# maxpit/human-pose-estimation

Hardware: AMD Instinct MI355X
Metric: images/sec (224x224, batch 256/GPU) (higher is better)
Workload: dtype f32; 1 GPU; batch=256/GPU 224x224x3 synthetic images, fp32 ResNet-50 v1 + 3-iter regressor + SMPL LBS at all 3 stages (configs[1] at batch 256; the BASELINE metric batch); global_batch=256, parallelism=dp1 (batch shard, replicated weights), regressor=synthetic 'survey' variant, input=float32 images resident in HBM

## Files before the change

### human-pose-estimation_amd/_lib.py

```python
from __future__ import annotations

import ctypes as C
import os

import numpy as np

_HERE = os.path.dirname(os.path.abspath(__file__))
LIB_PATH = os.path.join(_HERE, "lib", "libhpe_hip.so")

NUM_CONV = 53
NUM_DENSE = 3
NUM_CRITIC_DENSE = 9
NUM_VERTS = 6890
THETA_DIM = 85
FEATURE_DIM = 2048


class HpeError(RuntimeError):
    pass


class HpeConfig(C.Structure):
    _fields_ = [
        ("struct_size", C.c_int),
        ("device", C.c_int),
        ("max_batch", C.c_int),
        ("num_stage", C.c_int),
        ("bn_eps", C.c_float),
        ("encoder_dtype", C.c_int),
        ("n_streams", C.c_int),
        ("dual_gemm", C.c_int),
        ("stem_fused", C.c_int),
        ("wino_min_c", C.c_int),
        ("wino_min_items", C.c_int),
        ("wino_fused", C.c_int),
        ("wino_fused_min_hw", C.c_int),
        ("mesh_a2b", C.c_int),
        ("wino_f4", C.c_int),
        ("wino4_fused", C.c_int),
        ("bf16_p8", C.c_int),
        ("wino4_ksplit", C.c_int),
        ("chain_fuse", C.c_int),
        ("halo3", C.c_int),
        ("f32_split", C.c_int),
    ]


PLAN_OPTIONS = ("n_streams", "dual_gemm", "stem_fused", "wino_min_c", "wino_min_items", "wino_fused", "wino_fused_min_hw", "mesh_a2b", "wino_f4", "wino4_fused", "bf16_p8", "wino4_ksplit", "chain_fuse", "halo3", "f32_split")


class HpeSmplModel(C.Structure):
    _fields_ = [
        ("v_template", C.c_void_p),
        ("shapedirs", C.c_void_p),
        ("posedirs", C.c_void_p),
        ("J_regressor", C.c_void_p),
        ("weights", C.c_void_p),
        ("kp_regressor", C.c_void_p),
        ("parents", C.c_void_p),
        ("num_kp", C.c_int),
    ]


class HpeCriticModel(C.Structure):
    _fields_ = [("kernel", C.c_void_p * NUM_CRITIC_DENSE), ("bias", C.c_void_p * NUM_CRITIC_DENSE)]


class HpeRenderParams(C.Structure):
    _fields_ = [
        ("struct_size", C.c_int),
        ("color_id", C.c_int),
        ("do_alpha", C.c_int),
        ("rot_axis", C.c_int),
        ("rot_deg", C.c_float),
        ("near", C.c_float),
        ("far", C.c_float),
    ]


class HpeAugmentFrame(C.Structure):
    _fields_ = [("frame_offset", C.c_longlong), ("seg_offset", C.c_longlong), ("H", C.c_int), ("W", C.c_int), ("newH", C.c_int),
                ("newW", C.c_int), ("cx", C.c_int), ("cy", C.c_int), ("fx", C.c_float), ("fy", C.c_float), ("flip", C.c_int),
                ("inside", C.c_int), ("rx", C.c_float), ("ry", C.c_float)]


class HpeJpegInfo(C.Structure):
    _fields_ = [("status", C.c_int), ("H", C.c_int), ("W", C.c_int), ("ncomp", C.c_int), ("hs", C.c_int * 3), ("vs", C.c_int * 3),
                ("blocks_w", C.c_int * 3), ("blocks_h", C.c_int * 3), ("coefs", C.c_longlong)]


class HpeJpegImage(C.Structure):
    _fields_ = [("coef_offset", C.c_longlong * 3), ("plane_offset", C.c_longlong * 3), ("out_offset", C.c_longlong), ("H", C.c_int),
                ("W", C.c_int), ("ncomp", C.c_int), ("channels", C.c_int), ("hmax", C.c_int), ("vmax", C.c_int), ("blocks_w", C.c_int * 3),
                ("blocks_h", C.c_int * 3), ("idct_group0", C.c_int), ("store_group0", C.c_int), ("quant", (C.c_ubyte * 64) * 3)]


class HpeJpegEncImage(C.Structure):
    _fields_ = [("frame_offset", C.c_longlong), ("coef_offset", C.c_longlong * 3), ("H", C.c_int), ("W", C.c_int), ("C", C.c_int),
                ("hmax", C.c_int), ("vmax", C.c_int), ("blocks_w", C.c_int * 3), ("blocks_h", C.c_int * 3), ("real_w", C.c_int * 3),
                ("real_h", C.c_int * 3), ("group0", C.c_int), ("quant", (C.c_ubyte * 64) * 2)]


class HpePngImage(C.Structure):
    _fields_ = [("raw_offset", C.c_longlong), ("pal_offset", C.c_longlong), ("work_offset", C.c_longlong), ("out_offset", C.c_longlong),
                ("H", C.c_int), ("W", C.c_int), ("color_type", C.c_int), ("depth", C.c_int), ("channels", C.c_int), ("rowbytes", C.c_int),
                ("bpp", C.c_int), ("store_group0", C.c_int)]


class HpePngFilterImage(C.Structure):
    _fields_ = [("frame_offset", C.c_longlong), ("scan_offset", C.c_longlong), ("H", C.c_int), ("W", C.c_int), ("C", C.c_int), ("row0", C.c_int)]


def record_dtype(struct):
    d = np.dtype(struct)
    formats = []
    for name in d.names:
        t, shape = d.fields[name][0], ()
        while t.subdtype:
            t, shape = t.subdtype[0], shape + t.subdtype[1]
        formats.append((t, shape))
    return np.dtype({"names": list(d.names), "formats": formats, "offsets": [d.fields[n][1] for n in d.names], "itemsize": d.itemsize})


GEMM_DENSE, GEMM_STRIDED, GEMM_CONV3, GEMM_DUAL = 0, 1, 2, 4
GEMM_TILES = ((128, 128), (128, 64), (64, 64), (64, 128), (128, 128), (128, 64), (256, 128))


class HpeDebugGemm(C.Structure):
    _fields_ = [("struct_size", C.c_int), ("mode", C.c_int), ("tile", C.c_int), ("M", C.c_int), ("N", C.c_int), ("K", C.c_int),
                ("lda", C.c_int), ("ldw", C.c_int), ("ldy", C.c_int), ("ldres", C.c_int), ("w_rows", C.c_int), ("relu", C.c_int),
                ("Hi", C.c_int), ("Wi", C.c_int), ("Cin", C.c_int), ("Ho", C.c_int), ("Wo", C.c_int), ("stride", C.c_int),
                ("k1_slabs", C.c_int), ("y_slab8", C.c_int), ("use_splitk", C.c_int), ("reserved", C.c_int),
                ("x", C.c_void_p), ("x2", C.c_void_p), ("wt", C.c_void_p), ("residual", C.c_void_p), ("scale", C.c_void_p),
                ("shift", C.c_void_p), ("y", C.c_void_p), ("split_k", C.POINTER(C.c_int))]


CONV_KERNELS = ("f32", "f32s", "bf16", "bf16_p8", "halo3", "wino", "wino_fused", "wino4", "wino4_fused")
BLOCK_JOINS = ("separate", "dual", "chain")


class HpeConvRoute(C.Structure):
    _fields_ = [("struct_size", C.c_int), ("kernel", C.c_int), ("mode", C.c_int), ("tile", C.c_int), ("in_slab8", C.c_int), ("out_slab8", C.c_int),
                ("join", C.c_int), ("join_kernel", C.c_int), ("join_tile", C.c_int), ("next_slab8", C.c_int), ("packs", C.c_uint), ("reserved", C.c_int)]


def conv_route(lib, cfg, idx, B, concurrent=False, residual=False, workspace=True):
    r = HpeConvRoute(struct_size=C.sizeof(HpeConvRoute))
    check(lib.hpe_debug_conv_route(C.byref(cfg), int(idx), int(B), int(concurrent), int(residual), int(workspace), C.byref(r)))
    return r


ENCODER_PACKINGS = ("w", "w_split", "wino_u", "wino4_u", "stem_w", "scale", "shift", "w_dual", "w_dual_split", "shift_dual", "dxw", "flat")

OUTPUT_FIELDS = ("verts", "joints", "cams", "theta", "J_transformed", "kp2d", "verts2d", "Rs")


class HpeOutputs(C.Structure):
    _fields_ = [(n, C.c_void_p) for n in OUTPUT_FIELDS]


_PROTOS = {
    "hpe_last_error": (C.c_char_p, []),
    "hpe_version": (C.c_char_p, []),
    "hpe_conv_layer_name": (C.c_char_p, [C.c_int]),
    "hpe_bn_layer_name": (C.c_char_p, [C.c_int]),
    "hpe_conv_layer_geometry": (C.c_int, [C.c_int, C.POINTER(C.c_int)]),
    "hpe_config_init": (None, [C.POINTER(HpeConfig)]),
    "hpe_create": (C.c_int, [C.POINTER(HpeConfig), C.POINTER(C.c_void_p)]),
    "hpe_destroy": (C.c_int, [C.c_void_p]),
    "hpe_load_smpl": (C.c_int, [C.c_void_p, C.POINTER(HpeSmplModel)]),
    "hpe_load_conv": (C.c_int, [C.c_void_p, C.c_int] + [C.c_void_p] * 6),
    "hpe_load_dense": (C.c_int, [C.c_void_p, C.c_int, C.c_void_p, C.c_void_p]),
    "hpe_load_mean_theta": (C.c_int, [C.c_void_p, C.c_void_p]),
    "hpe_finalize": (C.c_int, [C.c_void_p]),
    "hpe_forward": (C.c_int, [C.c_void_p, C.c_void_p, C.c_int, C.POINTER(HpeOutputs), C.c_int, C.c_void_p]),
    "hpe_forward_pipelined": (C.c_int, [C.c_void_p, C.c_void_p, C.c_int, C.POINTER(HpeOutputs), C.c_int, C.c_void_p]),
    "hpe_join": (C.c_int, [C.c_void_p, C.c_void_p]),
    "hpe_tail": (C.c_int, [C.c_void_p, C.c_void_p, C.c_int, C.POINTER(HpeOutputs), C.c_int, C.c_void_p]),
    "hpe_tail_stream": (C.c_void_p, [C.c_void_p]),
    "hpe_encoder": (C.c_int, [C.c_void_p, C.c_void_p, C.c_int, C.c_void_p, C.c_void_p]),
    "hpe_regress_stage": (C.c_int, [C.c_void_p, C.c_void_p, C.c_void_p, C.c_int, C.c_void_p, C.c_void_p]),
    "hpe_smpl": (C.c_int, [C.c_void_p, C.c_void_p, C.c_int, C.POINTER(HpeOutputs), C.c_void_p]),
    "hpe_smpl_backward": (C.c_int, [C.c_void_p, C.c_void_p, C.c_int, C.POINTER(HpeOutputs), C.c_void_p, C.c_void_p]),
    "hpe_orth_proj": (C.c_int, [C.c_void_p, C.c_void_p, C.c_int, C.c_int, C.c_void_p, C.c_void_p]),
    "hpe_reproject_vertices": (C.c_int, [C.c_void_p, C.c_void_p, C.c_int, C.c_int, C.c_float, C.c_float, C.c_void_p, C.c_void_p]),
    "hpe_preprocess_u8": (C.c_int, [C.c_void_p, C.c_int, C.c_int, C.c_int, C.c_void_p, C.POINTER(C.c_int), C.c_void_p]),
    "hpe_preprocess_u8_batch": (C.c_int, [C.c_void_p, C.POINTER(C.c_longlong), C.POINTER(C.c_int), C.c_int, C.c_int, C.c_void_p, C.POINTER(C.c_int),
                                          C.c_void_p, C.c_void_p]),
    "hpe_augment_plan": (C.c_int, [C.c_int, C.c_void_p, C.c_void_p, C.c_void_p, C.c_void_p, C.c_void_p, C.c_int, C.c_void_p, C.c_void_p, C.c_void_p]),
    "hpe_augment_batch": (C.c_int, [C.c_void_p, C.c_void_p, C.c_void_p, C.c_void_p, C.c_void_p, C.c_int, C.c_void_p, C.c_void_p, C.c_void_p, C.c_void_p]),
    "hpe_adam_advance": (C.c_int, [C.c_void_p, C.c_double, C.c_double, C.c_double, C.c_void_p]),
    "hpe_adam_apply": (C.c_int, [C.c_void_p, C.c_void_p, C.c_void_p, C.c_void_p, C.c_longlong, C.c_void_p, C.c_float, C.c_float, C.c_float, C.c_void_p]),
    "hpe_adam_set_step": (C.c_int, [C.c_void_p, C.c_longlong, C.c_double, C.c_double, C.c_void_p]),
    "hpe_debug_adam_power": (C.c_int, [C.c_double, C.c_longlong, C.POINTER(C.c_double)]),
    "hpe_jpeg_info": (C.c_int, [C.c_int, C.c_void_p, C.c_void_p, C.c_void_p]),
    "hpe_jpeg_decode": (C.c_int, [C.c_int, C.c_void_p, C.c_void_p, C.c_void_p, C.c_int, C.c_void_p, C.c_longlong, C.c_void_p, C.c_void_p, C.c_void_p]),
    "hpe_jpeg_backend": (C.c_int, [C.c_void_p, C.c_void_p, C.c_int, C.c_void_p, C.c_longlong, C.c_void_p, C.c_longlong, C.c_void_p, C.c_longlong,
                                   C.c_void_p]),
    "hpe_jpeg_encode_layout": (C.c_int, [C.c_int, C.c_void_p, C.c_void_p, C.c_int, C.c_int, C.c_int, C.c_void_p, C.c_void_p]),
    "hpe_jpeg_forward": (C.c_int, [C.c_void_p, C.c_void_p, C.c_int, C.c_void_p, C.c_longlong, C.c_void_p, C.c_longlong, C.c_void_p]),
    "hpe_jpeg_entropy_encode": (C.c_int, [C.c_void_p, C.c_int, C.c_void_p, C.c_longlong, C.c_int, C.c_int, C.c_int, C.c_int, C.c_void_p, C.c_longlong,
                                          C.c_void_p, C.c_void_p]),
    "hpe_png_backend": (C.c_int, [C.c_void_p, C.c_void_p, C.c_int, C.c_void_p, C.c_longlong, C.c_void_p, C.c_longlong, C.c_void_p, C.c_longlong,
                                  C.c_void_p]),
    "hpe_png_filter": (C.c_int, [C.c_void_p, C.c_void_p, C.c_int, C.c_void_p, C.c_longlong, C.c_void_p, C.c_longlong, C.c_void_p]),
    "hpe_draw_panels": (C.c_int, [C.c_void_p] * 6 + [C.c_int, C.c_int, C.c_int, C.c_void_p, C.c_void_p]),
    "hpe_draw_skeleton": (C.c_int, [C.c_void_p] * 4 + [C.c_int, C.c_int, C.c_int, C.c_int, C.c_int, C.c_void_p]),
    "hpe_get_original": (C.c_int, [C.c_void_p, C.c_void_p, C.c_int, C.c_int, C.c_int, C.POINTER(C.c_int), C.c_float, C.c_int, C.c_void_p, C.POINTER(C.c_float), C.c_void_p, C.c_void_p, C.c_void_p]),
    "hpe_kp_loss": (C.c_int, [C.c_void_p, C.c_void_p, C.c_int, C.c_int, C.c_void_p, C.c_void_p]),
    "hpe_kp_loss_backward": (C.c_int, [C.c_void_p, C.c_void_p, C.c_int, C.c_int, C.c_void_p, C.c_void_p, C.c_void_p]),
    "hpe_mesh_loss": (C.c_int, [C.c_void_p, C.c_void_p, C.c_void_p, C.c_int, C.c_int, C.c_int, C.c_int, C.c_void_p, C.c_void_p]),
    "hpe_mesh_loss_grad": (C.c_int, [C.c_void_p, C.c_void_p, C.c_void_p, C.c_int, C.c_int, C.c_int, C.c_int, C.c_void_p, C.c_void_p, C.c_void_p,
                                     C.c_void_p, C.c_void_p]),
    "hpe_val_losses": (C.c_int, [C.c_void_p, C.c_void_p, C.c_void_p, C.POINTER(C.c_void_p), C.POINTER(C.c_void_p), C.c_int, C.c_int, C.c_int,
                                 C.c_int, C.c_int, C.c_int, C.c_void_p, C.c_void_p]),
    "hpe_critic_layer_name": (C.c_char_p, [C.c_int]),
    "hpe_critic_layer_shape": (C.c_int, [C.c_int, C.POINTER(C.c_int)]),
    "hpe_load_critic": (C.c_int, [C.c_void_p, C.POINTER(HpeCriticModel)]),
    "hpe_critic": (C.c_int, [C.c_void_p, C.c_void_p, C.c_int, C.c_void_p, C.c_int, C.c_void_p, C.c_int, C.c_void_p, C.c_void_p, C.c_void_p]),
    "hpe_critic_backward": (C.c_int, [C.c_void_p, C.c_void_p, C.c_int, C.c_void_p, C.c_int, C.c_void_p, C.c_int, C.c_void_p, C.c_void_p,
                                      C.c_void_p, C.c_void_p, C.c_void_p, C.c_void_p]),
    "hpe_critic_param_floats": (C.c_int, []),
    "hpe_critic_param_offset": (C.c_int, [C.c_int, C.c_int]),
    "hpe_critic_weight_grad_ws_floats": (C.c_longlong, [C.c_int]),
    "hpe_critic_reserve": (C.c_int, [C.c_void_p, C.c_int]),
    "hpe_critic_weight_grad": (C.c_int, [C.c_void_p, C.c_void_p, C.c_int, C.c_void_p, C.c_int, C.c_void_p, C.c_int, C.c_void_p, C.c_void_p,
                                         C.c_void_p, C.c_void_p, C.c_void_p, C.c_int, C.c_void_p, C.c_void_p]),
    "hpe_critic_get_params": (C.c_int, [C.c_void_p, C.c_void_p, C.c_void_p]),
    "hpe_critic_set_params_dev": (C.c_int, [C.c_void_p, C.c_void_p, C.c_void_p]),
    "hpe_regressor_param_floats": (C.c_int, []),
    "hpe_regressor_param_offset": (C.c_int, [C.c_int, C.c_int]),
    "hpe_regressor_get_params": (C.c_int, [C.c_void_p, C.c_void_p, C.c_void_p]),
    "hpe_regressor_set_params_dev": (C.c_int, [C.c_void_p, C.c_void_p, C.c_void_p]),
    "hpe_regressor_forward_train": (C.c_int, [C.c_void_p, C.c_void_p, C.c_int, C.c_void_p, C.c_void_p, C.c_void_p]),
    "hpe_regressor_backward": (C.c_int, [C.c_void_p, C.c_void_p, C.c_int, C.c_void_p, C.c_void_p, C.c_void_p, C.c_void_p, C.c_void_p]),
    "hpe_encoder_param_floats": (C.c_int, []),
    "hpe_encoder_param_offset": (C.c_int, [C.c_int, C.c_int]),
    "hpe_encoder_train_reserve": (C.c_int, [C.c_void_p, C.c_int]),
    "hpe_encoder_train_ws_floats": (C.c_longlong, [C.c_int]),
    "hpe_encoder_wg_slices": (C.c_int, [C.c_int, C.c_int]),
    "hpe_encoder_forward_train": (C.c_int, [C.c_void_p, C.c_void_p, C.c_int, C.c_void_p, C.c_void_p]),
    "hpe_encoder_backward": (C.c_int, [C.c_void_p, C.c_void_p, C.c_int, C.c_void_p, C.c_void_p, C.c_void_p]),
    "hpe_encoder_get_params": (C.c_int, [C.c_void_p, C.c_void_p, C.c_void_p]),
    "hpe_encoder_set_params": (C.c_int, [C.c_void_p, C.c_void_p]),
    "hpe_encoder_set_params_dev": (C.c_int, [C.c_void_p, C.c_void_p, C.c_void_p]),
    "hpe_debug_encoder_packing_bytes": (C.c_longlong, [C.c_void_p, C.c_int, C.c_int]),
    "hpe_debug_encoder_packing": (C.c_int, [C.c_void_p, C.c_int, C.c_int, C.c_void_p, C.c_void_p]),
    "hpe_debug_conv_backward": (C.c_int, [C.c_void_p, C.c_int, C.c_void_p, C.c_void_p, C.c_void_p, C.c_int, C.c_void_p, C.c_void_p, C.c_void_p]),
    "hpe_debug_maxpool_backward": (C.c_int, [C.c_void_p, C.c_void_p, C.c_int, C.c_int, C.c_int, C.c_void_p, C.c_void_p]),
    "hpe_debug_avgpool_backward": (C.c_int, [C.c_void_p, C.c_int, C.c_int, C.c_int, C.c_void_p, C.c_void_p]),
    "hpe_debug_encoder_stash": (C.c_int, [C.c_void_p, C.c_int, C.c_void_p, C.c_void_p]),
    "hpe_debug_encoder_stash_batch": (C.c_int, [C.c_void_p]),
    "hpe_encoder_stat_floats": (C.c_int, []),
    "hpe_encoder_stat_offset": (C.c_int, [C.c_int, C.c_int]),
    "hpe_encoder_train_reserve_batchnorm": (C.c_int, [C.c_void_p, C.c_int]),
    "hpe_encoder_train_ws_floats_batchnorm": (C.c_longlong, [C.c_int]),
    "hpe_debug_encoder_bn_slices": (C.c_int, [C.c_int, C.c_int]),
    "hpe_encoder_forward_batchnorm": (C.c_int, [C.c_void_p, C.c_void_p, C.c_int, C.c_void_p, C.c_void_p]),
    "hpe_encoder_backward_batchnorm": (C.c_int, [C.c_void_p, C.c_void_p, C.c_int, C.c_void_p, C.c_void_p, C.c_void_p]),
    "hpe_encoder_get_stats": (C.c_int, [C.c_void_p, C.c_void_p, C.c_void_p]),
    "hpe_encoder_update_stats": (C.c_int, [C.c_void_p, C.c_void_p, C.c_double, C.c_int, C.c_void_p]),
    "hpe_encoder_set_stats_dev": (C.c_int, [C.c_void_p, C.c_void_p, C.c_void_p]),
    "hpe_debug_conv_batchnorm": (C.c_int, [C.c_void_p, C.c_int, C.c_void_p, C.c_int, C.c_void_p, C.c_int, C.c_void_p, C.c_void_p, C.c_void_p, C.c_void_p]),
    "hpe_debug_conv_backward_batchnorm": (C.c_int, [C.c_void_p, C.c_int, C.c_void_p, C.c_void_p, C.c_void_p, C.c_void_p, C.c_int, C.c_void_p, C.c_void_p,
                                                    C.c_void_p]),
    "hpe_debug_encoder_stash_raw": (C.c_int, [C.c_void_p, C.c_int, C.c_void_p, C.c_void_p]),
    "hpe_debug_encoder_batch_stats": (C.c_int, [C.c_void_p, C.c_void_p, C.c_void_p]),
    "hpe_device_status": (C.c_int, [C.c_void_p, C.c_void_p]),
    "hpe_debug_conv": (C.c_int, [C.c_void_p, C.c_int, C.c_void_p, C.c_int, C.c_void_p, C.c_int, C.c_void_p, C.c_void_p]),
    "hpe_debug_chain": (C.c_int, [C.c_void_p, C.c_int, C.c_void_p, C.c_void_p, C.c_int, C.c_void_p, C.c_void_p, C.POINTER(C.c_int), C.c_void_p]),
    "hpe_debug_stem": (C.c_int, [C.c_void_p, C.c_void_p, C.c_int, C.c_int, C.c_void_p, C.c_void_p]),
    "hpe_debug_gemm": (C.c_int, [C.c_void_p, C.c_void_p, C.c_void_p, C.c_int, C.c_int, C.c_int, C.c_int, C.c_int, C.c_void_p, C.c_int, C.c_void_p, C.c_void_p]),
    "hpe_debug_gemm_ex": (C.c_int, [C.c_void_p, C.POINTER(HpeDebugGemm), C.c_void_p]),
    "hpe_debug_gemm_check": (C.c_int, [C.POINTER(HpeDebugGemm), C.c_int, C.c_int]),
    "hpe_debug_conv_route": (C.c_int, [C.POINTER(HpeConfig), C.c_int, C.c_int, C.c_int, C.c_int, C.c_int, C.POINTER(HpeConvRoute)]),
    "hpe_debug_maxpool": (C.c_int, [C.c_void_p, C.c_int, C.c_int, C.c_int, C.c_void_p, C.c_void_p]),
    "hpe_debug_avgpool": (C.c_int, [C.c_void_p, C.c_int, C.c_int, C.c_int, C.c_void_p, C.c_void_p]),
    "hpe_debug_joint_regress": (C.c_int, [C.c_void_p, C.c_void_p, C.c_int, C.c_int, C.c_void_p, C.c_void_p]),
    "hpe_enable_timing": (C.c_int, [C.c_void_p, C.c_int]),
    "hpe_get_timings": (C.c_int, [C.c_void_p, C.POINTER(C.c_float)]),
    "hpe_get_span_stats": (C.c_int, [C.c_void_p, C.POINTER(C.c_float), C.POINTER(C.c_int)]),
    "hpe_get_loss_timings": (C.c_int, [C.c_void_p, C.POINTER(C.c_float)]),
    "hpe_debug_set_loss_counter": (C.c_int, [C.c_void_p, C.c_void_p]),
    "hpe_get_conv_timings": (C.c_int, [C.c_void_p, C.POINTER(C.c_float)]),
    "hpe_render_params_init": (None, [C.POINTER(HpeRenderParams)]),
    "hpe_renderer_create": (C.c_int, [C.c_int, C.c_void_p, C.c_int, C.c_int, C.c_int, C.POINTER(C.c_void_p)]),
    "hpe_renderer_destroy": (C.c_int, [C.c_void_p]),
    "hpe_render": (C.c_int, [C.c_void_p, C.c_void_p, C.c_void_p, C.c_int, C.c_int, C.c_int, C.c_void_p, C.POINTER(HpeRenderParams), C.c_void_p,
                             C.c_void_p]),
    "hpe_debug_render_ids": (C.c_int, [C.c_void_p, C.c_void_p, C.c_void_p, C.c_int, C.c_int, C.c_int, C.POINTER(HpeRenderParams), C.c_void_p,
                                       C.c_void_p, C.c_void_p]),
    "hpe_debug_render_vertices": (C.c_int, [C.c_void_p, C.c_void_p, C.c_void_p, C.c_int, C.c_int, C.c_int, C.POINTER(HpeRenderParams),
                                            C.c_void_p, C.c_void_p]),
}

_lib = None


def load():
    global _lib
    if _lib is not None:
        return _lib
    if not os.path.exists(LIB_PATH):
        raise HpeError(
            "%s not found: build it with `python -c 'import __graft_entry__ as g; g.build()'` "
# ... 29 lines not shown
```

### human-pose-estimation_amd/build.py

```python
from __future__ import annotations

import os
import shutil
import subprocess
import sys

HERE = os.path.dirname(os.path.abspath(__file__))
CSRC = os.path.join(HERE, "csrc")
LIBDIR = os.path.join(HERE, "lib")
LIB = os.path.join(LIBDIR, "libhpe_hip.so")
SOURCES = ["conv_gemm.hip", "conv_gemm_f32s.hip", "conv_gemm_bf16.hip", "conv_gemm_bf16_p8.hip", "conv_chain_bf16.hip", "conv_chain_f32.hip", "conv3_halo_bf16.hip", "conv_wino.hip", "conv_wino4.hip", "stem_fused.hip", "encoder_ops.hip", "smpl.hip", "losses.hip", "prepost.hip", "render.hip", "hpe_plan.hip", "hpe_finalize.hip", "hpe_encoder.hip", "hpe_api.hip", "hpe_render_api.hip", "smpl_bwd.hip", "critic.hip", "critic_train.hip", "regressor_train.hip", "augment.hip", "encoder_train.hip", "encoder_grad.hip", "encoder_repack.hip", "encoder_bn.hip", "jpeg_entropy.hip", "jpeg_decode.hip", "jpeg_huffman_enc.hip", "jpeg_encode.hip", "png_decode.hip", "png_encode.hip", "draw.hip", "adam.hip"]
CFLAGS = ["--offload-arch=gfx950", "-O3", "-std=c++17", "-fPIC", "-fvisibility=hidden", "-fno-fast-math"]


def _hipcc():
    for cand in (os.environ.get("HIPCC"), shutil.which("hipcc"), "/opt/rocm/bin/hipcc"):
        if cand and os.path.exists(cand):
            return cand
    raise RuntimeError("hipcc not found (set HIPCC or install ROCm under /opt/rocm)")


def _deps():
    return [os.path.join(CSRC, f) for f in os.listdir(CSRC) if f.endswith(".h")] + [os.path.join(HERE, "..", "include", "hpe.h")]


def _obj_stale(src, obj):
    if not os.path.exists(obj):
        return True
    t = os.path.getmtime(obj)
    return any(os.path.getmtime(d) > t for d in [src] + _deps() if os.path.exists(d))


def _flags_now():
    return " ".join(CFLAGS + os.environ.get("HPE_EXTRA_FLAGS", "").split())


def built_flags():
    tag = os.path.join(LIBDIR, "obj", "flags.txt")
    return open(tag).read() if os.path.exists(tag) else ""


def _stale():
    if not os.path.exists(LIB):
        return True
    if built_flags() != _flags_now():
        return True
    t = os.path.getmtime(LIB)
    deps = [os.path.join(CSRC, f) for f in os.listdir(CSRC)] + [os.path.join(HERE, "..", "include", "hpe.h")]
    return any(os.path.getmtime(d) > t for d in deps if os.path.exists(d))


def build(force=False, verbose=False):
    if not force and not _stale():
        return LIB
    os.makedirs(LIBDIR, exist_ok=True)
    objdir = os.path.join(LIBDIR, "obj")
    os.makedirs(objdir, exist_ok=True)
    extra = os.environ.get("HPE_EXTRA_FLAGS", "").split()
    tag = os.path.join(objdir, "flags.txt")
    flags_now = _flags_now()
    if force or not os.path.exists(tag) or open(tag).read() != flags_now:
        for f in os.listdir(objdir):
            os.remove(os.path.join(objdir, f))
    hipcc = _hipcc()
    jobs = []
    for s in SOURCES:
        src = os.path.join(CSRC, s)
        if not os.path.exists(src):
            continue
        obj = os.path.join(objdir, s.replace(".hip", ".o"))
        jobs.append((src, obj))

    def compile_one(job):
        src, obj = job
        if not _obj_stale(src, obj):
            return None
        cmd = [hipcc] + CFLAGS + extra + ["-c", "-o", obj + ".tmp%d" % os.getpid(), src]
        if verbose:
            print(" ".join(cmd), file=sys.stderr)
        r = subprocess.run(cmd, capture_output=True, text=True)
        if r.returncode != 0:
            return "hipcc failed on %s:\n%s%s" % (os.path.basename(src), r.stdout, r.stderr)
        os.replace(obj + ".tmp%d" % os.getpid(), obj)
        return None

    from concurrent.futures import ThreadPoolExecutor

    with ThreadPoolExecutor(max_workers=min(len(jobs), max(1, (os.cpu_count() or 2) - 1))) as ex:
        errs = [e for e in ex.map(compile_one, jobs) if e]
    if errs:
        raise RuntimeError("\n".join(errs))
    open(tag, "w").write(flags_now)
    tmp = LIB + ".tmp%d" % os.getpid()
    cmd = [hipcc, "--offload-arch=gfx950", "-shared", "-fPIC", "-o", tmp] + [o for _, o in jobs]
    r = subprocess.run(cmd, capture_output=True, text=True)
    if r.returncode != 0:
        raise RuntimeError("link failed:\n" + r.stdout + r.stderr)
    os.replace(tmp, LIB)
    return LIB


if __name__ == "__main__":
    print(build(force="--force" in sys.argv, verbose=True))
```

### human-pose-estimation_amd/csrc/encoder_repack.hip

```cpp
#include <hip/hip_runtime.h>

#include <string>

#include "hpe_ctx.h"

namespace {

struct RepackLayer {
    float *w, *scale, *shift, *wino_u, *wino4_u, *dxw;
    unsigned short* w_split;
    int kh, cin, cout, n_pad, k_pad;
    int off[4];
    int stat;
};

struct RepackDual {
    float *w, *shift;
    unsigned short* split;
    int i2c, i1, K1, K2, N, n_pad;
};

enum { F_WT, F_BN, F_WINO, F_WINO4, F_DXW, F_DUAL, F_COUNT };

struct RepackForm {
    int n;
    int item[HPE_NUM_CONV];
    unsigned block0[HPE_NUM_CONV + 1];
};

struct RepackTable {
    RepackLayer L[HPE_NUM_CONV];
    RepackDual D[4];
    RepackForm F[F_COUNT];
};

constexpr int TILE_N = 32, TILE_K = 64;

__device__ inline int find_item(const RepackForm& f, unsigned b, unsigned* local) {
    int s = 0;
    while (s + 1 < f.n && f.block0[s + 1] <= b) ++s;
    *local = b - f.block0[s];
    return f.item[s];
}

__device__ inline void store_split(unsigned short* d, size_t piece, float x) {
    unsigned short h[3];
    bf16_split3(x, h);
    d[0] = h[0];
    d[piece] = h[1];
    d[2 * piece] = h[2];
}

__global__ __launch_bounds__(256) void repack_wt_kernel(const RepackTable* __restrict__ T, const float* __restrict__ flat) {
    unsigned lb;
    const int idx = find_item(T->F[F_WT], blockIdx.x, &lb);
    const RepackLayer& L = T->L[idx];
    const int kt_n = (L.k_pad + TILE_K - 1) / TILE_K;
    const int nt = lb / kt_n, kt = lb - nt * kt_n;
    const int k = kt * TILE_K + (threadIdx.x & 63);
    if (k >= L.k_pad) return;
    long row = -1;
    if (idx == 0) {
        const int kh = k >> 5, kw = (k & 31) >> 2, ci = k & 3;
        if (kh < 7 && kw < 7 && ci < 3) row = (kh * 7 + kw) * 3 + ci;
    } else if (k < L.kh * L.kh * L.cin) {
        row = k;
    }
    const float* src = flat + L.off[0];
    const int n0 = nt * TILE_N + (threadIdx.x >> 6) * 8;
#pragma unroll
    for (int j = 0; j < 8; ++j) {
        const int n = n0 + j;
        if (n >= L.n_pad) break;
        const float v = (row >= 0 && n < L.cout) ? src[row * L.cout + n] : 0.f;
        L.w[(size_t)n * L.k_pad + k] = v;
        if (L.w_split) store_split(L.w_split + (size_t)n * 3 * L.k_pad + k, L.k_pad, v);
    }
}

__global__ __launch_bounds__(256) void repack_bn_kernel(const RepackTable* __restrict__ T, const float* __restrict__ flat,
                                                        const float* __restrict__ mean, const double* __restrict__ sd) {
    unsigned lb;
    const RepackLayer& L = T->L[find_item(T->F[F_BN], blockIdx.x, &lb)];
    const int n = lb * 256 + threadIdx.x;
    if (n >= L.cout) return;
    double scale, shift;
    bn_fold_sd(flat[L.off[2] + n], flat[L.off[1] + n], mean[L.stat + n], flat[L.off[3] + n], sd[L.stat + n], &scale, &shift);
    L.scale[n] = (float)scale;
    L.shift[n] = (float)shift;
}

__global__ __launch_bounds__(256) void repack_stem_kernel(unsigned short* __restrict__ stem_w, const float* __restrict__ kernel) {
    const int o = blockIdx.x * 256 + threadIdx.x;
    if (o >= 64 * 224) return;
    const int n = o / 224, k = o - n * 224;
    const int kh = k >> 5, kw = (k & 31) >> 2, ci = k & 3;
    float v = 0.f;
    if (kw < 7 && ci < 3) v = kernel[((kh * 7 + kw) * 3 + ci) * 64 + n];
    store_split(stem_w + o, 64 * 224, v);
}

template <int TT>
__global__ __launch_bounds__(256) void repack_wino_kernel(const RepackTable* __restrict__ T, const float* __restrict__ flat) {
    unsigned lb;
    const RepackLayer& L = T->L[find_item(T->F[TT == 4 ? F_WINO : F_WINO4], blockIdx.x, &lb)];
    const int c4 = L.cin / 4;
    const int nb = lb / c4, cb = lb - nb * c4;
    const int n = nb * 64 + (threadIdx.x >> 2), ci = cb * 4 + (threadIdx.x & 3);
    const float* src = flat + L.off[0];
    double g[3][3];
#pragma unroll
    for (int a = 0; a < 3; ++a)
#pragma unroll
        for (int b = 0; b < 3; ++b) g[a][b] = src[(((size_t)a * 3 + b) * L.cin + ci) * L.cout + n];
    float* out = TT == 4 ? L.wino_u + wino_u_base(n, ci, L.cin) : L.wino4_u + wino4_u_base(n, ci, L.cin);
    constexpr size_t step = TT == 4 ? 512 : 256;
#pragma unroll
    for (int xi = 0; xi < TT; ++xi)
#pragma unroll
        for (int nu = 0; nu < TT; ++nu) {
            double gx[3], gn[3];
#pragma unroll
            for (int a = 0; a < 3; ++a) {
                gx[a] = TT == 4 ? wino_g(xi, a) : wino4_g(xi, a);
                gn[a] = TT == 4 ? wino_g(nu, a) : wino4_g(nu, a);
            }
            out[(size_t)(xi * TT + nu) * step] = wino_elem(gx, gn, g);
        }
}

__global__ __launch_bounds__(256) void repack_dxw_kernel(const RepackTable* __restrict__ T, const float* __restrict__ flat) {
    unsigned lb;
    const RepackLayer& L = T->L[find_item(T->F[F_DXW], blockIdx.x, &lb)];
    const int taps = L.kh * L.kh, K = taps * L.cout;
    const unsigned o = lb * 256 + threadIdx.x;
    const int ci = (int)(o / (unsigned)K), r = (int)(o - (unsigned)ci * K);
    if (ci >= ((L.cin + 127) / 128) * 128) return;
    const int t = r / L.cout, n = r - t * L.cout;
    L.dxw[o] = ci < L.cin ? flat[L.off[0] + ((size_t)(taps - 1 - t) * L.cin + ci) * L.cout + n] : 0.f;
}

__global__ __launch_bounds__(256) void repack_dual_kernel(const RepackTable* __restrict__ T, const float* __restrict__ flat,
                                                          const float* __restrict__ mean, const double* __restrict__ sd) {
#pragma clang fp contract(off)
    unsigned lb;
    const RepackDual& D = T->D[find_item(T->F[F_DUAL], blockIdx.x, &lb)];
    const int K = D.K1 + D.K2;
    const int kt_n = (K + TILE_K - 1) / TILE_K;
    const int nt = lb / kt_n, kt = lb - nt * kt_n;
    const int k = kt * TILE_K + (threadIdx.x & 63);
    if (k >= K) return;
    const RepackLayer &L2 = T->L[D.i2c], &L1 = T->L[D.i1];
    const RepackLayer& L = k < D.K1 ? L2 : L1;
    const float* src = flat + L.off[0] + (size_t)(k < D.K1 ? k : k - D.K1) * D.N;
    const int n0 = nt * TILE_N + (threadIdx.x >> 6) * 8;
#pragma unroll
    for (int j = 0; j < 8; ++j) {
        const int n = n0 + j;
        if (n >= D.n_pad) break;
        float v = 0.f;
        if (n < D.N) {
            double inv, shift;
            bn_fold_sd(flat[L.off[2] + n], flat[L.off[1] + n], mean[L.stat + n], flat[L.off[3] + n], sd[L.stat + n], &inv, &shift);
            v = (float)(inv * (double)src[n]);
            if (k == 0) {
                double inv1, shift1;
                bn_fold_sd(flat[L1.off[2] + n], flat[L1.off[1] + n], mean[L1.stat + n], flat[L1.off[3] + n], sd[L1.stat + n], &inv1, &shift1);
                D.shift[n] = (float)(shift + shift1);
            }
        }
        D.w[(size_t)n * K + k] = v;
        if (D.split) store_split(D.split + (size_t)n * 3 * K + k, K, v);
    }
}

unsigned blocks_of(int form, const ConvSpec& s, const ConvLayer& L, int idx) {
    switch (form) {
        case F_WT: return (unsigned)(L.n_pad / TILE_N) * ((L.k_pad + TILE_K - 1) / TILE_K);
        case F_BN: return (unsigned)(s.cout + 255) / 256;
        case F_WINO: return L.wino_u ? (unsigned)(s.cin / 4) * (s.cout / 64) : 0;
        case F_WINO4: return L.wino4_u ? (unsigned)(s.cin / 4) * (s.cout / 64) : 0;
        case F_DXW: return (unsigned)((conv_dxw_floats(idx) + 255) / 256);
    }
    return 0;
}

int check_debug(hpe_ctx* c, int idx, int which) {
    if (!c) return fail(HPE_ERR_INVALID, "null ctx");
    if (idx < 0 || idx >= HPE_NUM_CONV || which < 0 || which >= HPE_PACK_COUNT) return fail(HPE_ERR_INVALID, "hpe_debug_encoder_packing: idx or which out of range");
    if (c->dead) return fail(HPE_ERR_STATE, "hpe_finalize failed on this ctx: destroy it and create a new one");
    if (!c->finalized) return fail(HPE_ERR_STATE, "hpe_finalize() has not been called");
    if (!c->have_encoder) return fail(HPE_ERR_STATE, "encoder weights were not loaded before hpe_finalize");
    if (c->bf16) return fail(HPE_ERR_STATE, "hpe_debug_encoder_packing needs an fp32 context");
    return HPE_OK;
}

const void* packing_of(hpe_ctx* c, int idx, int which, size_t* bytes) {
    const ConvSpec& s = specs()[idx];
    const ConvLayer& L = c->conv[idx];
    const size_t wt = (size_t)L.n_pad * L.k_pad, dual = (size_t)round_up(s.cout, 128) * L.k_dual, u = (size_t)s.cin * s.cout;
    const void* p = nullptr;
    size_t n = 0;
    switch (which) {
        case HPE_PACK_W: p = L.w, n = wt * 4; break;
        case HPE_PACK_W_SPLIT: p = L.w_split, n = wt * 3 * 2; break;
        case HPE_PACK_WINO_U: p = L.wino_u, n = u * 16 * 4; break;
        case HPE_PACK_WINO4_U: p = L.wino4_u, n = u * 36 * 4; break;
        case HPE_PACK_STEM_W: p = L.stem_w, n = (size_t)3 * 64 * 224 * 2; break;
        case HPE_PACK_SCALE: p = L.scale, n = (size_t)s.cout * 4; break;
        case HPE_PACK_SHIFT: p = L.shift, n = (size_t)s.cout * 4; break;
        case HPE_PACK_W_DUAL: p = L.w_dual, n = dual * 4; break;
        case HPE_PACK_W_DUAL_SPLIT: p = L.w_dual_split, n = dual * 3 * 2; break;
        case HPE_PACK_SHIFT_DUAL: p = L.shift_dual, n = (size_t)s.cout * 4; break;
        case HPE_PACK_DXW: p = c->et.dxw[idx], n = conv_dxw_floats(idx) * 4; break;
        case HPE_PACK_FLAT:
            if (c->et.flat) p = c->et.flat + layout().off[idx][0];
            n = ((size_t)s.kh * s.kw * s.cin * s.cout + 3 * (size_t)s.cout) * 4;
            break;
    }
    *bytes = p ? n : 0;
    return *bytes ? p : nullptr;
}

}

size_t encoder_repack_reserve_floats() { return (sizeof(RepackTable) + 3) / 4; }

int encoder_repack_reserve(hpe_ctx* c) {
    RepackTable t{};
    for (int i = 0; i < HPE_NUM_CONV; ++i) {
        const ConvSpec& s = specs()[i];
        const ConvLayer& L = c->conv[i];
        RepackLayer& r = t.L[i];
        r.w = L.w;
        r.scale = L.scale;
        r.shift = L.shift;
        r.wino_u = L.wino_u;
        r.wino4_u = L.wino4_u;
        r.dxw = c->et.dxw[i];
        r.w_split = static_cast<unsigned short*>(L.w_split);
        r.kh = s.kh;
        r.cin = s.cin;
        r.cout = s.cout;
        r.n_pad = L.n_pad;
        r.k_pad = L.k_pad;
        for (int w = 0; w < 4; ++w) r.off[w] = layout().off[i][w];
        r.stat = layout().stat[i];
        if (s.kh != s.kw || L.n_pad % TILE_N != 0 || ((L.wino_u || L.wino4_u) && (s.cin % 8 != 0 || s.cout % 64 != 0)))
            return fail(HPE_ERR_STATE, std::string("encoder repack: unexpected geometry of ") + s.name);
    }
    for (int f = 0; f < F_DUAL; ++f) {
        RepackForm& F = t.F[f];
        unsigned b = 0;
        for (int i = 0; i < HPE_NUM_CONV; ++i) {
            const unsigned nb = blocks_of(f, specs()[i], c->conv[i], i);
            if (!nb) continue;
            F.item[F.n] = i;
            F.block0[F.n++] = b;
            b += nb;
        }
        F.block0[F.n] = b;
    }
    {
        RepackForm& F = t.F[F_DUAL];
        unsigned b = 0;
        for (const ResBlock& blk : blocks()) {
            if (!blk.first || !c->conv[blk.i2c].w_dual) continue;
            const ConvLayer& L2 = c->conv[blk.i2c];
            RepackDual& d = t.D[F.n];
            d.w = L2.w_dual;
            d.shift = L2.shift_dual;
            d.split = static_cast<unsigned short*>(L2.w_dual_split);
            d.i2c = blk.i2c;
            d.i1 = blk.i1;
            d.K1 = L2.k1_dual;
            d.K2 = L2.k_dual - L2.k1_dual;
            d.N = specs()[blk.i2c].cout;
            d.n_pad = round_up(d.N, 128);
            F.item[F.n] = F.n;
            F.block0[F.n++] = b;
            b += (unsigned)(d.n_pad / TILE_N) * ((L2.k_dual + TILE_K - 1) / TILE_K);
        }
        F.block0[F.n] = b;
    }
    float* p = nullptr;
    int rc = dev_alloc(c, &p, encoder_repack_reserve_floats(), false);
    if (rc) return rc;
    HIP_TRY(hipMemcpy(p, &t, sizeof(t), hipMemcpyHostToDevice));
    c->et.repack = p;
    static_assert(F_COUNT <= 8, "grid array");
    for (int f = 0; f < F_COUNT; ++f) c->et.repack_grid[f] = t.F[f].block0[t.F[f].n];
    return HPE_OK;
}

hipError_t encoder_repack_launch(hpe_ctx* c, const float* flat, hipStream_t st) {
    const EncTrainWork& w = c->et;
    const RepackTable* T = static_cast<const RepackTable*>(w.repack);
    const unsigned* grid = w.repack_grid;
    if (grid[F_WT]) hipLaunchKernelGGL(repack_wt_kernel, dim3(grid[F_WT]), dim3(256), 0, st, T, flat);
    if (grid[F_BN]) hipLaunchKernelGGL(repack_bn_kernel, dim3(grid[F_BN]), dim3(256), 0, st, T, flat, w.mean, w.sd);
    if (c->conv[0].stem_w)
        hipLaunchKernelGGL(repack_stem_kernel, grid1(64 * 224), dim3(256), 0, st, static_cast<unsigned short*>(c->conv[0].stem_w),
                           flat + layout().off[0][0]);
    if (grid[F_WINO]) hipLaunchKernelGGL(repack_wino_kernel<4>, dim3(grid[F_WINO]), dim3(256), 0, st, T, flat);
    if (grid[F_WINO4]) hipLaunchKernelGGL(repack_wino_kernel<6>, dim3(grid[F_WINO4]), dim3(256), 0, st, T, flat);
    if (grid[F_DXW]) hipLaunchKernelGGL(repack_dxw_kernel, dim3(grid[F_DXW]), dim3(256), 0, st, T, flat);
    if (grid[F_DUAL]) hipLaunchKernelGGL(repack_dual_kernel, dim3(grid[F_DUAL]), dim3(256), 0, st, T, flat, w.mean, w.sd);
    HIPE(hipGetLastError());
    return hipMemcpyAsync(w.flat, flat, (size_t)layout().total * sizeof(float), hipMemcpyDeviceToDevice, st);
}

hipError_t encoder_repack_stats_launch(hpe_ctx* c, hipStream_t st) {
    const EncTrainWork& w = c->et;
    const RepackTable* T = static_cast<const RepackTable*>(w.repack);
    const unsigned* grid = w.repack_grid;
    if (grid[F_BN]) hipLaunchKernelGGL(repack_bn_kernel, dim3(grid[F_BN]), dim3(256), 0, st, T, w.flat, w.mean, w.sd);
    if (grid[F_DUAL]) hipLaunchKernelGGL(repack_dual_kernel, dim3(grid[F_DUAL]), dim3(256), 0, st, T, w.flat, w.mean, w.sd);
    return hipGetLastError();
}

#pragma GCC visibility push(default)
extern "C" {

long long hpe_debug_encoder_packing_bytes(hpe_ctx* c, int idx, int which) {
    if (!c || idx < 0 || idx >= HPE_NUM_CONV || which < 0 || which >= HPE_PACK_COUNT) return 0;
    if (c->dead || !c->finalized || !c->have_encoder || c->bf16) return 0;
    size_t n;
    packing_of(c, idx, which, &n);
    return (long long)n;
}

int hpe_debug_encoder_packing(hpe_ctx* c, int idx, int which, void* dst, void* stream) {
    int rc = check_debug(c, idx, which);
    if (rc) return rc;
    if (!dst) return fail(HPE_ERR_INVALID, "null dst_dev");
    size_t n;
    const void* p = packing_of(c, idx, which, &n);
    if (!p) return fail(HPE_ERR_STATE, "hpe_debug_encoder_packing: this context does not hold that form of that layer");
    DeviceGuard g(c->cfg.device);
    HIP_TRY(hipMemcpyAsync(dst, p, n, hipMemcpyDeviceToDevice, static_cast<hipStream_t>(stream)));
    return HPE_OK;
}

}
#pragma GCC visibility pop
```

### human-pose-estimation_amd/csrc/hpe_api.hip

```cpp
#include <hip/hip_runtime.h>

#include <algorithm>
#include <cmath>
#include <cstdint>
#include <cstdio>
#include <cstdlib>
#include <cstring>
#include <string>
#include <vector>

#include "gemm_contract.h"
#include "hpe_ctx.h"

namespace {
thread_local std::string g_err;
}

int fail(int code, const std::string& msg) {
    g_err = msg;
    return code;
}

int check_ready(hpe_ctx* c, int B, int need) {
    if (!c) return fail(HPE_ERR_INVALID, "null ctx");
    if (c->dead) return fail(HPE_ERR_STATE, "hpe_finalize failed on this ctx: destroy it and create a new one");
    if (!c->finalized) return fail(HPE_ERR_STATE, "hpe_finalize() has not been called");
    if (B < 1 || B > c->cfg.max_batch) return fail(HPE_ERR_INVALID, "batch " + std::to_string(B) + " outside [1, max_batch]");
    if ((need & NEED_ENC) && !c->have_encoder) return fail(HPE_ERR_STATE, "encoder weights were not loaded before hpe_finalize");
    if ((need & NEED_REG) && !c->have_regressor) return fail(HPE_ERR_STATE, "regressor weights / mean theta were not loaded");
    if ((need & NEED_SMPL) && !c->have_smpl) return fail(HPE_ERR_STATE, "SMPL model was not loaded before hpe_finalize");
    return HPE_OK;
}

#pragma GCC visibility push(default)
extern "C" {


const char* hpe_last_error(void) { return g_err.c_str(); }
const char* hpe_version(void) { return "hpe_hip 0.1 (gfx950)"; }

const char* hpe_conv_layer_name(int idx) { return (idx >= 0 && idx < HPE_NUM_CONV) ? specs()[idx].name : nullptr; }
const char* hpe_bn_layer_name(int idx) { return (idx >= 0 && idx < HPE_NUM_CONV) ? specs()[idx].bn : nullptr; }

int hpe_conv_layer_geometry(int idx, int out[7]) {
    if (idx < 0 || idx >= HPE_NUM_CONV || !out) return fail(HPE_ERR_INVALID, "bad conv index");
    const ConvSpec& s = specs()[idx];
    out[0] = s.kh;
    out[1] = s.kw;
    out[2] = s.cin;
    out[3] = s.cout;
    out[4] = s.stride;
    out[5] = s.hin;
    out[6] = s.hout;
    return HPE_OK;
}

void hpe_config_init(HpeConfig* cfg) {
    if (!cfg) return;
    cfg->struct_size = (int)sizeof(HpeConfig);
    cfg->device = 0;
    cfg->max_batch = 8;
    cfg->num_stage = 3;
    cfg->bn_eps = 1e-3f;
    cfg->encoder_dtype = 0;
    cfg->n_streams = cfg->dual_gemm = cfg->stem_fused = cfg->wino_min_c = cfg->wino_min_items = cfg->wino_fused = -1;
    cfg->wino_fused_min_hw = cfg->mesh_a2b = cfg->wino_f4 = cfg->wino4_fused = cfg->bf16_p8 = cfg->wino4_ksplit = cfg->chain_fuse = cfg->halo3 = cfg->f32_split = -1;
}

int hpe_create(const HpeConfig* cfg, hpe_ctx** out) {
    if (!cfg || !out) return fail(HPE_ERR_INVALID, "null argument");
    if (cfg->struct_size != (int)sizeof(HpeConfig))
        return fail(HPE_ERR_INVALID, "HpeConfig.struct_size is " + std::to_string(cfg->struct_size) + ", this library expects " +
                                         std::to_string(sizeof(HpeConfig)) + ": fill the struct with hpe_config_init() of the same header");
    if (cfg->n_streams > 4 || cfg->n_streams == 0) return fail(HPE_ERR_INVALID, "n_streams must be -1 (default) or 1..4");
    if (cfg->mesh_a2b > 2) return fail(HPE_ERR_INVALID, "mesh_a2b must be -1 (default), 0 (grid), 1 (valu) or 2 (mfma)");
    if (cfg->max_batch < 1 || cfg->max_batch > 1024) return fail(HPE_ERR_INVALID, "max_batch must be in [1,1024]");
    if (cfg->num_stage < 1 || cfg->num_stage > 16) return fail(HPE_ERR_INVALID, "num_stage must be in [1,16]");
    if (cfg->encoder_dtype != 0 && cfg->encoder_dtype != 1) return fail(HPE_ERR_INVALID, "encoder_dtype must be 0 (fp32) or 1 (bf16)");
    int ndev = 0;
    if (hipGetDeviceCount(&ndev) != hipSuccess || ndev < 1) return fail(HPE_ERR_NO_DEVICE, "no HIP device visible");
    if (cfg->device < 0 || cfg->device >= ndev) return fail(HPE_ERR_INVALID, "device ordinal out of range");
    hipDeviceProp_t prop;
    HIP_TRY(hipGetDeviceProperties(&prop, cfg->device));
    if (strncmp(prop.gcnArchName, "gfx950", 6) != 0)
        return fail(HPE_ERR_NO_DEVICE, std::string("device is ") + prop.gcnArchName + ", kernels are built for gfx950 only");
    hpe_ctx* c = new hpe_ctx();
    c->cfg = *cfg;
    c->bf16 = cfg->encoder_dtype == 1;
    if (c->cfg.bn_eps <= 0.f) c->cfg.bn_eps = 1e-3f;
    *out = c;
    return HPE_OK;
}

int hpe_destroy(hpe_ctx* c) {
    if (!c) return HPE_OK;
    DeviceGuard g(c->cfg.device);
    (void)hipDeviceSynchronize();
    release_device_state(c);
    delete c;
    return HPE_OK;
}

int hpe_finalize(hpe_ctx* c) {
    if (!c) return fail(HPE_ERR_INVALID, "null ctx");
    if (c->dead) return fail(HPE_ERR_STATE, "an earlier hpe_finalize failed: destroy this ctx and create a new one");
    if (c->finalized) return fail(HPE_ERR_STATE, "already finalized");
    const int rc = finalize_impl(c);
    if (rc != HPE_OK && rc != HPE_ERR_STATE) {
        const std::string keep = g_err;
        DeviceGuard g(c->cfg.device);
        (void)hipDeviceSynchronize();
        release_device_state(c);
        c->dead = true;
        g_err = keep;
    }
    return rc;
}

int hpe_encoder(hpe_ctx* c, const float* images, int B, float* features, void* stream) {
    int rc = check_ready(c, B, NEED_ENC);
    if (rc) return rc;
    if (!images || !features) return fail(HPE_ERR_INVALID, "null pointer");
    DeviceGuard g(c->cfg.device);
    hipStream_t st = static_cast<hipStream_t>(stream);
    if (c->timing) {
        HIP_TRY(hipEventRecord(c->ev[0], st));
        HIP_TRY(hipEventRecord(c->span0[c->span_n % hpe_ctx::SPAN_RING], st));
    }
    HIP_TRY(encoder_impl(c, images, B, features, HPE_FEATURE_DIM, st));
    if (c->timing) {
        HIP_TRY(hipEventRecord(c->span1[c->span_n % hpe_ctx::SPAN_RING], st));
        ++c->span_n;
        HIP_TRY(hipEventRecord(c->ev[1], st));
        HIP_TRY(hipEventRecord(c->ev[4], st));
        c->timed_valid = true;
        c->conv_timed_valid = c->timing >= 2;
    }
    return HPE_OK;
}

int hpe_regress_stage(hpe_ctx* c, const float* features, const float* theta_prev, int B, float* theta_out, void* stream) {
    int rc = check_ready(c, B, NEED_REG);
    if (rc) return rc;
    if (!features || !theta_out) return fail(HPE_ERR_INVALID, "null pointer");
    DeviceGuard g(c->cfg.device);
    hipStream_t st = static_cast<hipStream_t>(stream);
    HIP_TRY(join_tail(c, st));
    HIP_TRY(features_proj(c, features, B, st));
    if (theta_prev)
        HIP_TRY(hpe_launch_copy_theta(theta_prev, HPE_THETA_DIM, c->thA, THETA_LD, B, HPE_THETA_DIM, st));
    else
        HIP_TRY(hpe_launch_tile_theta(c->mean_dev, c->thA, B, THETA_LD, st));
    HIP_TRY(regress_impl(c, c->thA, c->thB, B, st));
    HIP_TRY(hpe_launch_copy_theta(c->thB, THETA_LD, theta_out, HPE_THETA_DIM, B, HPE_THETA_DIM, st));
    return HPE_OK;
}

int hpe_smpl(hpe_ctx* c, const float* theta, int B, const HpeOutputs* outs, void* stream) {
    int rc = check_ready(c, B, NEED_SMPL);
    if (rc) return rc;
    if (!theta || !outs) return fail(HPE_ERR_INVALID, "null pointer");
    DeviceGuard g(c->cfg.device);
    HIP_TRY(join_tail(c, static_cast<hipStream_t>(stream)));
    HIP_TRY(hpe_launch_smpl(c->smpl, c->work, theta, HPE_THETA_DIM, B, outs, static_cast<hipStream_t>(stream)));
    return HPE_OK;
}

int hpe_smpl_backward(hpe_ctx* c, const float* theta, int B, const HpeOutputs* grad_outs, float* grad_theta, void* stream) {
    int rc = check_ready(c, B, NEED_SMPL);
    if (rc) return rc;
    if (!theta || !grad_outs || !grad_theta) return fail(HPE_ERR_INVALID, "null pointer");
    DeviceGuard g(c->cfg.device);
    HIP_TRY(hpe_launch_smpl_backward(c->smpl, c->bwd, theta, B, grad_outs, grad_theta, static_cast<hipStream_t>(stream)));
    return HPE_OK;
}

int hpe_forward(hpe_ctx* c, const float* images, int B, const HpeOutputs* stage_outs, int n_outs, void* stream) {
    return forward_impl(c, images, B, stage_outs, n_outs, static_cast<hipStream_t>(stream), false);
}

int hpe_forward_pipelined(hpe_ctx* c, const float* images, int B, const HpeOutputs* stage_outs, int n_outs, void* stream) {
    return forward_impl(c, images, B, stage_outs, n_outs, static_cast<hipStream_t>(stream), true);
}

int hpe_tail(hpe_ctx* c, const float* features, int B, const HpeOutputs* stage_outs, int n_outs, void* stream) {
    int rc = check_ready(c, B, NEED_REG | NEED_SMPL);
    if (rc) return rc;
    if (!features || !stage_outs) return fail(HPE_ERR_INVALID, "null pointer");
    if (n_outs < 1 || n_outs > c->cfg.num_stage) return fail(HPE_ERR_INVALID, "n_outs must be in [1, num_stage]");
    DeviceGuard g(c->cfg.device);
    hipStream_t st = static_cast<hipStream_t>(stream);
    HIP_TRY(join_tail(c, st));
    c->dense_on_tail = true;
    const hipError_t e = tail_impl(c, features, B, stage_outs, n_outs, st, nullptr);
    c->dense_on_tail = false;
    if (e != hipSuccess) return fail(HPE_ERR_HIP, std::string("hpe_tail: ") + hipGetErrorString(e));
    return HPE_OK;
}

int hpe_join(hpe_ctx* c, void* stream) {
    if (!c || !c->finalized) return fail(HPE_ERR_STATE, "needs a finalized ctx");
    DeviceGuard g(c->cfg.device);
    if (c->tail_pending) HIP_TRY(hipStreamWaitEvent(static_cast<hipStream_t>(stream), c->ev_tail, 0));
    return HPE_OK;
}

void* hpe_tail_stream(hpe_ctx* c) { return (c && c->finalized) ? static_cast<void*>(c->tail_st) : nullptr; }

int hpe_orth_proj(const float* X, const float* cam, int B, int P, float* out, void* stream) {
    if (!X || !cam || !out || B < 1 || P < 1) return fail(HPE_ERR_INVALID, "bad argument");
    HIP_TRY(hpe_launch_orth_proj(X, cam, B, P, 0.f, 0.f, 0, out, static_cast<hipStream_t>(stream)));
    return HPE_OK;
}

int hpe_reproject_vertices(const float* verts, const float* cam, int B, int P, float im_w, float im_h, float* out, void* stream) {
    if (!verts || !cam || !out || B < 1 || P < 1) return fail(HPE_ERR_INVALID, "bad argument");
    HIP_TRY(hpe_launch_orth_proj(verts, cam, B, P, im_w, im_h, 1, out, static_cast<hipStream_t>(stream)));
    return HPE_OK;
}
// ... 692 lines not shown
```

### human-pose-estimation_amd/csrc/hpe_ctx.h

```cpp
#pragma once
#include <hip/hip_runtime.h>

#include <cmath>
#include <cstdint>
#include <cstring>
#include <string>
#include <vector>

#include "../../include/hpe.h"
#include "hpe_internal.h"
#include "hpe_plan.h"

int fail(int code, const std::string& msg);

#define HIP_TRY(expr)                                                                                             \
    do {                                                                                                          \
        hipError_t _e = (expr);                                                                                   \
        if (_e != hipSuccess)                                                                                     \
            return fail(HPE_ERR_HIP, std::string(#expr) + ": " + hipGetErrorString(_e) + " (" __FILE__ ":" +      \
                                         std::to_string(__LINE__) + ")");                                         \
    } while (0)

struct ConvSpec {
    char name[24];
    char bn[24];
    int kh, kw, cin, cout, stride, hin, hout;
};

const std::vector<ConvSpec>& specs();

struct ResBlock {
    int stage;
    bool first, last;
    int i2a, i2b, i2c, i1;
    int in;
};
const std::vector<ResBlock>& blocks();

inline int round_up(int x, int m) { return ((x + m - 1) / m) * m; }

struct ConvLayer {
    std::vector<float> kernel, bias, gamma, beta, mean, var;
    bool loaded = false;
    float* w = nullptr;
    float* scale = nullptr;
    float* shift = nullptr;
    float* w_dual = nullptr;
    float* shift_dual = nullptr;
    int k_dual = 0, k1_dual = 0;
    void* w_split = nullptr;
    void* w_dual_split = nullptr;
    void* stem_w = nullptr;
    float* wino_u = nullptr;
    float* wino4_u = nullptr;
    int n_pad = 0, k_pad = 0;
};

inline int conv_wt_k(int idx, int kh, int kw, int ci) {
    const ConvSpec& s = specs()[idx];
    return idx == 0 ? kh * 32 + kw * 4 + ci : (kh * s.kw + kw) * s.cin + ci;
}

inline int conv_k_pad(int idx, bool bf16) { return round_up(idx == 0 ? 7 * 32 : specs()[idx].kh * specs()[idx].kw * specs()[idx].cin, bf16 ? 64 : 32); }


__host__ __device__ inline size_t wino_u_base(int n, int ci, int cin) {
    return ((((size_t)(n >> 6) * (cin / 8) + (ci >> 3)) * 16) * 2 + ((ci >> 2) & 1)) * 256 + (size_t)(n & 63) * 4 + (ci & 3);
}
__host__ __device__ inline size_t wino4_u_base(int n, int ci, int cin) {
    return (((size_t)(n >> 6) * (cin / 4) + (ci >> 2)) * 36) * 256 + (size_t)(n & 63) * 4 + (ci & 3);
}
__host__ __device__ inline double wino_g(int xi, int a) {
    constexpr double G[4][3] = {{1, 0, 0}, {0.5, 0.5, 0.5}, {0.5, -0.5, 0.5}, {0, 0, 1}};
    return G[xi][a];
}
__host__ __device__ inline double wino4_g(int xi, int a) {
    constexpr double G4[6][3] = {{0.25, 0, 0}, {-1.0 / 6, -1.0 / 6, -1.0 / 6}, {-1.0 / 6, 1.0 / 6, -1.0 / 6},
                                 {1.0 / 24, 1.0 / 12, 1.0 / 6}, {1.0 / 24, -1.0 / 12, 1.0 / 6}, {0, 0, 1}};
    return G4[xi][a];
}
__host__ __device__ inline float wino_elem(const double gx[3], const double gn[3], const double g[3][3]) {
#pragma clang fp contract(off)
    double u = 0.0;
    for (int a = 0; a < 3; ++a)
        for (int b = 0; b < 3; ++b) u += gx[a] * gn[b] * g[a][b];
    return (float)u;
}

__host__ __device__ inline void bn_fold_sd(float gamma, float bias, float mean, float beta, double sd, double* scale, double* shift) {
#pragma clang fp contract(off)
    *scale = (double)gamma / sd;
    *shift = ((double)bias - (double)mean) * *scale + (double)beta;
}
inline double bn_sd(const ConvLayer& L, int n, float eps) { return std::sqrt((double)L.var[n] + (double)eps); }
inline void bn_fold(const ConvLayer& L, int n, float eps, double* scale, double* shift) {
    bn_fold_sd(L.gamma[n], L.bias[n], L.mean[n], L.beta[n], bn_sd(L, n, eps), scale, shift);
}
inline float bn_istd(const ConvLayer& L, int n, float eps) { return (float)(1.0 / std::sqrt((double)L.var[n] + (double)eps)); }

__host__ __device__ inline unsigned short f2bf(float f) {
    unsigned u;
    memcpy(&u, &f, 4);
    return (unsigned short)((u + 0x7FFFu + ((u >> 16) & 1u)) >> 16);
}
__host__ __device__ inline float bf2f(unsigned short h) {
    const unsigned u = (unsigned)h << 16;
    float f;
    memcpy(&f, &u, 4);
    return f;
}
__host__ __device__ inline void bf16_split3(float x, unsigned short h[3]) {
    h[0] = f2bf(x);
    const float r1 = x - bf2f(h[0]);
    h[1] = f2bf(r1);
    const float r2 = r1 - bf2f(h[1]);
    h[2] = f2bf(r2);
}

struct DenseLayer {
    std::vector<float> kernel, bias;
    bool loaded = false;
};

constexpr int STEM_HP = 230;
constexpr int STEM_WP = 232;
constexpr int THETA_LD = 96;
constexpr size_t WINO_V_PITCH = 802816 + 16384;
constexpr size_t WINO_V_SLACK = 524288;


struct RegTrainWork {
    float *w1k = nullptr;
    float *w2k = nullptr;
    float *w3k = nullptr;
    float *p1 = nullptr;
    float *a1 = nullptr, *a2 = nullptr;
    float *th = nullptr;
    float *g = nullptr;
    float *r = nullptr;
    float *da = nullptr;
    float *dz1 = nullptr, *dz2 = nullptr;
    float *sum1 = nullptr;
    float *zeros = nullptr;
    float *partial = nullptr;
    size_t partial_floats = 0;
};

struct EncTrainWork {
    int B = 0;
    int stash_B = 0;
    float *flat = nullptr;
    float *mean = nullptr, *istd = nullptr;
    double *sd = nullptr;
    void *repack = nullptr;
    unsigned repack_grid[8] = {};
    float *stash = nullptr;
    float *g0 = nullptr, *g1 = nullptr;
    float *sbig = nullptr;
    float *t0 = nullptr, *t1 = nullptr, *ssmall = nullptr;
    float *partial = nullptr;
    size_t partial_floats = 0;
    float *dsh = nullptr;
    float *wgp = nullptr;
    float *zeros = nullptr;
    float *feat = nullptr;
    float *dxw[HPE_NUM_CONV] = {};
    int bn_B = 0;
    int bn_stat_B = 0;
    float *zstash = nullptr;
    float *bn_batch = nullptr;
    float *bn_stats = nullptr;
    double *bn_part = nullptr;
    int *bn_hw = nullptr;
};
constexpr int BN_MAX_SLICES = 512;
constexpr int BN_PART_COLS = 262144;
constexpr int WG_MAX_SLICES = 128;
constexpr int WG_WGP_FLOATS = 1152 * 512;
inline size_t conv_dxw_floats(int idx) {
    const ConvSpec& s = specs()[idx];
    return idx == 0 ? 0 : (size_t)round_up(s.cin, 128) * s.kh * s.kw * s.cout;
}
struct EncLayout {
    int off[HPE_NUM_CONV][4];
    int stat[HPE_NUM_CONV];
    size_t stash[HPE_NUM_CONV];
    size_t stash_pool, stash_per_image;
    int total, channels;
};
const EncLayout& layout();

struct hpe_ctx {
    HpeConfig cfg{};
    bool finalized = false;
    bool dead = false;
    HpePlan plan;
    bool bf16 = false;
    bool have_encoder = false, have_regressor = false, have_smpl = false;
    ConvLayer conv[HPE_NUM_CONV];
    DenseLayer dense[HPE_NUM_DENSE];
    bool smpl_loaded = false, mean_loaded = false;
    std::vector<float> h_vt, h_sd, h_pd, h_jreg, h_w, h_kreg;
    std::vector<int> h_par;
    int num_kp = 19;
    float h_mean[HPE_THETA_DIM];
    float *w1f = nullptr, *w1t = nullptr, *w2 = nullptr, *w3 = nullptr, *b1 = nullptr, *b2 = nullptr, *b3 = nullptr;
    float *ones = nullptr, *zeros = nullptr, *mean_dev = nullptr;
    EncTrainWork et{};
    RegTrainWork rt{};
    SmplDev smpl{};
    SmplWork work{};
    SmplBwdWork bwd{};
    float* smpl_basis_src = nullptr;
    float *padded = nullptr, *X0 = nullptr, *X1 = nullptr, *T1 = nullptr, *T2 = nullptr, *SC = nullptr;
    float *feat = nullptr, *P1 = nullptr, *H1 = nullptr, *H2 = nullptr, *thA = nullptr, *thB = nullptr;
    float* critic_buf = nullptr;
    CriticW critic{};
    bool have_critic = false;
    float* critic_ws = nullptr;
    size_t critic_ws_floats = 0;
    float* loss_ws = nullptr;
    size_t loss_ws_floats = 0;
    std::vector<void*> allocs;
    float* partial = nullptr;
    size_t partial_floats = 0;
    float* wino_v = nullptr;
    float* wino_ws = nullptr;
    unsigned* wino_flags = nullptr;
    unsigned* dev_err = nullptr;
    unsigned wino_epoch = 0;
    int n_cu = 0;
    bool loss_attr_done = false;
    unsigned long long* loss_counter = nullptr;
    hipStream_t aux[3]{};
    hipEvent_t ev_fork{}, ev_join[3]{};
    hipStream_t tail_st{};
    hipEvent_t ev_enc{}, ev_tail{}, ev_feat_free[2]{};
    bool feat_free_valid[2] = {false, false};
    bool tail_pending = false;
    unsigned pipe_idx = 0;
    float* feat_alt = nullptr;
    int co_running = 1;
    float* w4_split = nullptr;
    float* partial_tail = nullptr;
    size_t partial_tail_floats = 0;
    bool dense_on_tail = false;
    int timing = 0;
    hipEvent_t ev[8]{};
    static constexpr int SPAN_RING = 64;
    hipEvent_t span0[SPAN_RING]{}, span1[SPAN_RING]{};
    unsigned span_n = 0;
    hipEvent_t cev0[HPE_NUM_CONV]{}, cev1[HPE_NUM_CONV]{};
    hipEvent_t lev0[16]{}, lev1[16]{}, lev_all[2]{};
    int loss_timed_stages = 0;
    bool ev_ok = false, timed_valid = false, conv_timed_valid = false;
};

struct DeviceGuard {
    int prev = -1;
    bool changed = false;
    explicit DeviceGuard(int dev) {
        if (hipGetDevice(&prev) == hipSuccess && prev != dev) changed = hipSetDevice(dev) == hipSuccess;
    }
    ~DeviceGuard() {
        if (changed) (void)hipSetDevice(prev);
    }
};

int dev_alloc(hpe_ctx* c, float** p, size_t n_floats, bool zero);
// ... 63 lines not shown
```

### human-pose-estimation_amd/csrc/hpe_encoder.hip

```cpp
#include <hip/hip_runtime.h>

#include <cmath>
#include <cstdint>
#include <cstdio>
#include <cstdlib>
#include <cstring>
#include <string>
#include <vector>

#include "hpe_ctx.h"

static hipError_t launch_gemm(hpe_ctx* c, GemmArgs& p, const ConvRoute& r, const void* w_split, hipStream_t st) {
    if (!r.concurrent) p.partial = c->partial, p.partial_floats = c->partial_floats;
    if (r.kernel == CONV_K_BF16 || r.kernel == CONV_K_BF16_P8) return hpe_launch_gemm_bf16(p, r.mode, r.tile, st);
    if (r.kernel != CONV_K_F32S) return hpe_launch_gemm(p, r.mode, r.tile, c->plan.splitk_min_slabs, st);
    if (!w_split) return hipErrorInvalidValue;
    p.w = static_cast<const float*>(w_split);
    p.w_piece = p.ldw;
    p.ldw *= 3;
    return hpe_launch_gemm_f32s(p, r.mode, r.tile, st);
}

hipError_t run_conv(hpe_ctx* c, int idx, const ConvRoute& r, const float* x, int B, const float* res, int relu, float* y, hipStream_t st,
                    float* wino_v, int slot, const float* scale, const float* shift) {
    const ConvSpec& s = specs()[idx];
    const ConvLayer& L = c->conv[idx];
    if (!scale) scale = L.scale;
    if (!shift) shift = L.shift;
    const int H = s.hin;
    const bool f2 = r.kernel == CONV_K_WINO || r.kernel == CONV_K_WINO_FUSED, f4 = r.kernel == CONV_K_WINO4 || r.kernel == CONV_K_WINO4_FUSED;
    if ((r.kernel >= CONV_K_HALO3 && res) || (f2 && !L.wino_u) || (f4 && !L.wino4_u) || ((f2 || f4) && !r.in_slab8 && !wino_v)) return hipErrorInvalidValue;
    switch (r.kernel) {
        case CONV_K_WINO4_FUSED: return hpe_launch_wino4_fused_conv3(x, L.wino4_u, scale, shift, c->zeros, y, s.cout, B, H, H, s.cin, s.cout, relu, st);
        case CONV_K_WINO_FUSED: return hpe_launch_wino_fused_conv3(x, L.wino_u, scale, shift, c->zeros, y, s.cout, B, H, H, s.cin, s.cout, relu, st);
        case CONV_K_WINO4:
            return hpe_launch_wino4_conv3(x, s.cin, L.wino4_u, scale, shift, y, s.cout, B, H, H, s.cin, s.cout, relu, wino_v, st, r.concurrent ? c->co_running : 1,
                                          c->w4_split && slot >= 0 && slot < 4 ? c->w4_split + (size_t)slot * hpe_wino4_split_ws_floats() : nullptr, c->plan.wino4_n32,
                                          c->plan.w4_abl);
        case CONV_K_WINO: {
            WinoStreamK sk{};
            if (c->wino_ws && slot >= 0 && slot < 4) {
                sk.ws = c->wino_ws + (size_t)slot * c->n_cu * HPE_WINO_WS_FLOATS;
                sk.flags = c->wino_flags + (size_t)slot * c->n_cu;
                sk.epoch = ++c->wino_epoch;
                if (sk.epoch == 0) sk.epoch = ++c->wino_epoch;
                sk.n_wg = c->n_cu;
                sk.err = c->dev_err;
            }
            return hpe_launch_wino_conv3(x, s.cin, L.wino_u, scale, shift, y, s.cout, B, H, H, s.cin, s.cout, relu, wino_v, c->wino_ws ? &sk : nullptr, st);
        }
        case CONV_K_HALO3: {
            Halo3Args h{};
            h.x = reinterpret_cast<const __bf16*>(x), h.w = reinterpret_cast<const __bf16*>(L.w), h.y = reinterpret_cast<__bf16*>(y);
            h.scale = scale, h.shift = shift;
            h.M = B * s.hout * s.hout, h.N = s.cout, h.ldw = L.k_pad;
            h.relu = relu, h.two = c->plan.halo3_two;
            return hpe_launch_halo3_bf16(h, H, s.cin, st);
        }
    }
    GemmArgs p{};
    p.x = x, p.w = L.w, p.scale = scale, p.shift = shift, p.res = res, p.y = y, p.zero = c->zeros;
    p.M = B * s.hout * s.hout, p.N = s.cout, p.K = L.k_pad;
    p.lda = s.cin, p.ldw = L.k_pad, p.w_rows = L.n_pad, p.ldy = p.ldres = s.cout;
    p.Hi = p.Wi = H, p.Cin = s.cin, p.Ho = p.Wo = s.hout, p.stride = s.stride;
    p.cin_slabs = s.cin / (c->bf16 ? 64 : 32);
    p.relu = relu, p.y_slab8 = r.out_slab8 ? 1 : 0;
    if (r.mode == GEMM_STEM) p.Hi = STEM_HP, p.Wi = STEM_WP, p.Cin = 4;
    return launch_gemm(c, p, r, L.w_split, st);
}

hipError_t run_conv_nhwc(hpe_ctx* c, int idx, const float* x, int B, const float* res, int relu, float* y, hipStream_t st, const float* scale,
                         const float* shift) {
    const ConvRoute r = route_conv(c->plan, c->bf16, idx, ConvQuery{B, false, res != nullptr, c->wino_v != nullptr});
    if (r.in_slab8) {
        const ConvSpec& s = specs()[idx];
        HIPE(hpe_launch_nhwc_to_slab8(x, c->T1, (long)B * s.hin * s.hin, s.cin, st));
        x = c->T1;
    }
    return run_conv(c, idx, r, x, B, res, relu, y, st, c->wino_v, 0, scale, shift);
}

static hipError_t run_dual(hpe_ctx* c, int i2c, int i1, const ConvRoute& r, const float* t2, const float* x, int B, float* y, hipStream_t st) {
    const ConvSpec& s2 = specs()[i2c];
    const ConvSpec& s1 = specs()[i1];
    const ConvLayer& L = c->conv[i2c];
    GemmArgs p{};
    p.x = t2, p.x2 = x, p.w = L.w_dual, p.scale = c->ones, p.shift = L.shift_dual, p.y = y, p.zero = c->zeros;
    p.M = B * s2.hout * s2.hout, p.N = s2.cout, p.K = L.k_dual;
    p.k1_slabs = L.k1_dual / (c->bf16 ? 64 : 32), p.relu = 1;
    p.lda = s2.cin, p.ldw = L.k_dual, p.w_rows = round_up(s2.cout, 128), p.ldy = s2.cout;
    p.Hi = p.Wi = s1.hin, p.Cin = s1.cin, p.Ho = p.Wo = s1.hout, p.stride = s1.stride;
    return launch_gemm(c, p, r, L.w_dual_split, st);
}

hipError_t run_chain(hpe_ctx* c, int i2c, bool first, const float* t2, const float* res, int B, float* t3, float* u1, hipStream_t st,
                     bool u1_slab8) {
    const ConvSpec& s2 = specs()[i2c];
    const int inext = i2c + (first ? 2 : 1);
    const ConvSpec& sn = specs()[inext];
    const ConvLayer& L2 = c->conv[i2c];
    const ConvLayer& Ln = c->conv[inext];
    if (!c->bf16) {
        ChainArgsF32 q{};
        q.t2 = t2;
        q.res = res;
        q.w2c = L2.w;
        q.w2a = Ln.w;
        q.scaleA = L2.scale;
        q.shiftA = L2.shift;
        q.scaleB = Ln.scale;
        q.shiftB = Ln.shift;
        q.t3 = t3;
        q.u1 = u1;
        q.M = B * s2.hout * s2.hout;
        q.ldw2c = L2.k_pad;
        q.ldw2a = Ln.k_pad;
        q.u1_slab8 = u1_slab8 ? 1 : 0;
        return hpe_launch_chain_f32(q, s2.cin, s2.cout, sn.cout, st);
    }
    ChainArgs p{};
    p.t2 = reinterpret_cast<const __bf16*>(t2);
    if (first) {
        p.x2 = reinterpret_cast<const __bf16*>(res);
        p.w2c = reinterpret_cast<const __bf16*>(L2.w_dual);
        p.scaleA = c->ones;
        p.shiftA = L2.shift_dual;
        p.ldw2c = L2.k_dual;
    } else {
        p.res = reinterpret_cast<const __bf16*>(res);
        p.w2c = reinterpret_cast<const __bf16*>(L2.w);
        p.scaleA = L2.scale;
        p.shiftA = L2.shift;
        p.ldw2c = L2.k_pad;
    }
    p.w2a = reinterpret_cast<const __bf16*>(Ln.w);
    p.scaleB = Ln.scale;
    p.shiftB = Ln.shift;
    p.t3 = reinterpret_cast<__bf16*>(t3);
    p.u1 = reinterpret_cast<__bf16*>(u1);
    p.M = B * s2.hout * s2.hout;
    p.ldw2a = Ln.k_pad;
    return hpe_launch_chain_bf16(p, s2.cin, s2.cout, sn.cout, first ? specs()[i2c + 1].cin : 0, st);
}

hipError_t run_dense(hpe_ctx* c, const float* x, int lda, int M, int K, const float* w, int w_rows, int N, const float* scale,
                     const float* shift, const float* res, int ldres, int relu, float* y, int ldy, hipStream_t st, float* partial,
                     size_t partial_floats) {
    if (M <= 4) return hpe_launch_dense_gemv(x, lda, M, K, w, N, scale, shift, res, ldres, relu, y, ldy, st);
    GemmArgs p{};
    p.zero = shift;
    p.partial = partial ? partial : c->dense_on_tail ? c->partial_tail : c->partial;
    p.partial_floats = partial ? partial_floats : c->dense_on_tail ? c->partial_tail_floats : c->partial_floats;
    p.x = x;
    p.w = w;
    p.scale = scale;
    p.shift = shift;
    p.res = res;
    p.y = y;
    p.M = M;
    p.N = N;
    p.K = K;
    p.lda = lda;
    p.ldw = K;
    p.w_rows = w_rows;
    p.ldy = ldy;
    p.ldres = ldres;
    p.relu = relu;
    return hpe_launch_gemm(p, GEMM_DENSE, TILE_64x64, c->plan.splitk_min_slabs, st);
}

static hipError_t timed_conv(hpe_ctx* c, int idx, const ConvRoute& r, const float* x, int B, const float* res, int relu, float* y, hipStream_t st,
                             float* wino_v = nullptr, int slot = 0) {
    const bool t2 = c->timing >= 2;
    if (t2) HIPE(hipEventRecord(c->cev0[idx], st));
    HIPE(run_conv(c, idx, r, x, B, res, relu, y, st, wino_v, slot));
    if (t2) HIPE(hipEventRecord(c->cev1[idx], st));
    return hipSuccess;
}

static hipError_t encoder_chunk(hpe_ctx* c, const float* images, int i0, int B, float* features, int ldfeat, hipStream_t st, int slot = 0,
                         bool concurrent = false) {
    const int esz = c->bf16 ? 2 : 4;
    auto at = [&](float* base, size_t elems) { return reinterpret_cast<float*>(reinterpret_cast<char*>(base) + elems * esz); };
    const size_t o_img = (size_t)i0 * HPE_IMG_SIZE * HPE_IMG_SIZE * 3;
    const size_t o_pad = (size_t)i0 * STEM_HP * STEM_WP * 4;
    const size_t o_big = (size_t)i0 * 802816;
    const size_t o_mid = (size_t)i0 * 200704;
    float* padded = at(c->padded, o_pad);
    float* SC = at(c->SC, o_big);
    float* T1 = at(c->T1, o_mid);
    float* T2 = at(c->T2, o_mid);
    float* cur = at(c->X0, o_big);
    float* nxt = at(c->X1, o_big);
    float* wv = (c->wino_v && (i0 == 0 || B >= 32)) ? c->wino_v + (size_t)i0 * WINO_V_PITCH : nullptr;
    const ConvQuery q{B, concurrent, false, wv != nullptr};
    if (c->plan.stem_fused && (reinterpret_cast<uintptr_t>(images + o_img) & 15) == 0) {
        const bool t2 = c->timing >= 2;
        if (t2) HIPE(hipEventRecord(c->cev0[0], st));
        HIPE(hpe_launch_stem_fused(images + o_img, c->conv[0].stem_w, c->conv[0].scale, c->conv[0].shift, cur, B, hpe_stem_fused_pick_rows(B),
                                   c->bf16 ? 1 : 0, st));
        if (t2) HIPE(hipEventRecord(c->cev1[0], st));
    } else if (c->bf16) {
        HIPE(hpe_launch_pad_input_bf16(images + o_img, padded, B, HPE_IMG_SIZE, HPE_IMG_SIZE, STEM_HP, STEM_WP, st));
        HIPE(timed_conv(c, 0, route_conv(c->plan, true, 0, q), padded, B, nullptr, 1, SC, st));
// ... 184 lines not shown
```

### human-pose-estimation_amd/csrc/hpe_finalize.hip

```cpp
#include <hip/hip_runtime.h>

#include <algorithm>
#include <cmath>
#include <cstdint>
#include <cstdio>
#include <cstdlib>
#include <cstring>
#include <string>
#include <vector>

#include "hpe_ctx.h"

int dev_alloc(hpe_ctx* c, float** p, size_t n_floats, bool zero) {
    void* q = nullptr;
    HIP_TRY(hipMalloc(&q, n_floats * sizeof(float)));
    c->allocs.push_back(q);
    if (zero) HIP_TRY(hipMemset(q, 0, n_floats * sizeof(float)));
    *p = static_cast<float*>(q);
    return HPE_OK;
}

int upload(hpe_ctx* c, float** p, const std::vector<float>& h) {
    int rc = dev_alloc(c, p, h.size(), false);
    if (rc) return rc;
// ... 90 lines not shown
    if (c->finalized) return fail(HPE_ERR_STATE, "already finalized");
    if (!kernel || !bias) return fail(HPE_ERR_INVALID, "null dense array");
    const int din[3] = {2133, 1024, 1024}, dout[3] = {1024, 1024, 85};
    c->dense[idx].kernel.assign(kernel, kernel + (size_t)din[idx] * dout[idx]);
    c->dense[idx].bias.assign(bias, bias + dout[idx]);
    c->dense[idx].loaded = true;
    return HPE_OK;
}

int hpe_load_mean_theta(hpe_ctx* c, const float* mean85) {
    if (!c || !mean85) return fail(HPE_ERR_INVALID, "null argument");
    if (c->finalized) return fail(HPE_ERR_STATE, "already finalized");
    memcpy(c->h_mean, mean85, sizeof(float) * HPE_THETA_DIM);
    c->mean_loaded = true;
    return HPE_OK;
}

}
#pragma GCC visibility pop

void release_device_state(hpe_ctx* c) {
    for (void* p : c->allocs) (void)hipFree(p);
    c->allocs.clear();
    c->rt = RegTrainWork{};
    c->et = EncTrainWork{};
    if (c->critic_buf) {
        (void)hipFree(c->critic_buf);
        c->critic_buf = nullptr;
        c->critic = CriticW{};
        c->have_critic = false;
    }
    if (c->critic_ws) {
        (void)hipFree(c->critic_ws);
        c->critic_ws = nullptr;
        c->critic_ws_floats = 0;
    }
    for (auto& a : c->aux)
        if (a) {
            (void)hipStreamDestroy(a);
            a = nullptr;
        }
    auto kill = [](hipEvent_t& e) {
        if (e) {
            (void)hipEventDestroy(e);
            e = nullptr;
        }
    };
    kill(c->ev_fork);
    kill(c->ev_enc);
    kill(c->ev_tail);
    for (auto& e : c->ev_feat_free) kill(e);
    if (c->tail_st) {
        (void)hipStreamDestroy(c->tail_st);
        c->tail_st = nullptr;
    }
    for (auto& e : c->ev_join) kill(e);
    for (auto& e : c->ev) kill(e);
    for (auto& e : c->span0) kill(e);
    for (auto& e : c->span1) kill(e);
    for (auto& e : c->cev0) kill(e);
    for (auto& e : c->cev1) kill(e);
    for (auto& e : c->lev0) kill(e);
    for (auto& e : c->lev1) kill(e);
    for (auto& e : c->lev_all) kill(e);
    c->ev_ok = false;
}

static int check_loaded(hpe_ctx* c) {
    int nconv = 0, ndense = 0;
    for (int i = 0; i < HPE_NUM_CONV; ++i) nconv += c->conv[i].loaded ? 1 : 0;
    for (int i = 0; i < HPE_NUM_DENSE; ++i) ndense += c->dense[i].loaded ? 1 : 0;
    if (nconv != 0 && nconv != HPE_NUM_CONV) {
        for (int i = 0; i < HPE_NUM_CONV; ++i)
            if (!c->conv[i].loaded) return fail(HPE_ERR_STATE, std::string("conv layer not loaded: ") + specs()[i].name);
    }
    if (ndense != 0 && (ndense != HPE_NUM_DENSE || !c->mean_loaded))
        return fail(HPE_ERR_STATE, "regressor needs all 3 dense layers and the mean theta");
    c->have_encoder = nconv == HPE_NUM_CONV;
    c->have_regressor = ndense == HPE_NUM_DENSE && c->mean_loaded;
    c->have_smpl = c->smpl_loaded;
    if (!c->have_encoder && !c->have_regressor && !c->have_smpl) return fail(HPE_ERR_STATE, "nothing was loaded");
    return HPE_OK;
}

static int pack_dual_weights(hpe_ctx* c) {
    int rc;
    for (const ResBlock& blk : blocks()) {
        const unsigned packs = layer_packs(c->plan, c->bf16, blk.i2c);
        if (!(packs & PACK_W_DUAL)) continue;
        const ConvSpec& s2 = specs()[blk.i2c];
        const ConvSpec& s1 = specs()[blk.i1];
        ConvLayer& L2 = c->conv[blk.i2c];
        const ConvLayer& L1 = c->conv[blk.i1];
        const int K1 = s2.cin, K2 = s1.cin, N = s2.cout;
        const int n_pad = round_up(N, 128), K = K1 + K2;
        std::vector<float> wt((size_t)n_pad * K, 0.f), sh(N);
        for (int n = 0; n < N; ++n) {
            double inv2, inv1, shift2, shift1;
            bn_fold(L2, n, c->cfg.bn_eps, &inv2, &shift2);
            bn_fold(L1, n, c->cfg.bn_eps, &inv1, &shift1);
            for (int k = 0; k < K1; ++k) wt[(size_t)n * K + k] = (float)(inv2 * (double)L2.kernel[(size_t)k * N + n]);
            for (int k = 0; k < K2; ++k) wt[(size_t)n * K + K1 + k] = (float)(inv1 * (double)L1.kernel[(size_t)k * N + n]);
            sh[n] = (float)(shift2 + shift1);
        }
        if (c->bf16) {
            if ((rc = upload_bf16(c, &L2.w_dual, to_bf16(wt)))) return rc;
        } else {
            if ((rc = upload_to(c, &L2.w_dual, wt))) return rc;
            if ((packs & PACK_W_DUAL_SPLIT) && (rc = upload_split(c, &L2.w_dual_split, wt, n_pad, K))) return rc;
        }
        if ((rc = upload_to(c, &L2.shift_dual, sh))) return rc;
        L2.k_dual = K;
        L2.k1_dual = K1;
    }
    return HPE_OK;
}

static int pack_wino_weights(hpe_ctx* c, const ConvSpec& s, ConvLayer& L) {
    int rc;
    std::vector<float> U((size_t)16 * s.cin * s.cout);
    for (int ci = 0; ci < s.cin; ++ci)
        for (int n = 0; n < s.cout; ++n) {
            double g[3][3];
            for (int a = 0; a < 3; ++a)
                for (int b = 0; b < 3; ++b) g[a][b] = L.kernel[(((size_t)a * 3 + b) * s.cin + ci) * s.cout + n];
            const size_t base = wino_u_base(n, ci, s.cin);
            for (int xi = 0; xi < 4; ++xi)
                for (int nu = 0; nu < 4; ++nu) {
                    const double gx[3] = {wino_g(xi, 0), wino_g(xi, 1), wino_g(xi, 2)}, gn[3] = {wino_g(nu, 0), wino_g(nu, 1), wino_g(nu, 2)};
                    U[base + (size_t)(xi * 4 + nu) * 512] = wino_elem(gx, gn, g);
                }
        }
    if ((rc = upload_to(c, &L.wino_u, U))) return rc;
    return HPE_OK;
}

static int pack_wino4_weights(hpe_ctx* c, const ConvSpec& s, ConvLayer& L) {
    int rc;
    std::vector<float> U((size_t)36 * s.cin * s.cout);
    for (int ci = 0; ci < s.cin; ++ci)
        for (int n = 0; n < s.cout; ++n) {
            double g[3][3];
            for (int a = 0; a < 3; ++a)
                for (int b = 0; b < 3; ++b) g[a][b] = L.kernel[(((size_t)a * 3 + b) * s.cin + ci) * s.cout + n];
            const size_t base = wino4_u_base(n, ci, s.cin);
            for (int xi = 0; xi < 6; ++xi)
                for (int nu = 0; nu < 6; ++nu) {
                    const double gx[3] = {wino4_g(xi, 0), wino4_g(xi, 1), wino4_g(xi, 2)}, gn[3] = {wino4_g(nu, 0), wino4_g(nu, 1), wino4_g(nu, 2)};
                    U[base + (size_t)(xi * 6 + nu) * 256] = wino_elem(gx, gn, g);
                }
        }
    if ((rc = upload_to(c, &L.wino4_u, U))) return rc;
    return HPE_OK;
}

static int pack_stem_weights(hpe_ctx* c, ConvLayer& L) {
    const size_t ld = 7 * 32;
    std::vector<float> wp(64 * ld, 0.f);
    for (int kh = 0; kh < 7; ++kh)
        for (int kw = 0; kw < 7; ++kw)
            for (int ci = 0; ci < 3; ++ci) {
                const int k = conv_wt_k(0, kh, kw, ci);
                for (int n = 0; n < 64; ++n) wp[n * ld + k] = L.kernel[(((size_t)kh * 7 + kw) * 3 + ci) * 64 + n];
            }
    if (c->bf16) return upload_bf16(c, &L.stem_w, to_bf16(wp));
    std::vector<unsigned short> ws(3 * wp.size());
    for (size_t o = 0; o < wp.size(); ++o) {
        unsigned short h[3];
        bf16_split3(wp[o], h);
        for (int j = 0; j < 3; ++j) ws[j * wp.size() + o] = h[j];
    }
    return upload_bf16(c, &L.stem_w, ws);
}

static int pack_conv_weights(hpe_ctx* c) {
    int rc;
    for (int i = 0; i < HPE_NUM_CONV; ++i) {
        const ConvSpec& s = specs()[i];
        ConvLayer& L = c->conv[i];
        const unsigned packs = layer_packs(c->plan, c->bf16, i);
        L.n_pad = round_up(s.cout, 128);
        L.k_pad = conv_k_pad(i, c->bf16);
        std::vector<float> wt((size_t)L.n_pad * L.k_pad, 0.f);
        for (int kh = 0; kh < s.kh; ++kh)
            for (int kw = 0; kw < s.kw; ++kw)
                for (int ci = 0; ci < s.cin; ++ci) {
                    const int k = conv_wt_k(i, kh, kw, ci);
                    const float* src = &L.kernel[(((size_t)kh * s.kw + kw) * s.cin + ci) * s.cout];
                    for (int n = 0; n < s.cout; ++n) wt[(size_t)n * L.k_pad + k] = src[n];
                }
        if (c->bf16) {
            if ((rc = upload_bf16(c, &L.w, to_bf16(wt)))) return rc;
        } else {
            if ((rc = upload_to(c, &L.w, wt))) return rc;
            if ((packs & PACK_W_SPLIT) && (rc = upload_split(c, &L.w_split, wt, L.n_pad, L.k_pad))) return rc;
            if ((packs & PACK_WINO_U) && (rc = pack_wino_weights(c, s, L))) return rc;
            if ((packs & PACK_WINO4_U) && (rc = pack_wino4_weights(c, s, L))) return rc;
        }
        if ((packs & PACK_STEM_W) && (rc = pack_stem_weights(c, L))) return rc;
        std::vector<float> sc(s.cout), sh(s.cout);
        for (int n = 0; n < s.cout; ++n) {
            double scale, shift;
            bn_fold(L, n, c->cfg.bn_eps, &scale, &shift);
            sc[n] = (float)scale;
            sh[n] = (float)shift;
        }
        if ((rc = upload_to(c, &L.scale, sc))) return rc;
        if ((rc = upload_to(c, &L.shift, sh))) return rc;
        std::vector<float>().swap(L.kernel);
    }
    return HPE_OK;
}

static int pack_regressor(hpe_ctx* c) {
    int rc;
    const struct {
        float** p;
        size_t n;
    } live[] = {
        {&c->w1f, (size_t)1024 * 2048},
        {&c->w1t, (size_t)1024 * THETA_LD},
        {&c->w2, (size_t)1024 * 1024},
        {&c->w3, (size_t)128 * 1024},
        {&c->b1, 1024},
        {&c->b2, 1024},
        {&c->b3, 128},
        {&c->mean_dev, HPE_THETA_DIM},
        {&c->rt.w1k, (size_t)(2048 + 128) * 1024},
        {&c->rt.w2k, (size_t)1024 * 1024},
        {&c->rt.w3k, (size_t)1024 * THETA_LD},
    };
    for (const auto& b : live)
        if ((rc = dev_alloc(c, b.p, b.n, true))) return rc;
    std::vector<float> flat((size_t)regressor_param_offset(4, false));
    for (int i = 0; i < HPE_NUM_DENSE; ++i) {
        std::copy(c->dense[i].kernel.begin(), c->dense[i].kernel.end(), flat.begin() + regressor_param_offset(i, false));
        std::copy(c->dense[i].bias.begin(), c->dense[i].bias.end(), flat.begin() + regressor_param_offset(i, true));
    }
    std::copy(c->h_mean, c->h_mean + HPE_THETA_DIM, flat.begin() + regressor_param_offset(3, false));
    float* tmp = nullptr;
    if ((rc = upload(c, &tmp, flat))) return rc;
    HIP_TRY(regressor_params_copy(c, tmp, true, nullptr));
    HIP_TRY(hipDeviceSynchronize());
    c->allocs.pop_back();
    HIP_TRY(hipFree(tmp));
    return HPE_OK;
}

static int pack_smpl(hpe_ctx* c) {
    int rc;
    const int V = HPE_NUM_VERTS, V3 = V * 3;
    std::vector<float> src((size_t)11 * V3);
    memcpy(src.data(), c->h_vt.data(), sizeof(float) * V3);
    for (int i = 0; i < V3; ++i)
        for (int k = 0; k < 10; ++k) src[(size_t)(1 + k) * V3 + i] = c->h_sd[(size_t)i * 10 + k];
    if ((rc = upload(c, &c->smpl_basis_src, src))) return rc;
    c->smpl.v_template = c->smpl_basis_src;
    c->smpl.shapedirs = c->smpl_basis_src + V3;
    std::vector<float> pd((size_t)207 * V3);
    for (int i = 0; i < V3; ++i)
        for (int k = 0; k < 207; ++k) pd[(size_t)k * V3 + i] = c->h_pd[(size_t)i * 207 + k];
    float* p = nullptr;
    if ((rc = upload(c, &p, pd))) return rc;
    c->smpl.posedirs = p;
    if ((rc = upload(c, &p, c->h_w))) return rc;
    c->smpl.weights = p;
    std::vector<float> jr((size_t)V * SMPL_KP_PITCH, 0.f), kr((size_t)V * SMPL_KP_PITCH, 0.f);
    for (int j = 0; j < 24; ++j)
        for (int v = 0; v < V; ++v) jr[(size_t)v * SMPL_KP_PITCH + j] = c->h_jreg[(size_t)j * V + v];
    for (int j = 0; j < c->num_kp; ++j)
        for (int v = 0; v < V; ++v) kr[(size_t)v * SMPL_KP_PITCH + j] = c->h_kreg[(size_t)j * V + v];
    if ((rc = upload(c, &p, jr))) return rc;
    c->smpl.j_reg = p;
    if ((rc = upload(c, &p, kr))) return rc;
    c->smpl.kp_reg = p;
    int depth[24], maxd = 0;
    for (int j = 0; j < 24; ++j) {
        depth[j] = c->h_par[j] < 0 ? 0 : depth[c->h_par[j]] + 1;
        if (depth[j] > maxd) maxd = depth[j];
    }
    void* ip = nullptr;
    HIP_TRY(hipMalloc(&ip, sizeof(int) * 48));
    c->allocs.push_back(ip);
    HIP_TRY(hipMemcpy(ip, c->h_par.data(), sizeof(int) * 24, hipMemcpyHostToDevice));
    HIP_TRY(hipMemcpy(static_cast<int*>(ip) + 24, depth, sizeof(int) * 24, hipMemcpyHostToDevice));
    c->smpl.parents = static_cast<int*>(ip);
    c->smpl.depth = static_cast<int*>(ip) + 24;
    c->smpl.max_depth = maxd;
    c->smpl.num_kp = c->num_kp;
    float* jb = nullptr;
    if ((rc = dev_alloc(c, &jb, 11 * 24 * 3, true))) return rc;
    HIP_TRY(hpe_launch_joint_regress(c->smpl_basis_src, c->smpl.j_reg, 11, 24, jb, nullptr, nullptr, nullptr));
    HIP_TRY(hipDeviceSynchronize());
    c->smpl.j_basis = jb;
    return HPE_OK;
}

static int size_workspaces(hpe_ctx* c) {
    int rc;
    const size_t B = (size_t)c->cfg.max_batch;
    const size_t Bpad = (size_t)round_up(c->cfg.max_batch, SMPL_IMG_TILE);
    if (c->have_encoder) {
        if ((rc = dev_alloc(c, &c->padded, B * STEM_HP * STEM_WP * 4 + 64, true))) return rc;
        if ((rc = dev_alloc(c, &c->X0, B * 802816, false))) return rc;
        if ((rc = dev_alloc(c, &c->X1, B * 802816, false))) return rc;
        if ((rc = dev_alloc(c, &c->SC, B * 802816, false))) return rc;
        if ((rc = dev_alloc(c, &c->T1, B * 200704, false))) return rc;
        if ((rc = dev_alloc(c, &c->T2, B * 200704, false))) return rc;
        if ((rc = dev_alloc(c, &c->feat, B * HPE_FEATURE_DIM, true))) return rc;
        if ((rc = dev_alloc(c, &c->feat_alt, B * HPE_FEATURE_DIM, true))) return rc;
    }
    if (c->have_encoder && !c->bf16 && c->plan.wino_min_c > 0) {
        if ((rc = dev_alloc(c, &c->wino_v, B * WINO_V_PITCH + WINO_V_SLACK, false))) return rc;
        if (c->plan.wino_f4 && c->plan.wino4_ksplit) {
            const size_t nws = hpe_wino4_split_ws_floats();
            if ((rc = dev_alloc(c, &c->w4_split, 4 * nws, false))) return rc;
            for (int k = 0; k < 4; ++k) HIP_TRY(hipMemset(c->w4_split + (k + 1) * nws - 256, 0, 256 * sizeof(unsigned)));
        }
        if (c->plan.wino_streamk) {
            hipDeviceProp_t prop;
            HIP_TRY(hipGetDeviceProperties(&prop, c->cfg.device));
            c->n_cu = prop.multiProcessorCount;
            if ((rc = dev_alloc(c, &c->wino_ws, (size_t)4 * c->n_cu * HPE_WINO_WS_FLOATS, false))) return rc;
            float* fl = nullptr;
            if ((rc = dev_alloc(c, &fl, (size_t)4 * c->n_cu + 4, true))) return rc;
            c->wino_flags = reinterpret_cast<unsigned*>(fl);
            c->dev_err = c->wino_flags + (size_t)4 * c->n_cu;
        }
    }
    {
        c->partial_floats = (size_t)512 * 128 * 128;
        if ((rc = dev_alloc(c, &c->partial, c->partial_floats, false))) return rc;
        c->partial_tail_floats = (size_t)64 * 128 * 128;
        if ((rc = dev_alloc(c, &c->partial_tail, c->partial_tail_floats, false))) return rc;
    }
    if (c->have_regressor) {
        if ((rc = dev_alloc(c, &c->P1, B * 1024, true))) return rc;
        if ((rc = dev_alloc(c, &c->H1, B * 1024, true))) return rc;
        if ((rc = dev_alloc(c, &c->H2, B * 1024, true))) return rc;
        if ((rc = dev_alloc(c, &c->thA, B * THETA_LD, true))) return rc;
        if ((rc = dev_alloc(c, &c->thB, B * THETA_LD, true))) return rc;
        const size_t S = (size_t)c->cfg.num_stage;
        RegTrainWork& t = c->rt;
        if ((rc = dev_alloc(c, &t.p1, B * 1024, true))) return rc;
        if ((rc = dev_alloc(c, &t.a1, S * B * 1024, true))) return rc;
        if ((rc = dev_alloc(c, &t.a2, S * B * 1024, true))) return rc;
        if ((rc = dev_alloc(c, &t.th, (S + 1) * B * THETA_LD, true))) return rc;
        if ((rc = dev_alloc(c, &t.g, (S + 1) * B * THETA_LD, true))) return rc;
        if ((rc = dev_alloc(c, &t.r, B * THETA_LD, true))) return rc;
        if ((rc = dev_alloc(c, &t.da, B * 1024, true))) return rc;
// ... 78 lines not shown
```

### human-pose-estimation_amd/csrc/hpe_internal.h

```cpp
#pragma once
#include <hip/hip_runtime.h>
#include <stddef.h>

#include "../../include/hpe.h"

typedef float f32x4 __attribute__((ext_vector_type(4)));
typedef float f32x16 __attribute__((ext_vector_type(16)));

template <typename Id>
__device__ __forceinline__ int xcd_remap(Id bid, int total) {
    const int xcd = bid & 7;
    const int q = total >> 3, rr = total & 7;
    return (xcd < rr ? xcd * (q + 1) : rr * (q + 1) + (xcd - rr) * q) + (bid >> 3);
}

inline dim3 grid1(long n) { return dim3((unsigned)((n + 255) / 256)); }

enum GemmMode { GEMM_DENSE = 0, GEMM_STRIDED = 1, GEMM_CONV3 = 2, GEMM_STEM = 3, GEMM_DUAL = 4 };
enum GemmTile { TILE_128x128 = 0, TILE_128x64 = 1, TILE_64x64 = 2, TILE_64x128 = 3, TILE_128x128_W8 = 4, TILE_128x64_W8 = 5, TILE_256x128_W8 = 6,
                TILE_P8_256x256 = 7  };

struct GemmArgs {
    const float* x;
    const float* w;
    const float* scale;
    const float* shift;
    const float* res;
    float* y;
    int M, N, K;
    int lda, ldw, ldy, ldres, w_rows;
    int relu;
    int Hi, Wi, Cin, Ho, Wo, stride, cin_slabs;
    int n_mtiles, n_ntiles;
    int split_k;
    float* partial;
    size_t partial_floats;
    const float* zero;
    void* reserved;
    const float* x2;
    int k1_slabs;
    int res_prefetch;
    int y_slab8;
    int w_piece;
};

hipError_t hpe_launch_gemm(GemmArgs p, int mode, int tile, int splitk_min_slabs, hipStream_t st, int* split_k_out = nullptr);
hipError_t hpe_launch_gemm_f32s(GemmArgs p, int mode, int tile, hipStream_t st);

size_t hpe_wino_v_floats(int B, int H, int W, int C);
hipError_t hpe_wino_init_device();
#define HPE_WINO_WS_FLOATS 65536
struct WinoStreamK {
    float* ws;
    unsigned* flags;
    unsigned epoch;
    int n_wg;
    unsigned* err;
};
hipError_t hpe_launch_wino_conv3(const float* x, int lda, const float* U, const float* scale, const float* shift, float* y, int ldy,
                                 int B, int H, int W, int C, int N, int relu, float* V, const WinoStreamK* sk, hipStream_t st);

hipError_t hpe_launch_wino_fused_conv3(const float* xs, const float* U, const float* scale, const float* shift, const float* zero16, float* y,
                                       int ldy, int B, int H, int W, int C, int N, int relu, hipStream_t st);
int hpe_wino_fused_items(int B, int H, int W, int N);
hipError_t hpe_launch_nhwc_to_slab8(const float* x, float* xs, long M, int C, hipStream_t st);

size_t hpe_wino4_v_floats(int B, int H, int W, int C);
int hpe_wino4_items(int B, int H, int W, int N);
hipError_t hpe_wino4_init_device();
hipError_t hpe_launch_wino4_conv3(const float* x, int lda, const float* U, const float* scale, const float* shift, float* y, int ldy, int B,
                                  int H, int W, int C, int N, int relu, float* V, hipStream_t st, int co_running, float* split_ws, int n32_below, int abl);
size_t hpe_wino4_split_ws_floats();

hipError_t hpe_launch_wino4_fused_conv3(const float* xs, const float* U, const float* scale, const float* shift, const float* zero16, float* y,
                                        int ldy, int B, int H, int W, int C, int N, int relu, hipStream_t st);
int hpe_wino4_fused_items(int B, int H, int W, int N);

hipError_t hpe_launch_gemm_bf16(GemmArgs p, int mode, int tile, hipStream_t st);
hipError_t hpe_launch_gemm_bf16_p8(GemmArgs p, int mode, hipStream_t st);
struct ChainArgs {
    const __bf16* t2;
    const __bf16* res;
    const __bf16* x2;
    const __bf16* w2c;
    const __bf16* w2a;
    const float *scaleA, *shiftA;
    const float *scaleB, *shiftB;
    __bf16* t3;
    __bf16* u1;
    int M, ldw2c, ldw2a;
};
struct Halo3Args {
    const __bf16* x;
    const __bf16* w;
    const float* scale;
    const float* shift;
    __bf16* y;
    int M, N, ldw, relu;
    int n_ntiles;
    int two;
};
bool hpe_halo3_bf16_supported(int HW, int Cin, int N);
hipError_t hpe_launch_halo3_bf16(const Halo3Args& p, int HW, int Cin, hipStream_t st);

bool hpe_chain_bf16_supported(int C, int C4, int CP, int C2);
hipError_t hpe_launch_chain_bf16(const ChainArgs& p, int C, int C4, int CP, int C2, hipStream_t st);
hipError_t hpe_chain_bf16_occupancy(int out[3]);
struct ChainArgsF32 {
    const float *t2, *res, *w2c, *w2a, *scaleA, *shiftA, *scaleB, *shiftB;
    float *t3, *u1;
    int M, ldw2c, ldw2a, u1_slab8;
};
bool hpe_chain_f32_supported(int C, int C4, int CP);
hipError_t hpe_launch_chain_f32(const ChainArgsF32& p, int C, int C4, int CP, hipStream_t st);
hipError_t hpe_chain_f32_occupancy(int* out);
hipError_t hpe_launch_f32_to_bf16(const float* x, void* y, long n, hipStream_t st);
hipError_t hpe_launch_bf16_to_f32(const void* x, float* y, long n, hipStream_t st);
hipError_t hpe_launch_pad_input_bf16(const float* img, void* out, int B, int H, int W, int Hp, int Wp, hipStream_t st);
hipError_t hpe_launch_maxpool_bf16(const void* x, void* y, int B, int H, int C, hipStream_t st);
hipError_t hpe_launch_avgpool_bf16(const void* x, float* y, int B, int HW, int C, int ldy, hipStream_t st);

hipError_t hpe_launch_stem_fused(const float* img, const void* w, const float* scale, const float* shift, void* y, int B, int R, int bf16,
                                 hipStream_t st);
hipError_t hpe_stem_fused_init_device();
int hpe_stem_fused_pick_rows(int B);

hipError_t hpe_launch_pad_input(const float* img, float* out, int B, int H, int W, int Hp, int Wp, hipStream_t st);
hipError_t hpe_launch_maxpool(const float* x, float* y, int B, int H, int C, hipStream_t st);
hipError_t hpe_launch_avgpool(const float* x, float* y, int B, int HW, int C, int ldy, hipStream_t st);
hipError_t hpe_launch_dense_gemv(const float* x, int lda, int M, int K, const float* wt, int N, const float* scale, const float* shift, const float* res,
                                 int ldres, int relu, float* y, int ldy, hipStream_t st);
hipError_t hpe_launch_tile_theta(const float* mean85, float* theta, int B, int ld, hipStream_t st);
hipError_t hpe_launch_copy_theta(const float* src, int lds, float* dst, int ldd, int B, int n, hipStream_t st);

struct SmplDev {
    const float* v_template;
    const float* shapedirs;
    const float* posedirs;
    const float* weights;
    const float* kp_reg;
    const float* j_reg;
    const float* j_basis;
    const int* parents;
    const int* depth;
    int num_kp;
    int max_depth;
};
#define SMPL_V 6890
#define SMPL_KP_PITCH 24
#define SMPL_IMG_TILE 8
#define SMPL_SMALL_B 8

struct SmplWork {
    float* pfT;
    float* betaT;
    float* A;
    float* cams;
    float* verts_tmp;
    float* kp_part;
    int Bpad;
};

struct HpeOutputs;
hipError_t hpe_launch_smpl(const SmplDev& d, const SmplWork& w, const float* theta, int ldtheta, int B, const HpeOutputs* o,
                           hipStream_t st);
hipError_t hpe_launch_joint_regress(const float* X, const float* reg, int n, int K, float* out, const float* cams,
                                    float* kp2d, hipStream_t st);
hipError_t hpe_launch_orth_proj(const float* X, const float* cam, int B, int P, float sx, float sy, int pixels, float* out,
                                hipStream_t st);

#define SMPL_BWD_PART 512
struct SmplBwdWork {
    float* pfT;
    float* betaT;
    float* A;
    float* cams;
    float* rjg;
    float* gj;
    float* part;
    int Bpad;
};
size_t hpe_smpl_bwd_part_floats(int Bpad);
hipError_t hpe_launch_smpl_backward(const SmplDev& d, const SmplBwdWork& w, const float* theta, int B, const HpeOutputs* g,
                                    float* grad_theta, hipStream_t st);

#define CRITIC_ROWS 4
struct CriticLayerSpec {
    const char* name;
    int in, out;
};
const CriticLayerSpec* hpe_critic_layers();
struct CriticW {
    const float* w[HPE_NUM_CRITIC_DENSE];
    const float* wt[HPE_NUM_CRITIC_DENSE];
    const float* b[HPE_NUM_CRITIC_DENSE];
};
size_t hpe_critic_live_floats();
CriticW hpe_critic_live_view(const float* buf);
hipError_t hpe_launch_critic(const CriticW& w, const float* joints, int K, const float* betas, int betas_stride, const float* Rs, long N,
                             float* scores, float* kcs, hipStream_t st);
hipError_t hpe_launch_critic_backward(const CriticW& w, const float* joints, int K, const float* betas, int betas_stride, const float* Rs,
                                      long N, const float* grad_scores, float* grad_joints, float* grad_betas, float* grad_Rs,
                                      float* grad_kcs, hipStream_t st);

#define CRITIC_PARAM_FLOATS 114273
#define CRITIC_WG_ROW_FLOATS 1664
#define CRITIC_WG_CHUNK 64
int hpe_critic_wg_chunks(long N);
size_t hpe_critic_wg_ws_floats(long N);
int hpe_critic_flat_offset(int idx, bool bias);
hipError_t hpe_launch_critic_weight_grad(const CriticW& w, const float* joints, int K, const float* betas, int betas_stride, const float* Rs,
                                         long N, const float* grad_scores, const float* t_kcs, const float* t_joints, const float* t_betas,
                                         const float* t_Rs, int tangent_per_row, float* ws, float* grad_params, hipStream_t st);
hipError_t hpe_launch_critic_params(const CriticW& w, float* flat, bool set, hipStream_t st);

hipError_t hpe_launch_kp_loss(const float* gt, const float* pred, int n, float* out, hipStream_t st);
hipError_t hpe_launch_kp_loss_backward(const float* gt, const float* pred, int n, const float* grad_loss, float* grad_pred, hipStream_t st);
hipError_t hpe_losses_init_device();
size_t hpe_mesh_loss_ws_floats(int B, int H, int W, int P);
hipError_t hpe_launch_mesh_loss(const float* seg, const float* v2d, int B, int H, int W, int P, float* ws, float* out,
                                hipStream_t st, int a2b_mode, unsigned long long* counter);
hipError_t hpe_launch_mesh_loss_prepare(const float* seg, int B, int H, int W, int P, float* ws, hipStream_t st);
hipError_t hpe_launch_mesh_loss_search(const float* v2d, int B, int H, int W, int P, float* ws, float* out, hipStream_t st,
                                       hipEvent_t ev_a2b0, hipEvent_t ev_a2b1, int a2b_mode, unsigned long long* counter);

hipError_t hpe_launch_mesh_loss_grad(const float* seg, const float* v2d, int B, int H, int W, int P, float* ws, float* out, float* grad,
                                     int* nn_pix, int* nn_vert, hipStream_t st, int a2b_mode, unsigned long long* counter);

hipError_t hpe_launch_preprocess_u8(const unsigned char* img, int H, int W, int C, int newH, int newW, int start_x, int start_y,
                                    int margin, float* out, int S, hipStream_t st);
struct PreprocFrame {
    long long offset;
    int H, W, newH, newW, start_x, start_y;
};
hipError_t hpe_launch_preprocess_u8_batch(const unsigned char* img, const PreprocFrame* table_dev, PreprocFrame uni, int B, int C, int margin,
                                          float* out, int S, hipStream_t st);
hipError_t hpe_launch_shift_verts(const float* verts, const float* cam, int B, int P, float flength, float img_size, float* out,
                                  hipStream_t st);

struct RenderVert {
    int U, V;
    int valid;
    int pad;
    float iz;
    float r, g, b;
};
struct RenderArgs {
    const float* verts;
    const float* cam;
    const int* faces;
    const int* adj_off;
    const int* adj_face;
    RenderVert* rec;
    uint2* box;
    float* center;
    const unsigned char* bg;
// ... 13 lines not shown
```

### human-pose-estimation_amd/csrc/hpe_plan.h

```cpp
#pragma once
#include "../../include/hpe.h"
#include "hpe_internal.h"

struct HpePlan {
    int n_streams = 2;
    int dual_gemm = 1;
    int stem_fused = 1;
    int wino_min_c = 128;
    int wino_min_items = 128;
    int wino_fused = 1;
    int wino_fused_min_hw = 28;
    int mesh_a2b = 0;
    int wino_f4 = 7;
    int wino4_fused = 0;
    int bf16_p8 = 0;
    int wino4_ksplit = 1;
    int chain_fuse = 0;
    int halo3 = 0;
    int f32_split = 0;
    int chunk_images = 0;
    int min_chunk = 32;
    int halo3_two = 4;
    int f32s_min_tiles = 128;
    int wino_streamk = 0;
    int concurrent_tiles = 0;
    int bf16_w8_min_tiles = 128;
    int wide128_min_tiles = 384;
    int force_wide = -1;
    int splitk_min_slabs = 4;
    int wino4_min_items = 64;
    int wino4_n32 = 256;
    int w4_abl = 0;
};

constexpr int PLAN_BF16_128_MIN_TILES = 192;
constexpr int PLAN_BF16_P8_MIN_N = 256;
constexpr int PLAN_BF16_P8_MIN_K = 512;
constexpr int PLAN_EXPAND_SMALL_GRID = 128;
constexpr int PLAN_SHORTK_TILE = TILE_128x64_W8;
constexpr int PLAN_F32S_TILE = TILE_128x128;
constexpr int PLAN_F32S_EXPAND_TILE = TILE_128x128_W8;
constexpr int PLAN_F32S_EXPAND_MIN_K = 256;

HpePlan hpe_resolve_plan(const HpeConfig& cfg);

inline int stage_bit(int hout) { return hout >= 56 ? 1 : (hout >= 28 ? 2 : (hout >= 14 ? 4 : 8)); }
inline int f4_bit(int hin) { return hin <= 7 ? 1 : (hin <= 14 ? 2 : (hin <= 28 ? 4 : 8)); }

constexpr unsigned PACK_W_SPLIT = 1u << HPE_PACK_W_SPLIT, PACK_WINO_U = 1u << HPE_PACK_WINO_U, PACK_WINO4_U = 1u << HPE_PACK_WINO4_U,
                   PACK_STEM_W = 1u << HPE_PACK_STEM_W, PACK_W_DUAL = 1u << HPE_PACK_W_DUAL, PACK_W_DUAL_SPLIT = 1u << HPE_PACK_W_DUAL_SPLIT;
unsigned layer_packs(const HpePlan& pl, bool bf16, int idx);

enum ConvKernel { CONV_K_F32 = 0, CONV_K_F32S, CONV_K_BF16, CONV_K_BF16_P8, CONV_K_HALO3, CONV_K_WINO, CONV_K_WINO_FUSED, CONV_K_WINO4, CONV_K_WINO4_FUSED };
struct ConvQuery { int B; bool concurrent, residual, workspace; };
struct ConvRoute {
    int kernel, mode, tile;
    bool in_slab8;
    bool out_slab8;
    bool concurrent;
};
enum BlockJoin { JOIN_SEPARATE = 0, JOIN_DUAL, JOIN_CHAIN };
struct BlockRoute {
    ConvRoute r2a, r2b, r2c, r1;
    int join;
    bool u1_slab8;
};
struct ResBlock;
ConvRoute route_conv(const HpePlan& pl, bool bf16, int idx, const ConvQuery& q);
BlockRoute route_block(const HpePlan& pl, bool bf16, const ResBlock& blk, ConvQuery q);
int pick_tile(const HpePlan& pl, int M, int N, int K, bool residual_expand = false, bool concurrent = false);
```

### human-pose-estimation_amd/csrc/hpe_plan.hip

```cpp
#include <hip/hip_runtime.h>

#include <climits>
#include <cmath>
#include <cstdint>
#include <cstdio>
#include <cstdlib>
#include <cstring>
#include <string>
#include <vector>

#include "gemm_contract.h"
#include "hpe_ctx.h"

namespace {

struct Network {
    std::vector<ConvSpec> specs;
    std::vector<ResBlock> blocks;
};

Network build_network() {
    Network net;
    std::vector<ConvSpec>& v = net.specs;
    auto add = [&](const std::string& n, const std::string& b, int kh, int cin, int cout, int s, int hin, int hout) {
        ConvSpec c;
        snprintf(c.name, sizeof c.name, "%s", n.c_str());
        snprintf(c.bn, sizeof c.bn, "%s", b.c_str());
        c.kh = c.kw = kh;
        c.cin = cin;
        c.cout = cout;
        c.stride = s;
        c.hin = hin;
        c.hout = hout;
        v.push_back(c);
    };
    add("conv1", "bn_conv1", 7, 3, 64, 2, 224, 112);
    const int nblk[4] = {3, 4, 6, 3};
    const int filt[4][3] = {{64, 64, 256}, {128, 128, 512}, {256, 256, 1024}, {512, 512, 2048}};
    int cin = 64, h = 56;
    int in = -1;
    for (int st = 0; st < 4; ++st) {
        for (int b = 0; b < nblk[st]; ++b) {
            const bool first = b == 0;
            const int s = (first && st > 0) ? 2 : 1;
            const int hout = h / s;
            const int i2a = (int)v.size();
            net.blocks.push_back(ResBlock{st, first, b == nblk[st] - 1, i2a, i2a + 1, i2a + 2, first ? i2a + 3 : -1, in});
            in = i2a + 2;
            char base[24], bn[24];
            snprintf(base, sizeof base, "res%d%c_branch", st + 2, 'a' + b);
            snprintf(bn, sizeof bn, "bn%d%c_branch", st + 2, 'a' + b);
            add(std::string(base) + "2a", std::string(bn) + "2a", 1, cin, filt[st][0], s, h, hout);
            add(std::string(base) + "2b", std::string(bn) + "2b", 3, filt[st][0], filt[st][1], 1, hout, hout);
            add(std::string(base) + "2c", std::string(bn) + "2c", 1, filt[st][1], filt[st][2], 1, hout, hout);
            if (first) add(std::string(base) + "1", std::string(bn) + "1", 1, cin, filt[st][2], s, h, hout);
            cin = filt[st][2];
            h = hout;
        }
    }
    return net;
}

const Network& network() {
    static const Network n = build_network();
    return n;
}

}

const std::vector<ConvSpec>& specs() { return network().specs; }
const std::vector<ResBlock>& blocks() { return network().blocks; }

struct PlanOption {
    int HpePlan::*member;
    int HpeConfig::*cfg;
    const char* env;
    int dflt[2];
    int mask[2];
    int lo, hi;
};

constexpr int ANY = -1, NO_LO = INT_MIN, NO_HI = INT_MAX;

const PlanOption kPlanOptions[] = {
    {&HpePlan::n_streams, &HpeConfig::n_streams, "HPE_STREAMS", {2, 2}, {ANY, ANY}, 1, 4},
    {&HpePlan::dual_gemm, &HpeConfig::dual_gemm, "HPE_DUAL", {1, 1}, {ANY, ANY}, NO_LO, NO_HI},
    {&HpePlan::stem_fused, &HpeConfig::stem_fused, "HPE_STEM_FUSED", {1, 1}, {ANY, ANY}, NO_LO, NO_HI},
    {&HpePlan::wino_min_c, &HpeConfig::wino_min_c, "HPE_WINO_MINC", {128, 128}, {ANY, ANY}, NO_LO, NO_HI},
    {&HpePlan::wino_min_items, &HpeConfig::wino_min_items, "HPE_WINO_MIN_ITEMS", {128, 128}, {ANY, ANY}, NO_LO, NO_HI},
    {&HpePlan::wino_fused, &HpeConfig::wino_fused, "HPE_WINO_FUSED", {1, 1}, {ANY, ANY}, NO_LO, NO_HI},
    {&HpePlan::wino_fused_min_hw, &HpeConfig::wino_fused_min_hw, "HPE_WINO_FUSED_MINHW", {28, 28}, {ANY, ANY}, NO_LO, NO_HI},
    {&HpePlan::mesh_a2b, &HpeConfig::mesh_a2b, "HPE_MESH_A2B", {0, 0}, {ANY, ANY}, NO_LO, NO_HI},
    {&HpePlan::wino_f4, &HpeConfig::wino_f4, "HPE_WINO_F4", {7, 7}, {ANY, ANY}, NO_LO, NO_HI},
    {&HpePlan::wino4_fused, &HpeConfig::wino4_fused, "HPE_WINO4_FUSED", {0, 0}, {12, 12}, NO_LO, NO_HI},
    {&HpePlan::bf16_p8, &HpeConfig::bf16_p8, "HPE_BF16_P8", {0, 0}, {ANY, ANY}, NO_LO, NO_HI},
    {&HpePlan::wino4_ksplit, &HpeConfig::wino4_ksplit, "HPE_WINO4_KSPLIT", {1, 1}, {ANY, ANY}, NO_LO, NO_HI},
    {&HpePlan::chain_fuse, &HpeConfig::chain_fuse, "HPE_CHAIN", {8, 7}, {8, 23}, NO_LO, NO_HI},
    {&HpePlan::halo3, &HpeConfig::halo3, "HPE_HALO3", {15, 15}, {0, 15}, NO_LO, NO_HI},
    {&HpePlan::f32_split, &HpeConfig::f32_split, "HPE_F32_SPLIT", {14, 14}, {15, 0}, NO_LO, NO_HI},
    {&HpePlan::chunk_images, nullptr, "HPE_CHUNK", {0, 0}, {ANY, ANY}, NO_LO, NO_HI},
    {&HpePlan::min_chunk, nullptr, "HPE_MIN_CHUNK", {32, 24}, {ANY, ANY}, NO_LO, NO_HI},
    {&HpePlan::halo3_two, nullptr, "HPE_HALO3_TWO", {4, 4}, {7, 7}, NO_LO, NO_HI},
    {&HpePlan::f32s_min_tiles, nullptr, "HPE_F32S_MIN_TILES", {128, 128}, {ANY, ANY}, NO_LO, NO_HI},
    {&HpePlan::wino_streamk, nullptr, "HPE_WINO_STREAMK", {0, 0}, {ANY, ANY}, NO_LO, NO_HI},
    {&HpePlan::concurrent_tiles, nullptr, "HPE_CONCURRENT_TILES", {0, 0}, {ANY, ANY}, NO_LO, NO_HI},
    {&HpePlan::bf16_w8_min_tiles, nullptr, "HPE_BF16_W8_MIN_TILES", {128, 128}, {ANY, ANY}, NO_LO, NO_HI},
    {&HpePlan::wide128_min_tiles, nullptr, "HPE_WIDE128_MIN_TILES", {384, 384}, {ANY, ANY}, NO_LO, NO_HI},
    {&HpePlan::force_wide, nullptr, "HPE_TILE_WIDE", {-1, -1}, {ANY, ANY}, NO_LO, NO_HI},
    {&HpePlan::splitk_min_slabs, nullptr, "HPE_SPLITK_SLABS", {4, 4}, {ANY, ANY}, 2, NO_HI},
    {&HpePlan::wino4_min_items, nullptr, "HPE_WINO4_MIN_ITEMS", {64, 64}, {ANY, ANY}, NO_LO, NO_HI},
    {&HpePlan::wino4_n32, nullptr, "HPE_WINO4_N32", {256, 256}, {ANY, ANY}, NO_LO, NO_HI},
    {&HpePlan::w4_abl, nullptr, "HPE_W4_ABL", {0, 0}, {ANY, ANY}, NO_LO, NO_HI},
};

HpePlan hpe_resolve_plan(const HpeConfig& cfg) {
    const int dt = cfg.encoder_dtype == 1 ? 1 : 0;
    HpePlan pl;
    for (const PlanOption& o : kPlanOptions) {
        int v = o.dflt[dt];
        const char* e = getenv(o.env);
        if (o.cfg && cfg.*o.cfg >= 0) v = cfg.*o.cfg;
        else if (e && o.member == &HpePlan::mesh_a2b) v = e[0] == 'v' ? 1 : (e[0] == 'm' ? 2 : 0);
        else if (e) v = atoi(e);
        v &= o.mask[dt];
        pl.*o.member = v < o.lo ? o.lo : (v > o.hi ? o.hi : v);
    }
    if (pl.min_chunk < 8) pl.min_chunk = dt ? 24 : 32;
    pl.wino_fused = pl.wino_fused && pl.wino_min_c > 0;
    if (pl.wino_min_c <= 0) pl.wino_f4 = pl.wino4_fused = 0;
    return pl;
}

static int pick_f32s(const HpePlan& pl, bool split_packed, int M, int N, int K, bool residual_expand) {
    if (!split_packed || N <= 64) return -1;
    if (residual_expand && K < PLAN_F32S_EXPAND_MIN_K) return -1;
    const int tile = residual_expand ? PLAN_F32S_EXPAND_TILE : PLAN_F32S_TILE;
    const TileShape ts = tile_shape(GEMM_K_F32S, tile);
    return (long)((M + ts.bm - 1) / ts.bm) * ((N + ts.bn - 1) / ts.bn) >= pl.f32s_min_tiles ? tile : -1;
}

int pick_tile(const HpePlan& pl, int M, int N, int K, bool residual_expand, bool concurrent) {
    const bool wide = N > 64;
    if (wide && residual_expand) return (long)((M + 127) / 128) * ((N + 63) / 64) < PLAN_EXPAND_SMALL_GRID ? TILE_64x64 : TILE_128x64_W8;
    if (wide && pl.force_wide >= 0) return pl.force_wide;
    if (!wide) return TILE_128x64;
    if (K <= 128 && M >= 150000) return PLAN_SHORTK_TILE;
    if ((concurrent || pl.concurrent_tiles) && pl.wide128_min_tiles > 0 && (long)((M + 127) / 128) * ((N + 127) / 128) >= pl.wide128_min_tiles) return TILE_128x128;
    if (M >= 150000) return TILE_64x128;
    return TILE_64x64;
}

static int pick_bf16(const HpePlan& pl, int M, int N, int K, bool residual_expand, bool concurrent, int mode) {
    if (pl.bf16_p8 && N >= PLAN_BF16_P8_MIN_N && N % 256 == 0 && K >= PLAN_BF16_P8_MIN_K && !residual_expand) {
        const int bit = mode == GEMM_CONV3 ? (N == 256 ? 1 : 2) : (mode == GEMM_DUAL ? (N >= 2048 ? 8 : 16) : 4);
        if (pl.bf16_p8 & bit) return TILE_P8_256x256;
    }
    if (N <= 64) return TILE_128x64;
    const long t128 = (long)((M + 127) / 128) * ((N + 127) / 128);
    int tile = t128 >= ((concurrent || pl.concurrent_tiles) ? PLAN_BF16_128_MIN_TILES : 512) ? TILE_128x128 : TILE_64x128;
    if (residual_expand) tile = TILE_128x64_W8;
    else if (M <= 16384 && M >= 8192 && K >= 1024 && N >= 256) tile = TILE_256x128_W8;
    if (pl.bf16_w8_min_tiles > 0 && t128 >= pl.bf16_w8_min_tiles) tile = TILE_128x128_W8;
    return tile;
}

unsigned layer_packs(const HpePlan& pl, bool bf16, int idx) {
    const ConvSpec& s = specs()[idx];
    unsigned m = idx == 0 ? PACK_STEM_W : 0;
    const int slab = bf16 ? 64 : 32;
    const ResBlock* blk = nullptr;
    for (const ResBlock& b : blocks())
        if (b.first && b.i2c == idx) blk = &b;
    if (pl.dual_gemm && blk && s.cin % slab == 0 && specs()[blk->i1].cin % slab == 0) {
        m |= PACK_W_DUAL;
        if (!bf16 && (pl.f32_split & stage_bit(s.hout))) m |= PACK_W_DUAL_SPLIT;
    }
    if (bf16) return m;
    if (idx != 0 && s.kh == 1 && (pl.f32_split & stage_bit(s.hout))) m |= PACK_W_SPLIT;
    const bool wino = s.kh == 3 && s.stride == 1 && s.cin % 32 == 0 && s.cout % 64 == 0;
    if (wino && pl.wino_min_c > 0 && (s.cin >= pl.wino_min_c || (pl.wino_fused && s.hin >= pl.wino_fused_min_hw))) m |= PACK_WINO_U;
    if (wino && ((pl.wino_f4 | pl.wino4_fused) & f4_bit(s.hin))) m |= PACK_WINO4_U;
    return m;
}

static ConvRoute route_gemm(const HpePlan& pl, bool bf16, int mode, int M, int N, int K, bool expand, bool split_packed, bool concurrent) {
    ConvRoute r{CONV_K_F32, mode, -1, false, false, concurrent};
    if (bf16) {
        r.tile = pick_bf16(pl, M, N, K, expand, concurrent, mode);
        r.kernel = r.tile == TILE_P8_256x256 ? CONV_K_BF16_P8 : CONV_K_BF16;
    } else if ((r.tile = pick_f32s(pl, split_packed, M, N, K, expand)) >= 0) {
        r.kernel = CONV_K_F32S;
    } else {
        r.tile = pick_tile(pl, M, N, K, expand, concurrent);
    }
    return r;
}

ConvRoute route_conv(const HpePlan& pl, bool bf16, int idx, const ConvQuery& q) {
    const ConvSpec& s = specs()[idx];
    const unsigned packs = layer_packs(pl, bf16, idx);
    const int B = q.B, H = s.hin;
    const int mode = idx == 0 ? GEMM_STEM : s.kh == 3 ? GEMM_CONV3 : s.stride == 1 ? GEMM_DENSE : GEMM_STRIDED;
    const bool plain3 = mode == GEMM_CONV3 && s.stride == 1 && !q.residual;
    auto special = [&](int kernel) { return ConvRoute{kernel, mode, -1, kernel == CONV_K_WINO_FUSED || kernel == CONV_K_WINO4_FUSED, false, q.concurrent}; };
    const int min4 = pl.wino_min_items < pl.wino4_min_items ? pl.wino_min_items : pl.wino4_min_items;
    if (plain3 && (packs & PACK_WINO4_U) && (pl.wino4_fused & f4_bit(H)) && hpe_wino4_fused_items(B, H, H, s.cout) >= min4) return special(CONV_K_WINO4_FUSED);
    const bool f4 = plain3 && (packs & PACK_WINO4_U) && (pl.wino_f4 & f4_bit(H)) && hpe_wino4_items(B, H, H, s.cout) >= min4;
    if (plain3 && !f4 && pl.wino_fused && (packs & PACK_WINO_U) && H >= pl.wino_fused_min_hw && hpe_wino_fused_items(B, H, H, s.cout) >= pl.wino_min_items)
        return special(CONV_K_WINO_FUSED);
    if (f4 && q.workspace) return special(CONV_K_WINO4);
    if (plain3 && (packs & PACK_WINO_U) && q.workspace && s.cin >= pl.wino_min_c &&
        (long)((B * ((H + 1) / 2) * ((H + 1) / 2) + 63) / 64) * (s.cout / 64) >= pl.wino_min_items)
        return special(CONV_K_WINO);
    if (bf16 && plain3 && (pl.halo3 & f4_bit(H)) && hpe_halo3_bf16_supported(H, s.cin, s.cout)) return special(CONV_K_HALO3);
    return route_gemm(pl, bf16, mode, B * s.hout * s.hout, s.cout, conv_k_pad(idx, bf16), mode == GEMM_DENSE && q.residual && s.cout == 4 * s.cin,
                      (packs & PACK_W_SPLIT) != 0, q.concurrent);
}

static bool use_chain(const HpePlan& pl, bool bf16, const ResBlock& blk) {
    if (blk.last) return false;
    const int stg = blk.stage, i2c = blk.i2c;
    const ConvSpec& s2 = specs()[i2c];
    const ConvSpec& sn = specs()[i2c + (blk.first ? 2 : 1)];
    if (sn.kh != 1 || sn.stride != 1 || sn.cin != s2.cout) return false;
    if (!bf16) return !blk.first && stg == 0 && (pl.chain_fuse & 8) && hpe_chain_f32_supported(s2.cin, s2.cout, sn.cout);
    if (blk.first) {
        const ConvSpec& s1 = specs()[blk.i1];
        return stg == 0 && (pl.chain_fuse & 4) && (layer_packs(pl, bf16, i2c) & PACK_W_DUAL) && s1.stride == 1 && s1.hin == s2.hin &&
               hpe_chain_bf16_supported(s2.cin, s2.cout, sn.cout, s1.cin);
    }
    const int bit = stg == 0 ? 1 : stg == 1 ? 2 : stg == 2 ? 16 : 0;
    return (pl.chain_fuse & bit) && hpe_chain_bf16_supported(s2.cin, s2.cout, sn.cout, 0);
}

BlockRoute route_block(const HpePlan& pl, bool bf16, const ResBlock& blk, ConvQuery q) {
    BlockRoute b{};
    q.residual = false;
    b.r2a = route_conv(pl, bf16, blk.i2a, q);
    b.r2b = route_conv(pl, bf16, blk.i2b, q);
    b.r2a.out_slab8 = b.r2b.in_slab8;
    const ConvSpec& s2 = specs()[blk.i2c];
    if (use_chain(pl, bf16, blk)) {
        b.join = JOIN_CHAIN;
        b.u1_slab8 = route_conv(pl, bf16, blk.i2c + (blk.first ? 3 : 2), q).in_slab8;
    } else if (blk.first && (layer_packs(pl, bf16, blk.i2c) & PACK_W_DUAL)) {
        b.join = JOIN_DUAL;
        b.r2c = route_gemm(pl, bf16, GEMM_DUAL, q.B * s2.hout * s2.hout, s2.cout, s2.cin + specs()[blk.i1].cin, false,
                           (layer_packs(pl, bf16, blk.i2c) & PACK_W_DUAL_SPLIT) != 0, q.concurrent);
    } else {
        if (blk.first) b.r1 = route_conv(pl, bf16, blk.i1, q);
        q.residual = true;
        b.r2c = route_conv(pl, bf16, blk.i2c, q);
    }
    return b;
}
```

### human-pose-estimation_amd/predictor.py

```python
from __future__ import annotations

import os
from os.path import dirname, join

import numpy as np

from . import engine as _engine
from .projection import batch_orth_proj_idrot
from .smpl import SMPL
from . import assets


def _load_smpl_file(path):
    return assets.load_smpl_model(path)


def _load_mean_file(smpl_model_path):
    return assets.load_mean_params(smpl_model_path)


def resolve_critic_params(config, critic_params=None, weights=None, checkpoint_info=None):
    if critic_params is not None:
        return critic_params
    critic_params = getattr(config, "critic_params", None)
    if critic_params is not None:
        return critic_params
    if weights is not None and any(k.startswith("critic/") for k in weights):
        return weights
    if checkpoint_info is not None:
        from . import tf_checkpoint

        try:
            return tf_checkpoint.load_critic_weights(checkpoint_info["prefix"])[0]
        except tf_checkpoint.NoCriticError:
            return None
    return None


class Predictor(object):
    def __init__(self, config, smpl_model=None, mean_params=None, encoder_params=None, regressor_params=None, device=None,
                 critic_params=None):
        import torch

        self.model_dir = getattr(config, "model_dir", None)
        self.load_path = getattr(config, "load_path", None)
        self.data_format = getattr(config, "data_format", "NHWC")
        self.smpl_model_path = getattr(config, "smpl_model_path", None)
        self.pretrained_model_path = getattr(config, "pretrained_model_path", None)
        self.img_size = getattr(config, "img_size", 224)
        self.num_stage = getattr(config, "num_stage", 3)
        self.batch_size = getattr(config, "batch_size", 8)
        self.checkpoint_dir = getattr(config, "checkpoint_dir", None)
        self.smpl_face_path = getattr(config, "smpl_face_path", None)
        self._renderer = None
        if self.img_size != 224:
            raise ValueError("img_size must be 224 (the encoder plan is built for 224x224 inputs)")
        self.num_joints = 14
        self.proj_fn = batch_orth_proj_idrot
        self.num_cam = 3
        self.num_theta = 72
        self.total_params = self.num_theta + self.num_cam + 10

        if device is None:
            device = torch.cuda.current_device() if torch.cuda.is_available() else 0
        self.engine = _engine.HpeEngine(
            device=device, max_batch=self.batch_size, num_stage=self.num_stage, bn_eps=getattr(config, "bn_eps", 1e-3),
            encoder_dtype=getattr(config, "encoder_dtype", "fp32"), **(getattr(config, "plan_options", None) or {}),
        )
        if smpl_model is None:
            smpl_model = getattr(config, "smpl_model", None)
        if smpl_model is None:
            smpl_model = _load_smpl_file(self.smpl_model_path)
        self.engine.load_smpl(smpl_model, joint_type="cocoplus")
        self._mean_params = mean_params if mean_params is not None else getattr(config, "mean_params", None)
        self.mean_np = self.load_mean_param()
        self.engine.load_mean_theta(self.mean_np)
        w, self.checkpoint_info = None, None
        if encoder_params is None or regressor_params is None:
            w = getattr(config, "weights", None)
            if w is None and self.checkpoint_dir and os.path.exists(join(self.checkpoint_dir, "weights.npz")):
                with np.load(join(self.checkpoint_dir, "weights.npz"), allow_pickle=False) as z:
                    w = {k: z[k] for k in z.files}
            if w is None and self.checkpoint_dir and os.path.exists(join(self.checkpoint_dir, "checkpoint")):
                from . import tf_checkpoint

                w, self.checkpoint_info = tf_checkpoint.load_hmr_weights(self.checkpoint_dir)
            if w is None:
                raise FileNotFoundError(
                    "no encoder/regressor weights: pass encoder_params/regressor_params, config.weights, or put a "
                    "TensorFlow checkpoint (checkpoint + ckpt-N.index/.data-*) or weights.npz (Keras-layout names) in "
                    "config.checkpoint_dir"
                )
            encoder_params = encoder_params or w
            regressor_params = regressor_params or w
            if self.checkpoint_info is not None and "mean_var" in w:
                self.mean_np = np.asarray(w["mean_var"], np.float32).reshape(1, self.total_params)
                self.engine.load_mean_theta(self.mean_np)
        self.engine.load_encoder(encoder_params)
        self.engine.load_regressor(regressor_params)
        self.engine.finalize()
        critic_params = resolve_critic_params(config, critic_params, w, self.checkpoint_info)
        if critic_params is not None:
            self.engine.load_critic(critic_params)
        self.smpl = SMPL(None, engine=self.engine)
        self.mean_var = torch.from_numpy(self.mean_np).to(self.engine.tdev)
        self.theta_prev = self.mean_var
        if w is not None and "inital_theta" in w:
            self.theta_prev = torch.from_numpy(np.asarray(w["inital_theta"], np.float32)).to(self.engine.tdev)

    @property
    def renderer(self):
        if self._renderer is None:
            if not self.smpl_face_path:
                raise FileNotFoundError("Predictor.renderer needs the SMPL faces: set config.smpl_face_path (smpl_faces.npy, or an SMPL "
                                        ".pkl / .npz with an 'f' field)")
            from .render import SMPLRenderer

            self._renderer = SMPLRenderer(img_size=self.img_size, face_path=self.smpl_face_path, max_batch=self.batch_size,
                                          device=self.engine.device)
        return self._renderer

    def load_mean_param(self):
        mean = np.zeros((1, self.total_params))
        mean[0, 0] = 0.9
        mean_vals = self._mean_params if self._mean_params is not None else _load_mean_file(self.smpl_model_path)
        mean_pose = np.array(mean_vals["pose"], dtype=np.float64).copy()
        mean_pose[:3] = 0.0
        mean_shape = np.array(mean_vals["shape"], dtype=np.float64)
        mean_pose[0] = np.pi
        mean[0, 3:] = np.hstack((mean_pose, mean_shape))
        return mean.astype(np.float32)

    def _to_device(self, images):
        import torch

        if isinstance(images, np.ndarray):
            images = torch.from_numpy(np.ascontiguousarray(images, dtype=np.float32))
        if not images.is_cuda:
            images = images.to(self.engine.tdev, non_blocking=True)
        return images.float()

    def predict(self, images, all_stages=False):
        import torch

        images = self._to_device(images)
        if images.dim() != 4 or tuple(images.shape[1:]) != (224, 224, 3):
            raise ValueError("images must be [B,224,224,3] NHWC, got %s" % (tuple(images.shape),))
        B = images.shape[0]
        chunks = []
        many = B > self.batch_size
        try:
            for lo in range(0, B, self.batch_size):
                chunks.append(self.engine.forward(images[lo : lo + self.batch_size], all_stages=all_stages, pipelined=many))
        finally:
            if many:
                self.engine.join()
        if len(chunks) == 1:
            stages = chunks[0]
        else:
            stages = [{k: torch.cat([c[i][k] for c in chunks], 0) for k in chunks[0][i]} for i in range(len(chunks[0]))]
        last = stages[-1]
        result = {
            "generated_joints": last["joints"],
            "generated_verts": last["verts"],
            "generated_cams": last["cams"],
            "theta": last["theta"],
            "J_transformed": last["J_transformed"],
            "generated_kp2d": last["kp2d"],
        }
        if all_stages:
            result["stages"] = stages
        return result

    def val_step(self, images, seg_gts, kp2d_gts, use_mesh_repro_loss=True, kpr_loss_weight=60.0, mr_loss_weight=0.001,
                 reduce_fn=None, critic_loss_weight=None):
        import torch

        if critic_loss_weight is not None and not self.engine.has_critic:
            raise RuntimeError("val_step(critic_loss_weight=...) needs critic weights: pass critic_params / config.critic_params, put "
                               "critic/<layer>/kernel|bias into weights.npz, or use a checkpoint that holds its discriminator")

        images = self._to_device(images)
        seg = self._to_device(seg_gts)
        if seg.dim() == 4:
            seg = seg[..., 0]
        seg = seg.contiguous()
        kp_gt = self._to_device(kp2d_gts).contiguous()
        B = images.shape[0]
        if B > self.batch_size:
            raise ValueError("val_step needs B <= config.batch_size")
        want = ("verts", "joints", "cams", "theta", "kp2d") + (("verts2d",) if use_mesh_repro_loss else ())
        if critic_loss_weight is not None:
            want += ("Rs",)
        stages = self.engine.forward(images, all_stages=True, want=want)
        packed = self.engine.val_losses(kp_gt, [st["kp2d"] for st in stages], seg if use_mesh_repro_loss else None,
                                        [st["verts2d"] for st in stages] if use_mesh_repro_loss else None)
        if critic_loss_weight is not None:
            from .ops import generator_critic_loss

            parts = torch.stack([generator_critic_loss(self.engine, st["joints"], st["theta"][:, 75:], st["Rs"], return_parts=True)
                                 for st in stages])
            packed = torch.cat([packed, parts], 1)
        if reduce_fn is not None:
            packed = reduce_fn(packed)
        if critic_loss_weight is not None:
            packed, parts = packed[:, :4].contiguous(), packed[:, 4:].contiguous()
        kpr = [packed[i, 2] * kpr_loss_weight for i in range(len(stages))]
        result = {"kpr_losses": kpr, "pred_keypoints": torch.stack([s["kp2d"] for s in stages], 1),
                  "generated_verts": torch.stack([s["verts"] for s in stages], 1),
                  "generated_cams": torch.stack([s["cams"] for s in stages], 1), "loss_parts": packed}
        if use_mesh_repro_loss:
            result["mr_losses"] = [packed[i, 3] * mr_loss_weight for i in range(len(stages))]
        if critic_loss_weight is not None:
            result["critic_parts"] = parts
            result["generator_critic_losses"] = [-(parts[i, :3] / parts[i, 3]).sum() * critic_loss_weight for i in range(len(stages))]
        return result

    def predict_single_image(self, image):
        image = self._to_device(image)
        pred_results = self.predict(image.unsqueeze(0))
# ... 2 lines not shown
```

### include/hpe.h

```cpp
#ifndef HPE_H_
#define HPE_H_

#ifdef __cplusplus
extern "C" {
#endif

#define HPE_OK 0
#define HPE_ERR_INVALID 1
#define HPE_ERR_HIP 2
#define HPE_ERR_STATE 3
#define HPE_ERR_NO_DEVICE 4

#define HPE_NUM_CONV 53
#define HPE_NUM_DENSE 3
#define HPE_NUM_CRITIC_DENSE 9
#define HPE_NUM_VERTS 6890
#define HPE_NUM_JOINTS 24
#define HPE_NUM_BETAS 10
#define HPE_NUM_POSE_BASIS 207
#define HPE_THETA_DIM 85
#define HPE_FEATURE_DIM 2048
#define HPE_MAX_KP 24
#define HPE_IMG_SIZE 224

typedef struct hpe_ctx hpe_ctx;

typedef struct HpeConfig {
    int struct_size;
    int device;
    int max_batch;
    int num_stage;
    float bn_eps;
    int encoder_dtype;
    int n_streams;
    int dual_gemm;
    int stem_fused;
    int wino_min_c;
    int wino_min_items;
    int wino_fused;
    int wino_fused_min_hw;
    int mesh_a2b;
    int wino_f4;
    int wino4_fused;
    int bf16_p8;
    int wino4_ksplit;
    int chain_fuse;
    int halo3;
    int f32_split;
} HpeConfig;

void hpe_config_init(HpeConfig* cfg);

typedef struct HpeSmplModel {
    const float* v_template;
    const float* shapedirs;
    const float* posedirs;
    const float* J_regressor;
    const float* weights;
    const float* kp_regressor;
    const int* parents;
    int num_kp;
} HpeSmplModel;

typedef struct HpeOutputs {
    float* verts;
    float* joints;
    float* cams;
    float* theta;
    float* J_transformed;
    float* kp2d;
    float* verts2d;
    float* Rs;
} HpeOutputs;

const char* hpe_last_error(void);
const char* hpe_version(void);

const char* hpe_conv_layer_name(int idx);
const char* hpe_bn_layer_name(int idx);
int hpe_conv_layer_geometry(int idx, int out[7]);

int hpe_create(const HpeConfig* cfg, hpe_ctx** out);
int hpe_destroy(hpe_ctx* ctx);

int hpe_load_smpl(hpe_ctx* ctx, const HpeSmplModel* host_model);
int hpe_load_conv(hpe_ctx* ctx, int idx, const float* kernel_hwio, const float* bias, const float* gamma,
                  const float* beta, const float* moving_mean, const float* moving_variance);
int hpe_load_dense(hpe_ctx* ctx, int idx, const float* kernel_in_out, const float* bias);
int hpe_load_mean_theta(hpe_ctx* ctx, const float* mean85);
int hpe_finalize(hpe_ctx* ctx);

int hpe_forward(hpe_ctx* ctx, const float* images_dev, int B, const HpeOutputs* stage_outs, int n_outs, void* stream);

int hpe_forward_pipelined(hpe_ctx* ctx, const float* images_dev, int B, const HpeOutputs* stage_outs, int n_outs, void* stream);
int hpe_join(hpe_ctx* ctx, void* stream);
int hpe_tail(hpe_ctx* ctx, const float* features_dev, int B, const HpeOutputs* stage_outs, int n_outs, void* stream);
void* hpe_tail_stream(hpe_ctx* ctx);

int hpe_encoder(hpe_ctx* ctx, const float* images_dev, int B, float* features_dev, void* stream);
int hpe_regress_stage(hpe_ctx* ctx, const float* features_dev, const float* theta_prev_dev, int B, float* theta_out_dev,
                      void* stream);
int hpe_smpl(hpe_ctx* ctx, const float* theta_dev, int B, const HpeOutputs* outs, void* stream);
int hpe_smpl_backward(hpe_ctx* ctx, const float* theta_dev, int B, const HpeOutputs* grad_outs, float* grad_theta_dev, void* stream);
int hpe_orth_proj(const float* X_dev, const float* cam_dev, int B, int P, float* out_dev, void* stream);
int hpe_reproject_vertices(const float* verts_dev, const float* cam_dev, int B, int P, float im_w, float im_h, float* out_dev,
                           void* stream);
int hpe_kp_loss(const float* kp_gt_dev, const float* kp_pred_dev, int B, int K, float* out_dev, void* stream);
int hpe_kp_loss_backward(const float* kp_gt_dev, const float* kp_pred_dev, int B, int K, const float* grad_loss_dev,
                         float* grad_kp_pred_dev, void* stream);
int hpe_mesh_loss(hpe_ctx* ctx, const float* seg_dev, const float* verts2d_dev, int B, int H, int W, int P, float* out_dev,
                  void* stream);
int hpe_mesh_loss_grad(hpe_ctx* ctx, const float* seg_dev, const float* verts2d_dev, int B, int H, int W, int P,
                       float* out_dev, float* grad_verts2d_dev, int* nn_pix_dev, int* nn_vert_dev, void* stream);

const char* hpe_critic_layer_name(int idx);
int hpe_critic_layer_shape(int idx, int out[2]);
typedef struct HpeCriticModel {
    const float* kernel[HPE_NUM_CRITIC_DENSE];
    const float* bias[HPE_NUM_CRITIC_DENSE];
} HpeCriticModel;
int hpe_load_critic(hpe_ctx* ctx, const HpeCriticModel* host_model);
int hpe_critic(hpe_ctx* ctx, const float* joints_dev, int K, const float* betas_dev, int betas_stride, const float* Rs_dev, int N,
               float* scores_dev, float* kcs_dev, void* stream);
int hpe_critic_backward(hpe_ctx* ctx, const float* joints_dev, int K, const float* betas_dev, int betas_stride, const float* Rs_dev, int N,
                        const float* grad_scores_dev, float* grad_joints_dev, float* grad_betas_dev, float* grad_Rs_dev,
                        float* grad_kcs_dev, void* stream);

int hpe_critic_param_floats(void);
int hpe_critic_param_offset(int idx, int is_bias);
long long hpe_critic_weight_grad_ws_floats(int N);
int hpe_critic_reserve(hpe_ctx* ctx, int N);
int hpe_critic_weight_grad(hpe_ctx* ctx, const float* joints_dev, int K, const float* betas_dev, int betas_stride, const float* Rs_dev,
                           int N, const float* grad_scores_dev, const float* tangent_kcs_dev, const float* tangent_joints_dev,
                           const float* tangent_betas_dev, const float* tangent_Rs_dev, int tangent_per_row, float* grad_params_dev,
                           void* stream);
int hpe_critic_get_params(hpe_ctx* ctx, float* flat_dev, void* stream);
int hpe_critic_set_params_dev(hpe_ctx* ctx, const float* flat_dev, void* stream);

int hpe_regressor_param_floats(void);
int hpe_regressor_param_offset(int idx, int is_bias);
int hpe_regressor_get_params(hpe_ctx* ctx, float* flat_dev, void* stream);
int hpe_regressor_set_params_dev(hpe_ctx* ctx, const float* flat_dev, void* stream);
int hpe_regressor_forward_train(hpe_ctx* ctx, const float* features_dev, int B, const float* drop_dev, float* thetas_dev, void* stream);
int hpe_regressor_backward(hpe_ctx* ctx, const float* features_dev, int B, const float* drop_dev, const float* grad_thetas_dev,
                           float* grad_flat_dev, float* grad_features_dev, void* stream);

int hpe_encoder_param_floats(void);
int hpe_encoder_param_offset(int idx, int which);
int hpe_encoder_train_reserve(hpe_ctx* ctx, int B);
long long hpe_encoder_train_ws_floats(int B);
int hpe_encoder_wg_slices(int idx, int B);
int hpe_encoder_forward_train(hpe_ctx* ctx, const float* images_dev, int B, float* features_dev, void* stream);
int hpe_encoder_backward(hpe_ctx* ctx, const float* images_dev, int B, const float* grad_features_dev, float* grad_flat_dev, void* stream);
int hpe_encoder_get_params(hpe_ctx* ctx, float* flat_dev, void* stream);
int hpe_encoder_set_params(hpe_ctx* ctx, const float* flat_host);
int hpe_encoder_set_params_dev(hpe_ctx* ctx, const float* flat_dev, void* stream);
enum {
    HPE_PACK_W = 0,
    HPE_PACK_W_SPLIT,
    HPE_PACK_WINO_U,
    HPE_PACK_WINO4_U,
    HPE_PACK_STEM_W,
    HPE_PACK_SCALE,
    HPE_PACK_SHIFT,
    HPE_PACK_W_DUAL,
    HPE_PACK_W_DUAL_SPLIT,
    HPE_PACK_SHIFT_DUAL,
    HPE_PACK_DXW,
    HPE_PACK_FLAT,
    HPE_PACK_COUNT
};
long long hpe_debug_encoder_packing_bytes(hpe_ctx* ctx, int idx, int which);
int hpe_debug_encoder_packing(hpe_ctx* ctx, int idx, int which, void* dst_dev, void* stream);
int hpe_debug_conv_backward(hpe_ctx* ctx, int idx, const float* x_dev, const float* y_dev, const float* dy_dev, int B, float* dx_dev,
                            float* grad_layer_dev, void* stream);
int hpe_debug_maxpool_backward(const float* x_dev, const float* dy_dev, int B, int H, int C, float* dx_dev, void* stream);
int hpe_debug_avgpool_backward(const float* dy_dev, int B, int HW, int C, float* dx_dev, void* stream);
int hpe_debug_encoder_stash(hpe_ctx* ctx, int idx, float* out_dev, void* stream);
int hpe_debug_encoder_stash_batch(hpe_ctx* ctx);

int hpe_encoder_stat_floats(void);
int hpe_encoder_stat_offset(int idx, int which);
int hpe_encoder_train_reserve_batchnorm(hpe_ctx* ctx, int B);
long long hpe_encoder_train_ws_floats_batchnorm(int B);
int hpe_encoder_forward_batchnorm(hpe_ctx* ctx, const float* images_dev, int B, float* features_dev, void* stream);
int hpe_encoder_backward_batchnorm(hpe_ctx* ctx, const float* images_dev, int B, const float* grad_features_dev, float* grad_flat_dev, void* stream);
int hpe_encoder_get_stats(hpe_ctx* ctx, float* stats_dev, void* stream);
int hpe_encoder_update_stats(hpe_ctx* ctx, float* stats_dev, double momentum, int unbiased, void* stream);
int hpe_encoder_set_stats_dev(hpe_ctx* ctx, const float* stats_dev, void* stream);
int hpe_debug_conv_batchnorm(hpe_ctx* ctx, int idx, const float* x_dev, int B, const float* residual_dev, int relu, float* y_dev, float* z_out_dev,
                             float* stats_out_dev, void* stream);
int hpe_debug_conv_backward_batchnorm(hpe_ctx* ctx, int idx, const float* x_dev, const float* z_dev, const float* y_dev, const float* dy_dev, int B,
                                      float* dx_dev, float* grad_layer_dev, void* stream);
int hpe_debug_encoder_stash_raw(hpe_ctx* ctx, int idx, float* out_dev, void* stream);
int hpe_debug_encoder_batch_stats(hpe_ctx* ctx, float* out_dev, void* stream);
int hpe_debug_encoder_bn_slices(int idx, int B);

int hpe_val_losses(hpe_ctx* ctx, const float* seg_dev, const float* kp_gt_dev, const float* const* kp2d_dev,
                   const float* const* verts2d_dev, int n_stage, int B, int K, int H, int W, int P, float* out_dev, void* stream);

int hpe_preprocess_u8(const unsigned char* img_dev, int H, int W, int C, float* out224_dev, int proc_param[5], void* stream);
int hpe_preprocess_u8_batch(const unsigned char* frames_dev, const long long* offsets, const int* sizes_hw, int B, int C,
                            float* out_dev, int* proc_params, void* table_dev, void* stream);
int hpe_get_original(const float* verts_dev, const float* cam_dev, int B, int P, int K, const int start_pt[2], float scale,
                     int img_size, float* vert_shifted_dev, float cam_for_render[3], float* kp_original_host,
                     const float* joints2d_host, void* stream);

typedef struct HpeAugmentFrame {
    long long frame_offset;
    long long seg_offset;
    int H, W;
    int newH, newW;
    int cx, cy;
    float fx, fy;
    int flip;
    int inside;
    float rx, ry;
} HpeAugmentFrame;

int hpe_augment_plan(int B, const int* sizes_hw, const int* centers_xy, const int* trans_xy, const float* scales,
                     const unsigned char* flips, int trans_max, const long long* frame_offsets, const long long* seg_offsets,
                     HpeAugmentFrame* table_out);
int hpe_augment_batch(const unsigned char* frames_dev, const unsigned char* segs_dev, const HpeAugmentFrame* table_host,
                      const HpeAugmentFrame* table_dev, const float* kp_dev, int B, float* images_out, float* seg_out, float* kp_out,
                      void* stream);

int hpe_adam_advance(double* state_dev, double lr, double beta1, double beta2, void* stream);
int hpe_adam_apply(float* p, float* m, float* v, const float* g, long long n, const double* state_dev, float one_minus_beta1,
                   float one_minus_beta2, float eps, void* stream);
int hpe_adam_set_step(double* state_dev, long long t, double beta1, double beta2, void* stream);
int hpe_debug_adam_power(double beta, long long t, double* out);

#define HPE_JPEG_MAX_SIDE 16384
typedef struct HpeJpegInfo {
    int status;
    int H, W, ncomp;
    int hs[3], vs[3];
    int blocks_w[3], blocks_h[3];
    long long coefs;
} HpeJpegInfo;

typedef struct HpeJpegImage {
    long long coef_offset[3];
    long long plane_offset[3];
    long long out_offset;
    int H, W;
    int ncomp;
    int channels;
    int hmax, vmax;
    int blocks_w[3], blocks_h[3];
    int idct_group0;
    int store_group0;
    unsigned char quant[3][64];
} HpeJpegImage;

int hpe_jpeg_info(int B, const unsigned char* const* streams, const long long* lengths, HpeJpegInfo* info_out);
int hpe_jpeg_decode(int B, const unsigned char* const* streams, const long long* lengths, const int* channels, int threads,
                    short* coef_out, long long coef_capacity, HpeJpegImage* table_out, int* status_out, long long* totals_out);
int hpe_jpeg_backend(const HpeJpegImage* table_host, const HpeJpegImage* table_dev, int B, const short* coef_dev, long long coef_count,
                     unsigned char* workspace_dev, long long workspace_bytes, unsigned char* frames_dev, long long frames_bytes,
                     void* stream);

#define HPE_JPEG_ENC_HEADER_BYTES 640
#define HPE_JPEG_ENC_BLOCK_BYTES 416
typedef struct HpeJpegEncImage {
    long long frame_offset;
    long long coef_offset[3];
    int H, W;
    int C;
    int hmax, vmax;
    int blocks_w[3], blocks_h[3];
    int real_w[3], real_h[3];
    int group0;
    unsigned char quant[2][64];
} HpeJpegEncImage;

int hpe_jpeg_encode_layout(int B, const int* shapes, const long long* frame_offsets, int hmax, int vmax, int quality,
                           HpeJpegEncImage* table_out, long long* totals_out);
int hpe_jpeg_forward(const HpeJpegEncImage* table_host, const HpeJpegEncImage* table_dev, int B, const unsigned char* frames_dev,
                     long long frames_bytes, short* coef_dev, long long coef_count, void* stream);
int hpe_jpeg_entropy_encode(const HpeJpegEncImage* table, int B, const short* coef, long long coef_count, int units, int xdensity,
                            int ydensity, int threads, unsigned char* out, long long out_capacity, long long* offsets_out,
                            long long* lengths_out);

#define HPE_PNG_MAX_SIDE 16384
#define HPE_PNG_STORE_BYTES_PER_GROUP 1024
typedef struct HpePngImage {
    long long raw_offset;
    long long pal_offset;
    long long work_offset;
    long long out_offset;
    int H, W;
    int color_type;
    int depth;
    int channels;
    int rowbytes;
    int bpp;
    int store_group0;
} HpePngImage;

int hpe_png_backend(const HpePngImage* table_host, const HpePngImage* table_dev, int B, const unsigned char* raw_dev, long long raw_bytes,
                    unsigned char* workspace_dev, long long workspace_bytes, unsigned char* frames_dev, long long frames_bytes,
                    void* stream);

typedef struct HpePngFilterImage {
    long long frame_offset;
    long long scan_offset;
    int H, W;
    int C;
    int row0;
} HpePngFilterImage;

int hpe_png_filter(const HpePngFilterImage* table_host, const HpePngFilterImage* table_dev, int B, const unsigned char* frames_dev,
                   long long frames_bytes, unsigned char* scan_dev, long long scan_bytes, void* stream);

#define HPE_DRAW_JOINTS 19
#define HPE_DRAW_MAX_RADIUS 256
int hpe_draw_panels(const float* images, const float* kp_gt, const float* kp_pred, const unsigned char* rend_img,
                    const unsigned char* rend_seg, const int* skeleton, int n, int T, int S, unsigned char* out, void* stream);
int hpe_draw_skeleton(unsigned char* images, const float* joints, const unsigned char* vis, const int* skeleton, int n, int H, int W,
                      int draw_edges, int radius, void* stream);

// ... 96 lines not shown
```

Baseline: 20730 images/sec.

## Add fp32 halo 3x3 conv kernel using three-way bf16 split MFMA

```diff
diff --git a/human-pose-estimation_amd/_lib.py b/human-pose-estimation_amd/_lib.py
--- a/human-pose-estimation_amd/_lib.py
+++ b/human-pose-estimation_amd/_lib.py
@@ -43,10 +43,11 @@
         ("chain_fuse", C.c_int),
         ("halo3", C.c_int),
         ("f32_split", C.c_int),
+        ("conv3_split", C.c_int),
     ]
 
 
-PLAN_OPTIONS = ("n_streams", "dual_gemm", "stem_fused", "wino_min_c", "wino_min_items", "wino_fused", "wino_fused_min_hw", "mesh_a2b", "wino_f4", "wino4_fused", "bf16_p8", "wino4_ksplit", "chain_fuse", "halo3", "f32_split")
+PLAN_OPTIONS = ("n_streams", "dual_gemm", "stem_fused", "wino_min_c", "wino_min_items", "wino_fused", "wino_fused_min_hw", "mesh_a2b", "wino_f4", "wino4_fused", "bf16_p8", "wino4_ksplit", "chain_fuse", "halo3", "f32_split", "conv3_split")
 
 
 class HpeSmplModel(C.Structure):
@@ -150,7 +151,7 @@
     return r
 
 
-ENCODER_PACKINGS = ("w", "w_split", "wino_u", "wino4_u", "stem_w", "scale", "shift", "w_dual", "w_dual_split", "shift_dual", "dxw", "flat")
+ENCODER_PACKINGS = ("w", "w_split", "wino_u", "wino4_u", "stem_w", "scale", "shift", "w_dual", "w_dual_split", "shift_dual", "dxw", "flat", "conv3_split")
 
 OUTPUT_FIELDS = ("verts", "joints", "cams", "theta", "J_transformed", "kp2d", "verts2d", "Rs")
 
diff --git a/human-pose-estimation_amd/build.py b/human-pose-estimation_amd/build.py
--- a/human-pose-estimation_amd/build.py
+++ b/human-pose-estimation_amd/build.py
@@ -9,7 +9,7 @@
 CSRC = os.path.join(HERE, "csrc")
 LIBDIR = os.path.join(HERE, "lib")
 LIB = os.path.join(LIBDIR, "libhpe_hip.so")
-SOURCES = ["conv_gemm.hip", "conv_gemm_f32s.hip", "conv_gemm_bf16.hip", "conv_gemm_bf16_p8.hip", "conv_chain_bf16.hip", "conv_chain_f32.hip", "conv3_halo_bf16.hip", "conv_wino.hip", "conv_wino4.hip", "stem_fused.hip", "encoder_ops.hip", "smpl.hip", "losses.hip", "prepost.hip", "render.hip", "hpe_plan.hip", "hpe_finalize.hip", "hpe_encoder.hip", "hpe_api.hip", "hpe_render_api.hip", "smpl_bwd.hip", "critic.hip", "critic_train.hip", "regressor_train.hip", "augment.hip", "encoder_train.hip", "encoder_grad.hip", "encoder_repack.hip", "encoder_bn.hip", "jpeg_entropy.hip", "jpeg_decode.hip", "jpeg_huffman_enc.hip", "jpeg_encode.hip", "png_decode.hip", "png_encode.hip", "draw.hip", "adam.hip"]
+SOURCES = ["conv_gemm.hip", "conv_gemm_f32s.hip", "conv_gemm_bf16.hip", "conv_gemm_bf16_p8.hip", "conv_chain_bf16.hip", "conv_chain_f32.hip", "conv3_halo_bf16.hip", "conv3_halo_f32s.hip", "conv_wino.hip", "conv_wino4.hip", "stem_fused.hip", "encoder_ops.hip", "smpl.hip", "losses.hip", "prepost.hip", "render.hip", "hpe_plan.hip", "hpe_finalize.hip", "hpe_encoder.hip", "hpe_api.hip", "hpe_render_api.hip", "smpl_bwd.hip", "critic.hip", "critic_train.hip", "regressor_train.hip", "augment.hip", "encoder_train.hip", "encoder_grad.hip", "encoder_repack.hip", "encoder_bn.hip", "jpeg_entropy.hip", "jpeg_decode.hip", "jpeg_huffman_enc.hip", "jpeg_encode.hip", "png_decode.hip", "png_encode.hip", "draw.hip", "adam.hip"]
 CFLAGS = ["--offload-arch=gfx950", "-O3", "-std=c++17", "-fPIC", "-fvisibility=hidden", "-fno-fast-math"]
 
 
diff --git a/human-pose-estimation_amd/csrc/conv3_halo_f32s.hip b/human-pose-estimation_amd/csrc/conv3_halo_f32s.hip
--- /dev/null
+++ b/human-pose-estimation_amd/csrc/conv3_halo_f32s.hip
@@ -0,0 +1,251 @@
+#include <hip/hip_runtime.h>
+#include <stdint.h>
+#include <stdlib.h>
+
+#include "hpe_internal.h"
+
+typedef float f32x16 __attribute__((ext_vector_type(16)));
+typedef float f32x4 __attribute__((ext_vector_type(4)));
+typedef __bf16 bf16x8 __attribute__((ext_vector_type(8)));
+typedef __bf16 bf16x4 __attribute__((ext_vector_type(4)));
+
+namespace {
+
+__device__ __forceinline__ void dma16(const void* src, void* lds_dst) {
+    __builtin_amdgcn_global_load_lds((const __attribute__((address_space(1))) void*)src, (__attribute__((address_space(3))) void*)lds_dst, 16, 0, 0);
+}
+__device__ __forceinline__ void lds_barrier() { asm volatile("s_waitcnt lgkmcnt(0)\n\ts_barrier" ::: "memory"); }
+
+__device__ __forceinline__ void split3(const f32x4& x, bf16x4& h0, bf16x4& h1, bf16x4& h2) {
+#pragma unroll
+    for (int e = 0; e < 4; ++e) {
+        const __bf16 b0 = (__bf16)x[e];
+        const float r1 = x[e] - (float)b0;
+        const __bf16 b1 = (__bf16)r1;
+        const float r2 = r1 - (float)b1;
+        h0[e] = b0;
+        h1[e] = b1;
+        h2[e] = (__bf16)r2;
+    }
+}
+
+template <int HW, int CIN, int BM, int NR>
+__global__ __launch_bounds__(BM, 2) void conv3_halo_f32s_kernel(Halo3SplitArgs p) {
+    constexpr int BN = 64, KC = 16, NTHR = BM, NW = BM / 64;
+    constexpr int CS = CIN / KC;
+    constexpr int HALO = HW + 1;
+    constexpr int ROWS = BM + 2 * HALO;
+    constexpr int ROWB = KC * 2;
+    constexpr int PLANE = 256 + ((ROWS * ROWB + 255) / 256) * 256;
+    constexpr int W_PIECE = BN * ROWB;
+    constexpr int W_BYTES = 3 * W_PIECE;
+    constexpr int WPC = W_BYTES / 1024;
+    constexpr int WI = (WPC + NW - 1) / NW;
+    constexpr int D = NR - 1;
+    constexpr int A_OFF = NR * W_BYTES;
+    constexpr int NA = (ROWS * 4 + NTHR - 1) / NTHR;
+    constexpr int OUT_BYTES = BM * BN * 4;
+    constexpr int LDS_BYTES = A_OFF + 3 * PLANE > OUT_BYTES ? A_OFF + 3 * PLANE : OUT_BYTES;
+    constexpr int STEPS = 9 * CS;
+    static_assert((NR & (NR - 1)) == 0 && D >= 1 && D <= 8 && CIN % KC == 0 && BM % 64 == 0 && A_OFF % 256 == 0 && LDS_BYTES <= 80 * 1024, "geometry");
+
+    __shared__ __attribute__((aligned(256))) unsigned char lds[LDS_BYTES];
+
+    const int t = threadIdx.x;
+    const int lane = t & 63;
+    const int wave = __builtin_amdgcn_readfirstlane(t >> 6);
+    const int hi = lane >> 5;
+    const int swz = xcd_remap(blockIdx.x, (int)gridDim.x);
+    const int mtile = __builtin_amdgcn_readfirstlane(swz / p.n_ntiles);
+    const int n0 = (swz - mtile * p.n_ntiles) * BN;
+    const int m0 = mtile * BM;
+
+    if (t < 48) reinterpret_cast<f32x4*>(lds + A_OFF + (t >> 4) * PLANE)[t & 15] = f32x4{0.f, 0.f, 0.f, 0.f};
+
+    auto row_item = [&](int i, int& r, int& c4) {
+        int tt = t;
+        asm volatile("" : "+v"(tt));
+        int q = tt + NTHR * i;
+        if (q >= ROWS * 4) q = ROWS * 4 - 1;
+        r = q >> 2, c4 = q & 3;
+    };
+    f32x4 xa[NA];
+    auto load_rows = [&](int cs) {
+#pragma unroll
+        for (int i = 0; i < NA; ++i) {
+            int r, c4;
+            row_item(i, r, c4);
+            long g = (long)m0 - HALO + r;
+            g = g < 0 ? 0 : (g >= p.M ? p.M - 1 : g);
+            xa[i] = *reinterpret_cast<const f32x4*>(p.x + (size_t)g * CIN + cs * KC + c4 * 4);
+        }
+    };
+    auto write_planes = [&]() {
+#pragma unroll
+        for (int i = 0; i < NA; ++i) {
+            int r, c4;
+            row_item(i, r, c4);
+            unsigned char* d = lds + A_OFF + 256 + r * ROWB + ((((c4 >> 1) ^ (r >> 3)) & 1) << 4) + (c4 & 1) * 8;
+            bf16x4 h0, h1, h2;
+            split3(xa[i], h0, h1, h2);
+            *reinterpret_cast<bf16x4*>(d) = h0;
+            *reinterpret_cast<bf16x4*>(d + PLANE) = h1;
+            *reinterpret_cast<bf16x4*>(d + 2 * PLANE) = h2;
+        }
+    };
+
+    unsigned woff[WI];
+    int wdst[WI];
+#pragma unroll
+    for (int i = 0; i < WI; ++i) {
+        const int pi = wave + NW * i < WPC ? wave + NW * i : wave;
+        const int r = (pi & 1) * 32 + (lane >> 1);
+        woff[i] = (unsigned)((((pi >> 1) * p.N + n0 + r) * KC + (((lane ^ (r >> 3)) & 1) << 3)) * 2);
+        wdst[i] = pi * 1024;
+    }
+    const char* Wb = reinterpret_cast<const char*>(p.w);
+    auto issue_w = [&](int s, int buf) {
+        const char* base = Wb + (size_t)s * 3 * p.N * ROWB;
+#pragma unroll
+        for (int i = 0; i < WI; ++i) dma16(base + woff[i], lds + buf * W_BYTES + wdst[i]);
+    };
+
+    int arow[2];
+    unsigned amask[2];
+#pragma unroll
+    for (int i = 0; i < 2; ++i) {
+        const int ml = wave * 64 + i * 32 + (lane & 31);
+        arow[i] = ml + HALO;
+        long m = (long)m0 + ml;
+        if (m >= p.M) m = p.M - 1;
+        const int xw = (int)(m % HW), yh = (int)((m / HW) % HW);
+        unsigned mk = 0;
+#pragma unroll
+        for (int tap = 0; tap < 9; ++tap) {
+            const int dh = tap / 3 - 1, dw = tap % 3 - 1;
+            if ((unsigned)(yh + dh) < (unsigned)HW && (unsigned)(xw + dw) < (unsigned)HW) mk |= 1u << tap;
+        }
+        amask[i] = mk;
+    }
+    unsigned wfrag[2];
+#pragma unroll
+    for (int j = 0; j < 2; ++j) {
+        const int r = j * 32 + (lane & 31);
+        wfrag[j] = (unsigned)(r * ROWB + (((hi ^ (r >> 3)) & 1) << 4));
+    }
+
+    f32x16 acc[2][2], acx[2][2];
+#pragma unroll
+    for (int i = 0; i < 2; ++i)
+#pragma unroll
+        for (int j = 0; j < 2; ++j)
+#pragma unroll
+            for (int e = 0; e < 16; ++e) acc[i][j][e] = acx[i][j][e] = 0.f;
+
+    load_rows(0);
+#pragma unroll
+    for (int u = 0; u < D; ++u) issue_w(u, u);
+
+#pragma unroll 1
+    for (int cs = 0; cs < CS; ++cs) {
+        write_planes();
+#pragma unroll
+        for (int tap = 0; tap < 9; ++tap) {
+            const int s = cs * 9 + tap;
+            const int buf = s & (NR - 1);
+            __builtin_amdgcn_sched_barrier(0);
+            if (tap >= 1 && tap <= D) asm volatile("s_waitcnt vmcnt(%0)" ::"n"((D - 1) * WI + NA) : "memory");
+            else asm volatile("s_waitcnt vmcnt(%0)" ::"n"((D - 1) * WI) : "memory");
+            lds_barrier();
+
+            const int shift = (tap / 3 - 1) * HW + (tap % 3 - 1);
+            bf16x8 a[3][2], w[3][2];
+#pragma unroll
+            for (int i = 0; i < 2; ++i) {
+                int ar = arow[i];
+                asm volatile("" : "+v"(ar));
+                const int lr = ar + shift;
+                const unsigned in_row = (unsigned)(lr * ROWB + (((hi ^ (lr >> 3)) & 1) << 4));
+                const unsigned off = ((amask[i] >> tap) & 1u) ? 256u + in_row : (in_row & 255u);
+#pragma unroll
+                for (int pc = 0; pc < 3; ++pc) a[pc][i] = *reinterpret_cast<const bf16x8*>(lds + A_OFF + pc * PLANE + off);
+            }
+#pragma unroll
+            for (int j = 0; j < 2; ++j)
+#pragma unroll
+                for (int pc = 0; pc < 3; ++pc) w[pc][j] = *reinterpret_cast<const bf16x8*>(lds + buf * W_BYTES + pc * W_PIECE + wfrag[j]);
+
+            const int sn = s + D < STEPS ? s + D : s + D - STEPS;
+            issue_w(sn, (buf + D) & (NR - 1));
+            if (tap == 0) load_rows(cs + 1 < CS ? cs + 1 : cs);
+
+#pragma unroll
+            for (int i = 0; i < 2; ++i)
+#pragma unroll
+                for (int j = 0; j < 2; ++j) {
+                    acx[i][j] = __builtin_amdgcn_mfma_f32_32x32x16_bf16(w[0][j], a[2][i], acx[i][j], 0, 0, 0);
+                    acx[i][j] = __builtin_amdgcn_mfma_f32_32x32x16_bf16(w[1][j], a[1][i], acx[i][j], 0, 0, 0);
+                    acx[i][j] = __builtin_amdgcn_mfma_f32_32x32x16_bf16(w[2][j], a[0][i], acx[i][j], 0, 0, 0);
+                    acx[i][j] = __builtin_amdgcn_mfma_f32_32x32x16_bf16(w[0][j], a[1][i], acx[i][j], 0, 0, 0);
+                    acx[i][j] = __builtin_amdgcn_mfma_f32_32x32x16_bf16(w[1][j], a[0][i], acx[i][j], 0, 0, 0);
+                    acc[i][j] = __builtin_amdgcn_mfma_f32_32x32x16_bf16(w[0][j], a[0][i], acc[i][j], 0, 0, 0);
+                }
+        }
+        __builtin_amdgcn_sched_barrier(0);
+        asm volatile("s_waitcnt vmcnt(%0)" ::"n"(D * WI) : "memory");
+        lds_barrier();
+    }
+    asm volatile("s_waitcnt vmcnt(0)" ::: "memory");
+    lds_barrier();
+
+#pragma unroll
+    for (int i = 0; i < 2; ++i) {
+        const int ml = wave * 64 + i * 32 + (lane & 31);
+#pragma unroll
+        for (int j = 0; j < 2; ++j)
+#pragma unroll
+            for (int g = 0; g < 4; ++g) {
+                const int c = j * 32 + 8 * g + 4 * hi;
+                const f32x4 sc = *reinterpret_cast<const f32x4*>(p.scale + n0 + c);
+                const f32x4 sh = *reinterpret_cast<const f32x4*>(p.shift + n0 + c);
+                f32x4 o;
+#pragma unroll
+                for (int k = 0; k < 4; ++k) {
+                    const float v = (acc[i][j][4 * g + k] + acx[i][j][4 * g + k]) * sc[k] + sh[k];
+                    o[k] = p.relu ? fmaxf(v, 0.f) : v;
+                }
+                *reinterpret_cast<f32x4*>(lds + ml * (BN * 4) + (((c >> 2) ^ (ml & 7)) << 4)) = o;
+            }
+    }
+    asm volatile("s_waitcnt vmcnt(0)" ::: "memory");
+    lds_barrier();
+#pragma unroll
+    for (int pass = 0; pass < (BM * 16) / NTHR; ++pass) {
+        const int idx = pass * NTHR + t;
+        const int r = idx >> 4, u = idx & 15;
+        const f32x4 v = *reinterpret_cast<const f32x4*>(lds + r * (BN * 4) + ((u ^ (r & 7)) << 4));
+        const long m = (long)m0 + r;
+        if (m < p.M) *reinterpret_cast<f32x4*>(p.y + (size_t)m * p.N + n0 + u * 4) = v;
+    }
+}
+
+template <int HW, int CIN, int BM, int NR = 4>
+hipError_t launch_halo3s(Halo3SplitArgs p, hipStream_t st) {
+    p.n_ntiles = p.N / 64;
+    const int grid = ((p.M + BM - 1) / BM) * p.n_ntiles;
+    hipLaunchKernelGGL((conv3_halo_f32s_kernel<HW, CIN, BM, NR>), dim3(grid), dim3(BM), 0, st, p);
+    return hipGetLastError();
+}
+
+}
+
+bool hpe_halo3_f32s_supported(int HW, int Cin, int N) { return (HW == 56 && Cin == 64 && N == 64) || (HW == 28 && Cin == 128 && N == 128); }
+
+int hpe_halo3_f32s_items(int B, int HW, int N) { return ((B * HW * HW + 255) / 256) * (N / 64); }
+
+hipError_t hpe_launch_halo3_f32s(const Halo3SplitArgs& p, int HW, int Cin, hipStream_t st) {
+    if (!hpe_halo3_f32s_supported(HW, Cin, p.N)) return hipErrorInvalidValue;
+    if (p.M <= 0 || p.M % (HW * HW) != 0 || !p.x || !p.w || !p.y || !p.scale || !p.shift) return hipErrorInvalidValue;
+    if ((((uintptr_t)p.x | (uintptr_t)p.w | (uintptr_t)p.y | (uintptr_t)p.scale | (uintptr_t)p.shift) & 15) != 0) return hipErrorInvalidValue;
+    return HW == 56 ? launch_halo3s<56, 64, 256>(p, st) : launch_halo3s<28, 128, 256>(p, st);
+}
diff --git a/human-pose-estimation_amd/csrc/encoder_repack.hip b/human-pose-estimation_amd/csrc/encoder_repack.hip
--- a/human-pose-estimation_amd/csrc/encoder_repack.hip
+++ b/human-pose-estimation_amd/csrc/encoder_repack.hip
@@ -8,11 +8,14 @@
 
 struct RepackLayer {
     float *w, *scale, *shift, *wino_u, *wino4_u, *dxw;
-    unsigned short* w_split;
-    int kh, cin, cout, n_pad, k_pad;
+    unsigned short *w_split, *w3_split;
+    short kh, cin, cout, n_pad;
+    int k_pad;
     int off[4];
     int stat;
 };
+
+static_assert(sizeof(RepackLayer) == 96, "the repack table is counted in hpe_encoder_train_ws_floats");
 
 struct RepackDual {
     float *w, *shift;
@@ -75,6 +78,7 @@
         const float v = (row >= 0 && n < L.cout) ? src[row * L.cout + n] : 0.f;
         L.w[(size_t)n * L.k_pad + k] = v;
         if (L.w_split) store_split(L.w_split + (size_t)n * 3 * L.k_pad + k, L.k_pad, v);
+        if (L.w3_split && row >= 0 && n < L.cout) store_split(L.w3_split + conv3_split_index(n, k / L.cin, k % L.cin, 0, L.cout), (size_t)L.cout * 16, v);
     }
 }
 
@@ -217,6 +221,7 @@
             if (c->et.flat) p = c->et.flat + layout().off[idx][0];
             n = ((size_t)s.kh * s.kw * s.cin * s.cout + 3 * (size_t)s.cout) * 4;
             break;
+        case HPE_PACK_CONV3_SPLIT: p = L.w3_split, n = u * 27 * 2; break;
     }
     *bytes = p ? n : 0;
     return *bytes ? p : nullptr;
@@ -239,10 +244,11 @@
         r.wino4_u = L.wino4_u;
         r.dxw = c->et.dxw[i];
         r.w_split = static_cast<unsigned short*>(L.w_split);
-        r.kh = s.kh;
-        r.cin = s.cin;
-        r.cout = s.cout;
-        r.n_pad = L.n_pad;
+        r.w3_split = static_cast<unsigned short*>(L.w3_split);
+        r.kh = (short)s.kh;
+        r.cin = (short)s.cin;
+        r.cout = (short)s.cout;
+        r.n_pad = (short)L.n_pad;
         r.k_pad = L.k_pad;
         for (int w = 0; w < 4; ++w) r.off[w] = layout().off[i][w];
         r.stat = layout().stat[i];
diff --git a/human-pose-estimation_amd/csrc/hpe_api.hip b/human-pose-estimation_amd/csrc/hpe_api.hip
--- a/human-pose-estimation_amd/csrc/hpe_api.hip
+++ b/human-pose-estimation_amd/csrc/hpe_api.hip
@@ -64,7 +64,7 @@
     cfg->bn_eps = 1e-3f;
     cfg->encoder_dtype = 0;
     cfg->n_streams = cfg->dual_gemm = cfg->stem_fused = cfg->wino_min_c = cfg->wino_min_items = cfg->wino_fused = -1;
-    cfg->wino_fused_min_hw = cfg->mesh_a2b = cfg->wino_f4 = cfg->wino4_fused = cfg->bf16_p8 = cfg->wino4_ksplit = cfg->chain_fuse = cfg->halo3 = cfg->f32_split = -1;
+    cfg->wino_fused_min_hw = cfg->mesh_a2b = cfg->wino_f4 = cfg->wino4_fused = cfg->bf16_p8 = cfg->wino4_ksplit = cfg->chain_fuse = cfg->halo3 = cfg->f32_split = cfg->conv3_split = -1;
 }
 
 int hpe_create(const HpeConfig* cfg, hpe_ctx** out) {
diff --git a/human-pose-estimation_amd/csrc/hpe_ctx.h b/human-pose-estimation_amd/csrc/hpe_ctx.h
--- a/human-pose-estimation_amd/csrc/hpe_ctx.h
+++ b/human-pose-estimation_amd/csrc/hpe_ctx.h
@@ -50,6 +50,7 @@
     int k_dual = 0, k1_dual = 0;
     void* w_split = nullptr;
     void* w_dual_split = nullptr;
+    void* w3_split = nullptr;
     void* stem_w = nullptr;
     float* wino_u = nullptr;
     float* wino4_u = nullptr;
@@ -115,6 +116,10 @@
     h[1] = f2bf(r1);
     const float r2 = r1 - bf2f(h[1]);
     h[2] = f2bf(r2);
+}
+
+__host__ __device__ inline size_t conv3_split_index(int n, int tap, int ci, int piece, int cout) {
+    return ((((size_t)(ci >> 4) * 9 + tap) * 3 + piece) * cout + n) * 16 + (ci & 15);
 }
 
 struct DenseLayer {
diff --git a/human-pose-estimation_amd/csrc/hpe_encoder.hip b/human-pose-estimation_amd/csrc/hpe_encoder.hip
--- a/human-pose-estimation_amd/csrc/hpe_encoder.hip
+++ b/human-pose-estimation_amd/csrc/hpe_encoder.hip
@@ -50,6 +50,13 @@
             return hpe_launch_wino_conv3(x, s.cin, L.wino_u, scale, shift, y, s.cout, B, H, H, s.cin, s.cout, relu, wino_v, c->wino_ws ? &sk : nullptr, st);
         }
         case CONV_K_HALO3: {
+            if (!c->bf16) {
+                if (!L.w3_split) return hipErrorInvalidValue;
+                Halo3SplitArgs h{};
+                h.x = x, h.w = L.w3_split, h.y = y, h.scale = scale, h.shift = shift;
+                h.M = B * s.hout * s.hout, h.N = s.cout, h.relu = relu;
+                return hpe_launch_halo3_f32s(h, H, s.cin, st);
+            }
             Halo3Args h{};
             h.x = reinterpret_cast<const __bf16*>(x), h.w = reinterpret_cast<const __bf16*>(L.w), h.y = reinterpret_cast<__bf16*>(y);
             h.scale = scale, h.shift = shift;
diff --git a/human-pose-estimation_amd/csrc/hpe_finalize.hip b/human-pose-estimation_amd/csrc/hpe_finalize.hip
--- a/human-pose-estimation_amd/csrc/hpe_finalize.hip
+++ b/human-pose-estimation_amd/csrc/hpe_finalize.hip
@@ -266,6 +266,18 @@
         }
     if ((rc = upload_to(c, &L.wino4_u, U))) return rc;
     return HPE_OK;
+}
+
+static int pack_conv3_split(hpe_ctx* c, const ConvSpec& s, ConvLayer& L) {
+    std::vector<unsigned short> ws((size_t)27 * s.cin * s.cout);
+    for (int tap = 0; tap < 9; ++tap)
+        for (int ci = 0; ci < s.cin; ++ci)
+            for (int n = 0; n < s.cout; ++n) {
+                unsigned short h[3];
+                bf16_split3(L.kernel[((size_t)tap * s.cin + ci) * s.cout + n], h);
+                for (int j = 0; j < 3; ++j) ws[conv3_split_index(n, tap, ci, j, s.cout)] = h[j];
+            }
+    return upload_bf16(c, &L.w3_split, ws);
 }
 
 static int pack_stem_weights(hpe_ctx* c, ConvLayer& L) {
@@ -310,6 +322,7 @@
             if ((packs & PACK_W_SPLIT) && (rc = upload_split(c, &L.w_split, wt, L.n_pad, L.k_pad))) return rc;
             if ((packs & PACK_WINO_U) && (rc = pack_wino_weights(c, s, L))) return rc;
             if ((packs & PACK_WINO4_U) && (rc = pack_wino4_weights(c, s, L))) return rc;
+            if ((packs & PACK_CONV3_SPLIT) && (rc = pack_conv3_split(c, s, L))) return rc;
         }
         if ((packs & PACK_STEM_W) && (rc = pack_stem_weights(c, L))) return rc;
         std::vector<float> sc(s.cout), sh(s.cout);
diff --git a/human-pose-estimation_amd/csrc/hpe_internal.h b/human-pose-estimation_amd/csrc/hpe_internal.h
--- a/human-pose-estimation_amd/csrc/hpe_internal.h
+++ b/human-pose-estimation_amd/csrc/hpe_internal.h
@@ -102,6 +102,18 @@
 };
 bool hpe_halo3_bf16_supported(int HW, int Cin, int N);
 hipError_t hpe_launch_halo3_bf16(const Halo3Args& p, int HW, int Cin, hipStream_t st);
+struct Halo3SplitArgs {
+    const float* x;
+    const void* w;
+    const float* scale;
+    const float* shift;
+    float* y;
+    int M, N, relu;
+    int n_ntiles;
+};
+bool hpe_halo3_f32s_supported(int HW, int Cin, int N);
+int hpe_halo3_f32s_items(int B, int HW, int N);
+hipError_t hpe_launch_halo3_f32s(const Halo3SplitArgs& p, int HW, int Cin, hipStream_t st);
 
 bool hpe_chain_bf16_supported(int C, int C4, int CP, int C2);
 hipError_t hpe_launch_chain_bf16(const ChainArgs& p, int C, int C4, int CP, int C2, hipStream_t st);
diff --git a/human-pose-estimation_amd/csrc/hpe_plan.h b/human-pose-estimation_amd/csrc/hpe_plan.h
--- a/human-pose-estimation_amd/csrc/hpe_plan.h
+++ b/human-pose-estimation_amd/csrc/hpe_plan.h
@@ -18,6 +18,7 @@
     int chain_fuse = 0;
     int halo3 = 0;
     int f32_split = 0;
+    int conv3_split = 0;
     int chunk_images = 0;
     int min_chunk = 32;
     int halo3_two = 4;
@@ -40,6 +41,7 @@
 constexpr int PLAN_SHORTK_TILE = TILE_128x64_W8;
 constexpr int PLAN_F32S_TILE = TILE_128x128;
 constexpr int PLAN_F32S_EXPAND_TILE = TILE_128x128_W8;
+constexpr int PLAN_CONV3_SPLIT_MIN_ITEMS = 256;
 constexpr int PLAN_F32S_EXPAND_MIN_K = 256;
 
 HpePlan hpe_resolve_plan(const HpeConfig& cfg);
@@ -48,7 +50,8 @@
 inline int f4_bit(int hin) { return hin <= 7 ? 1 : (hin <= 14 ? 2 : (hin <= 28 ? 4 : 8)); }
 
 constexpr unsigned PACK_W_SPLIT = 1u << HPE_PACK_W_SPLIT, PACK_WINO_U = 1u << HPE_PACK_WINO_U, PACK_WINO4_U = 1u << HPE_PACK_WINO4_U,
-                   PACK_STEM_W = 1u << HPE_PACK_STEM_W, PACK_W_DUAL = 1u << HPE_PACK_W_DUAL, PACK_W_DUAL_SPLIT = 1u << HPE_PACK_W_DUAL_SPLIT;
+                   PACK_STEM_W = 1u << HPE_PACK_STEM_W, PACK_W_DUAL = 1u << HPE_PACK_W_DUAL, PACK_W_DUAL_SPLIT = 1u << HPE_PACK_W_DUAL_SPLIT,
+                   PACK_CONV3_SPLIT = 1u << HPE_PACK_CONV3_SPLIT;
 unsigned layer_packs(const HpePlan& pl, bool bf16, int idx);
 
 enum ConvKernel { CONV_K_F32 = 0, CONV_K_F32S, CONV_K_BF16, CONV_K_BF16_P8, CONV_K_HALO3, CONV_K_WINO, CONV_K_WINO_FUSED, CONV_K_WINO4, CONV_K_WINO4_FUSED };
diff --git a/human-pose-estimation_amd/csrc/hpe_plan.hip b/human-pose-estimation_amd/csrc/hpe_plan.hip
--- a/human-pose-estimation_amd/csrc/hpe_plan.hip
+++ b/human-pose-estimation_amd/csrc/hpe_plan.hip
@@ -98,6 +98,7 @@
     {&HpePlan::chain_fuse, &HpeConfig::chain_fuse, "HPE_CHAIN", {8, 7}, {8, 23}, NO_LO, NO_HI},
     {&HpePlan::halo3, &HpeConfig::halo3, "HPE_HALO3", {15, 15}, {0, 15}, NO_LO, NO_HI},
     {&HpePlan::f32_split, &HpeConfig::f32_split, "HPE_F32_SPLIT", {14, 14}, {15, 0}, NO_LO, NO_HI},
+    {&HpePlan::conv3_split, &HpeConfig::conv3_split, "HPE_CONV3_SPLIT", {0, 0}, {31, 0}, NO_LO, NO_HI},
     {&HpePlan::chunk_images, nullptr, "HPE_CHUNK", {0, 0}, {ANY, ANY}, NO_LO, NO_HI},
     {&HpePlan::min_chunk, nullptr, "HPE_MIN_CHUNK", {32, 24}, {ANY, ANY}, NO_LO, NO_HI},
     {&HpePlan::halo3_two, nullptr, "HPE_HALO3_TWO", {4, 4}, {7, 7}, NO_LO, NO_HI},
@@ -180,6 +181,7 @@
     const bool wino = s.kh == 3 && s.stride == 1 && s.cin % 32 == 0 && s.cout % 64 == 0;
     if (wino && pl.wino_min_c > 0 && (s.cin >= pl.wino_min_c || (pl.wino_fused && s.hin >= pl.wino_fused_min_hw))) m |= PACK_WINO_U;
     if (wino && ((pl.wino_f4 | pl.wino4_fused) & f4_bit(s.hin))) m |= PACK_WINO4_U;
+    if (s.kh == 3 && s.stride == 1 && (pl.conv3_split & f4_bit(s.hin)) && hpe_halo3_f32s_supported(s.hin, s.cin, s.cout)) m |= PACK_CONV3_SPLIT;
     return m;
 }
 
@@ -204,6 +206,7 @@
     const bool plain3 = mode == GEMM_CONV3 && s.stride == 1 && !q.residual;
     auto special = [&](int kernel) { return ConvRoute{kernel, mode, -1, kernel == CONV_K_WINO_FUSED || kernel == CONV_K_WINO4_FUSED, false, q.concurrent}; };
     const int min4 = pl.wino_min_items < pl.wino4_min_items ? pl.wino_min_items : pl.wino4_min_items;
+    if (plain3 && (packs & PACK_CONV3_SPLIT) && ((pl.conv3_split & 16) || hpe_halo3_f32s_items(B, H, s.cout) >= PLAN_CONV3_SPLIT_MIN_ITEMS)) return special(CONV_K_HALO3);
     if (plain3 && (packs & PACK_WINO4_U) && (pl.wino4_fused & f4_bit(H)) && hpe_wino4_fused_items(B, H, H, s.cout) >= min4) return special(CONV_K_WINO4_FUSED);
     const bool f4 = plain3 && (packs & PACK_WINO4_U) && (pl.wino_f4 & f4_bit(H)) && hpe_wino4_items(B, H, H, s.cout) >= min4;
     if (plain3 && !f4 && pl.wino_fused && (packs & PACK_WINO_U) && H >= pl.wino_fused_min_hw && hpe_wino_fused_items(B, H, H, s.cout) >= pl.wino_min_items)
diff --git a/human-pose-estimation_amd/predictor.py b/human-pose-estimation_amd/predictor.py
--- a/human-pose-estimation_amd/predictor.py
+++ b/human-pose-estimation_amd/predictor.py
@@ -35,6 +35,9 @@
         except tf_checkpoint.NoCriticError:
             return None
     return None
+
+
+CONV3_SPLIT_FP32 = 8
 
 
 class Predictor(object):
@@ -63,9 +66,13 @@
 
         if device is None:
             device = torch.cuda.current_device() if torch.cuda.is_available() else 0
+        encoder_dtype = getattr(config, "encoder_dtype", "fp32")
+        plan_options = getattr(config, "plan_options", None) or {}
+        if not plan_options and encoder_dtype == "fp32" and "HPE_CONV3_SPLIT" not in os.environ:
+            plan_options = {"conv3_split": CONV3_SPLIT_FP32}
         self.engine = _engine.HpeEngine(
             device=device, max_batch=self.batch_size, num_stage=self.num_stage, bn_eps=getattr(config, "bn_eps", 1e-3),
-            encoder_dtype=getattr(config, "encoder_dtype", "fp32"), **(getattr(config, "plan_options", None) or {}),
+            encoder_dtype=encoder_dtype, **plan_options,
         )
         if smpl_model is None:
             smpl_model = getattr(config, "smpl_model", None)
diff --git a/include/hpe.h b/include/hpe.h
--- a/include/hpe.h
+++ b/include/hpe.h
@@ -47,6 +47,7 @@
     int chain_fuse;
     int halo3;
     int f32_split;
+    int conv3_split;
 } HpeConfig;
 
 void hpe_config_init(HpeConfig* cfg);
@@ -168,6 +169,7 @@
     HPE_PACK_SHIFT_DUAL,
     HPE_PACK_DXW,
     HPE_PACK_FLAT,
+    HPE_PACK_CONV3_SPLIT,
     HPE_PACK_COUNT
 };
 long long hpe_debug_encoder_packing_bytes(hpe_ctx* ctx, int idx, int which);
```

Result: no change. 20730 images/sec, median of 2 (+0.0%).
